# auggiemarignier/pxmcmc

Hardware: AMD Instinct MI355X
Metric: MYULA samples/sec at L=256 synthesis (higher is better)
Workload: dtype f64

## Files before the change

include/pxmcmc_amd.h:

```cpp
#ifndef PXMCMC_AMD_H
#define PXMCMC_AMD_H

#include <stddef.h>
#include <stdint.h>

#ifdef __cplusplus
extern "C" {
#endif

typedef struct pxm_sht_plan_s* pxm_sht_plan_t;
typedef struct pxm_wav_plan_s* pxm_wav_plan_t;
typedef struct pxm_dwav_plan_s* pxm_dwav_plan_t;
typedef struct pxm_hwav_plan_s* pxm_hwav_plan_t;
typedef struct pxm_dft_plan_s* pxm_dft_plan_t;
typedef struct pxm_gemm_plan_s* pxm_gemm_plan_t;
typedef void* pxm_stream_t;

int pxm_version(void);
#ifdef PXM_NOISE_F64
#error "the -DPXM_NOISE_F64 build switch was removed: pass the flag PXM_NOISE_F64 per call (one library serves both precisions)"
#endif
#define PXM_NOISE_F64 16
int pxm_noise_bits(void);
int64_t pxm_host_check_address_ranges(int L, double B, int J_min, int spin, int max_chains, int what);
int64_t pxm_host_gram_table_bytes(int L, double B, int J_min, int spin, int max_chains);
const char* pxm_last_error(void);
int pxm_device_count(void);

int pxm_capture_begin(void);
int pxm_capture_end(void);
int pxm_deferred_pending(void);
int pxm_tables_trim(void);

int pxm_j_max(int L, double B);
int pxm_wav_bandlimits(int L, double B, int J_min, int* bl_out, int cap);
int64_t pxm_wav_ncoefs(int L, double B, int J_min, int64_t* nscal_out);
int pxm_tiling_axisym(int L, double B, int J_min, double* kappa0, double* kappa);
int pxm_mw_ring_weights(int L, double* q);
int pxm_host_sht_tables(int L, int spin, int m, double* Binv, double* Afwd);
int pxm_host_rec_table(int L, int spin, int m, double* Brec);
int pxm_host_rec_geometry(int L, int spin, int C, int* out);
int pxm_host_pfa511_tables(uint16_t* idx, double* b2);
int pxm_host_dft_geometry(int L, int* out);

int pxm_sht_plan_create(int L, int spin, int max_chains, unsigned flags, pxm_sht_plan_t* plan);
int pxm_sht_plan_destroy(pxm_sht_plan_t plan);
int pxm_sht_uses_recursion(pxm_sht_plan_t plan);
int pxm_rec_reduce_selftest(double* out128);
int pxm_sht_inverse(pxm_sht_plan_t plan, const void* flm, void* f, int C, pxm_stream_t stream);
int pxm_sht_forward(pxm_sht_plan_t plan, const void* f, void* flm, int C, pxm_stream_t stream);
int pxm_sht_inverse_adjoint(pxm_sht_plan_t plan, const void* f, void* flm, int C, pxm_stream_t stream);
int pxm_sht_forward_adjoint(pxm_sht_plan_t plan, const void* flm, void* f, int C, pxm_stream_t stream);
int64_t pxm_sht_table_bytes(pxm_sht_plan_t plan, int op );

int pxm_dft_plan_create(int L, int max_chains, pxm_dft_plan_t* plan);
int pxm_dft_plan_destroy(pxm_dft_plan_t plan);
int pxm_dft_px2ring(pxm_dft_plan_t plan, const void* f, void* G, int C, pxm_stream_t stream);
int pxm_dft_ring2px(pxm_dft_plan_t plan, const void* G, void* f, int C, pxm_stream_t stream);
int pxm_dft_status(pxm_dft_plan_t plan, int clear, pxm_stream_t stream);

#define PXM_GEMM_SIDE_INTS 16
int pxm_gemm_plan_create(int spin, int max_chains, int pk, const int* sides, int n_sides, pxm_gemm_plan_t* plan);
int pxm_gemm_plan_destroy(pxm_gemm_plan_t plan);
int64_t pxm_gemm_plan_report(pxm_gemm_plan_t plan, int what, int side, int64_t* out, int64_t cap);
int64_t pxm_host_gemm_plan_report(int spin, int max_chains, int pk, const int* sides, int n_sides, int what, int side,
                                  int64_t* out, int64_t cap);
int pxm_gemm_plan_write(pxm_gemm_plan_t plan, int64_t offset, const double* src, int64_t n, pxm_stream_t stream);
int pxm_gemm_plan_read(pxm_gemm_plan_t plan, int64_t offset, double* dst, int64_t n, pxm_stream_t stream);
int pxm_gemm_plan_table_read(pxm_gemm_plan_t plan, int side, int which, double* dst, int64_t n, pxm_stream_t stream);
int pxm_gemm_plan_run(pxm_gemm_plan_t plan, int C, int affine, double ns, double wr, double wi, int bump, pxm_stream_t stream);

int pxm_wav_plan_create(int L, double B, int J_min, int max_chains, unsigned flags, pxm_wav_plan_t* plan);
int pxm_wav_plan_create_spin(int L, double B, int J_min, int spin, int max_chains, unsigned flags, pxm_wav_plan_t* plan);
int pxm_wav_plan_destroy(pxm_wav_plan_t plan);
int pxm_wav_synthesis(pxm_wav_plan_t plan, const void* X, void* f, int C, pxm_stream_t stream);
int pxm_wav_synthesis_adjoint(pxm_wav_plan_t plan, const void* f, void* X, int C, pxm_stream_t stream);
int pxm_wav_analysis(pxm_wav_plan_t plan, const void* f, void* X, int C, pxm_stream_t stream);
int pxm_wav_analysis_adjoint(pxm_wav_plan_t plan, const void* X, void* f, int C, pxm_stream_t stream);
int64_t pxm_wav_table_bytes(pxm_wav_plan_t plan, int op );

int pxm_dwav_plan_create(int L, double B, int J_min, int N, int max_chains, unsigned flags, pxm_dwav_plan_t* plan);
int pxm_dwav_plan_destroy(pxm_dwav_plan_t plan);
int pxm_dwav_synthesis(pxm_dwav_plan_t plan, const void* X, void* f, int C, pxm_stream_t stream);
int pxm_dwav_synthesis_adjoint(pxm_dwav_plan_t plan, const void* f, void* X, int C, pxm_stream_t stream);
int pxm_dwav_analysis(pxm_dwav_plan_t plan, const void* f, void* X, int C, pxm_stream_t stream);
int pxm_dwav_analysis_adjoint(pxm_dwav_plan_t plan, const void* X, void* f, int C, pxm_stream_t stream);
int64_t pxm_dwav_ncoefs(int L, double B, int J_min, int N, int64_t* nscal_out);
int64_t pxm_dwav_table_bytes(pxm_dwav_plan_t plan);
int pxm_dwav_status(pxm_dwav_plan_t plan, int clear, pxm_stream_t stream);
int pxm_dwav_plan_info(pxm_dwav_plan_t plan, int* nitems, int* split_blocks, int* gamma_blocks);

int pxm_hwav_plan_create(int L, double B, int J_min, int N, int spin, int max_chains, unsigned flags, pxm_hwav_plan_t* plan);
int pxm_hwav_plan_destroy(pxm_hwav_plan_t plan);
int pxm_hwav_synthesis(pxm_hwav_plan_t plan, const void* X, void* flm, int C, pxm_stream_t stream);
int pxm_hwav_synthesis_adjoint(pxm_hwav_plan_t plan, const void* flm, void* X, int C, pxm_stream_t stream);
int pxm_hwav_analysis(pxm_hwav_plan_t plan, const void* flm, void* X, int C, pxm_stream_t stream);
int pxm_hwav_analysis_adjoint(pxm_hwav_plan_t plan, const void* X, void* flm, int C, pxm_stream_t stream);
int64_t pxm_hwav_ncoefs(int L, double B, int J_min, int N, int64_t* nscal_out);
int pxm_hwav_status(pxm_hwav_plan_t plan, int clear, pxm_stream_t stream);
int pxm_hwav_myula_step(pxm_hwav_plan_t plan, const void* X, const void* data, const void* invcov, int invcov_complex,
                        const double* kernel, const double* T, double T_scalar, double delta, double lmda, int mode,
                        uint64_t seed, uint64_t chain0, uint64_t iter, const uint64_t* iter_dev, void* X_out,
                        void* preds_out, int C, pxm_stream_t stream);
int pxm_hwav_plan_info(pxm_hwav_plan_t plan, int* nitems, int* split_blocks, int* kact);

int pxm_wav_set_iter_counter(pxm_wav_plan_t plan, uint64_t* counter_dev);
int pxm_wav_release_iter_counter(pxm_wav_plan_t plan, const uint64_t* counter_dev);
int pxm_wav_iter_counter_add(pxm_wav_plan_t plan, uint64_t inc, pxm_stream_t stream);
#define PXM_STATUS_PAIR_SYNC 2
int pxm_wav_status(pxm_wav_plan_t plan, int clear, pxm_stream_t stream);
int pxm_sht_status(pxm_sht_plan_t plan, int clear, pxm_stream_t stream);
int pxm_wav_exact_dft_scales(pxm_wav_plan_t plan);

int pxm_wav_profile_enable(pxm_wav_plan_t plan, int max_launches);
int pxm_wav_profile_read(pxm_wav_plan_t plan, double* gemm_ms, int64_t* gemm_launches, double* gemm_alg_bytes,
                         double* gemm_flops);
int pxm_wav_profile_read_dft(pxm_wav_plan_t plan, double* dft_ms, int64_t* dft_launches, double* dft_alg_bytes);
int pxm_wav_profile_read_launches(pxm_wav_plan_t plan, double* launch_ms, double* launch_alg_bytes,
                                  int32_t* launch_workgroups, int64_t cap, int64_t* launches);
int64_t pxm_wav_workspace_nonfinite(pxm_wav_plan_t plan, pxm_stream_t stream);

#define PXM_MODE_REAL_NOISE 0
#define PXM_MODE_CPLX_NOISE 1
#define PXM_MODE_REAL_PAIRS 2
int pxm_wav_gradg_step(pxm_wav_plan_t plan, const void* X, const void* preds, const void* data,
                       const void* invcov, int invcov_complex, const double* T, double T_scalar,
                       double delta, double lmda, const void* noise, int mode,
                       uint64_t seed, uint64_t chain0, uint64_t iter, void* X_out, int C,
                       pxm_stream_t stream);

int pxm_wav_image_init(pxm_wav_plan_t plan, const void* preds, const void* data, const void* invcov,
                       int invcov_complex, int C, pxm_stream_t stream);
int pxm_wav_image_step(pxm_wav_plan_t plan, const void* X, const void* data, const void* invcov,
                       int invcov_complex, const double* T, double T_scalar, double delta, double lmda,
                       const void* noise, int mode, uint64_t seed, uint64_t chain0, uint64_t iter,
                       void* X_out, void* preds_out, int C, pxm_stream_t stream);

int pxm_wav_ring_set_data(pxm_wav_plan_t plan, const void* data, pxm_stream_t stream);
int pxm_wav_ring_init(pxm_wav_plan_t plan, const void* X, int C, pxm_stream_t stream);
int pxm_wav_ring_step(pxm_wav_plan_t plan, const void* X, double w_re, double w_im, const double* T,
                      double T_scalar, double delta, double lmda, const void* noise, int mode,
                      uint64_t seed, uint64_t chain0, uint64_t iter, void* X_out, int C, pxm_stream_t stream);
int pxm_wav_ring_preds(pxm_wav_plan_t plan, void* preds, int C, pxm_stream_t stream);

int pxm_wav_wl_attach(pxm_wav_plan_t plan, const int32_t* pix2data, const double* weight, int64_t ndata);
int pxm_wav_wl_uses_recursion(pxm_wav_plan_t plan);
int pxm_wav_wl_forward(pxm_wav_plan_t plan, const void* X, void* gamma, int C, pxm_stream_t stream);
int pxm_wav_wl_adjoint(pxm_wav_plan_t plan, const void* gamma, const void* data, const void* invcov,
                       int invcov_complex, void* X_out, int C, pxm_stream_t stream);

int pxm_soft(const void* X, const double* T, double T_scalar, void* out, int64_t n, int C, int dtype,
             pxm_stream_t stream);
int pxm_residual_grad(const void* preds, const void* data, const void* invcov, int invcov_complex,
                      void* out, int64_t n, int C, int dtype, pxm_stream_t stream);
int pxm_myula_step(const void* X, const void* gradg, const double* T, double T_scalar,
                   const double* delta_dev, double delta, double lmda, const void* noise,
                   int noise_complex, uint64_t seed, uint64_t chain0, uint64_t iter,
                   const uint64_t* iter_dev, void* X_out, int64_t n, int C, int dtype,
                   pxm_stream_t stream);
int pxm_chain_step(const void* X, const void* proxf, const void* gradg, const double* delta_dev,
                   double delta, double lmda, const void* noise, int noise_complex, uint64_t seed,
                   uint64_t chain0, uint64_t iter, const uint64_t* iter_dev, void* X_out, int64_t n,
                   int C, int dtype, pxm_stream_t stream);
int pxm_skrock_stage(const void* U, const void* proxf, const double* T, double T_scalar, const void* gradg,
                     const void* V, double a, double b, double c, double e, double r, const void* noise,
                     int noise_complex, uint64_t seed, uint64_t chain0, uint64_t iter, const uint64_t* iter_dev,
                     void* out, int64_t n, int C, int dtype, pxm_stream_t stream);
#define PXM_FISTA_SLICES_MAX 256
int pxm_fista_step(const void* Y, const void* gradg, const void* proxf, const double* T, double T_scalar,
                   const void* X_prev, double gamma, double lmda, const double* beta_table, int64_t n_beta,
                   uint64_t iter, const uint64_t* iter_dev, void* X_out, void* Y_out, double* sums, double* scratch,
                   int64_t n, int C, int dtype, pxm_stream_t stream);
int pxm_fista_step_restart(const void* Y, const void* gradg, const void* proxf, const double* T, double T_scalar,
                           const void* X_prev, double gamma, double lmda, const double* beta_table, int64_t n_beta,
                           uint64_t* momentum_index, uint64_t* restarts, int restart_on, void* X_out, void* Y_out,
                           double* sums, double* scratch, int64_t n, int C, int dtype, pxm_stream_t stream);
#define PXM_SAPG_SLICES_MAX 256
int pxm_sapg_step(const void* X, const void* gradg, const double* T, double T_scalar, double delta, double lmda,
                  const void* noise, int noise_complex, uint64_t seed, uint64_t chain0, uint64_t iter,
                  const uint64_t* iter_dev, double* theta, double* eta, double d, const double* rho_table, int64_t n_rho,
                  double eta_min, double eta_max, int pool, double* trace, int64_t n_trace, void* X_out, double* scratch,
                  int64_t n, int C, int dtype, pxm_stream_t stream);
#define PXM_SAPG_GROUPS_MAX 32
int pxm_sapg_step_groups(const void* X, const void* gradg, const double* T, double T_scalar, double delta, double lmda,
                         const void* noise, int noise_complex, uint64_t seed, uint64_t chain0, uint64_t iter,
                         const uint64_t* iter_dev, double* theta, double* eta, const int64_t* bounds, int K, const double* d,
                         const double* rho_table, int64_t n_rho, double eta_min, double eta_max, int pool, double* trace,
                         int64_t n_trace, void* X_out, double* scratch, int64_t n, int C, int dtype, pxm_stream_t stream);
#define PXM_LCI_POINTS 32
#define PXM_LCI_ROUNDS_MAX 64
#define PXM_LCI_EMPTY 1
#define PXM_LCI_UNCONSTRAINED 2
#define PXM_LCI_NONFINITE 4
int64_t pxm_lci_scratch_doubles(int64_t n, int C);
int pxm_lci_data_terms(const void* preds_a, const void* preds_b, const void* data, const double* w, double* quad,
                       double* scratch, int64_t ndata, int C, int dtype, pxm_stream_t stream);
int pxm_lci_eval(const void* a, const void* b, const double* T, double T_scalar, const double* xi, double* P,
                 double* scratch, int64_t n, int C, int dtype, pxm_stream_t stream);
int pxm_lci_search(const void* a, const void* b, const double* T, double T_scalar, const double* quad, double lmda,
                   const double* gamma, int rounds, double* out, int* status, double* scratch, int64_t n, int C, int dtype,
                   pxm_stream_t stream);
int pxm_randn(void* out, int64_t n, int C, int dtype, uint64_t seed, uint64_t chain0, uint64_t iter,
              pxm_stream_t stream);
int pxm_box_muller(const double* u1, const double* u2, double* z0, double* z1, int64_t n, int f64, pxm_stream_t stream);
int64_t pxm_reduce_scratch_doubles(int C);
int pxm_reduce_l1(const void* X, const double* w, double* out, double* scratch, int64_t n, int C, int dtype,
                  pxm_stream_t stream);
int pxm_reduce_l2(const void* preds, const void* data, const void* invcov, int invcov_complex,
                  double* out, double* scratch, int64_t n, int C, int dtype, pxm_stream_t stream);
int pxm_reduce_vdot(const void* a, const void* b, double* out, double* scratch, int64_t n, int C, int dtype,
                    pxm_stream_t stream);
int pxm_quantile_range(const double* chain, int64_t nsamples, int64_t nparams, int64_t ld, double alpha, double* out,
                       pxm_stream_t stream);
int pxm_logtransition(const void* X1, const void* X2, const void* proxf, const void* gradg,
                      const double* delta_dev, double delta, double lmda, double* out, double* scratch,
                      int64_t n, int C, int dtype, pxm_stream_t stream);
int pxm_pxmala_propose(const void* X, const void* proxf, const void* gradg, const double* T, double T_scalar,
                       const double* prior_weights, const double* delta_dev, double lmda, const void* noise,
                       int noise_complex, uint64_t seed, uint64_t chain0, uint64_t iter, const uint64_t* iter_dev,
                       void* X_prop, void* proxf_prop, double* logtrans_out, double* prior_out, double* scratch,
                       int64_t n, int C, int dtype, pxm_stream_t stream);
int pxm_pxmala_accept(const double* logtrans_pc, const double* logtrans_cp, const double* prior_p, const double* L2_p,
                      double mu, double* logpi_c, double* L2_c, double* prior_c, const double* u, uint64_t seed,
                      uint64_t chain0, uint64_t iter, const uint64_t* iter_dev, int32_t* accept_out, double* delta_dev,
                      int tune, double lmda, int32_t* acc_trace, double* delta_trace, int chunk, int C,
                      pxm_stream_t stream);
int pxm_pxmala_finish(const void* X_prop, const void* X_curr, const void* proxf_prop, const double* T, double T_scalar,
                      const void* gradg_prop, int64_t n, int dtype, const void* preds_prop, const void* data, const void* invcov, int invcov_complex,
                      int64_t n_data, int data_dtype, const double* propose_scratch, double mu, double lmda, double* logpi_c,
                      double* L2_c, double* prior_c, const double* u, uint64_t seed, uint64_t chain0, uint64_t iter,
                      const uint64_t* iter_dev, int32_t* accept_out, double* delta_dev, int tune, int32_t* acc_trace,
                      double* delta_trace, int chunk, double* logtrans_pc_out, double* logtrans_cp_out, double* prior_p_out,
                      double* L2_p_out, double* scratch, uint64_t* bump_counter, int C, pxm_stream_t stream);
int pxm_select_copy_many(const int32_t* flag, int narrays, const void* const* src, void* const* dst, const int64_t* n,
                         const int* esize, int C, pxm_stream_t stream);
int pxm_counter_add(uint64_t* counter_dev, uint64_t inc, pxm_stream_t stream);

int pxm_moments_update(const double* x, int x_stride, int64_t* count, double* mean, double* m2, const int* mask,
                       const double* logpi, int logpi_stride, double* best_logpi, double* best_x, int64_t m, int C,
                       pxm_stream_t stream);
int64_t pxm_moments_scratch_doubles(int64_t m);
int pxm_moments_finalize(const int64_t* count, const double* mean, const double* m2, int64_t m, int C, double* pooled_mean,
                         double* pooled_var, double* rhat, double* stats, double* scratch, pxm_stream_t stream);

int64_t pxm_tails_buffer_doubles(int64_t m, int C, int64_t k);
int64_t pxm_tails_stage_doubles(int64_t m, int C);
int pxm_tails_update(const double* x, int x_stride, const int64_t* count, double* lo, double* hi, double* thr_lo, double* thr_hi,
                     double* stage, const int* mask, int64_t m, int C, int64_t k, int64_t nsamples, pxm_stream_t stream);
int pxm_tails_quantiles(const int64_t* count, const double* lo, const double* hi, const double* stage, int64_t m, int C, int64_t k,
                        int64_t nsamples, double alpha, double* q_lo, double* q_hi, pxm_stream_t stream);

int pxm_acov_stage_depth(void);
int64_t pxm_acov_state_doubles(int64_t m, int C, int K);
int64_t pxm_acov_ring_doubles(int64_t m, int C, int K);
int64_t pxm_acov_scratch_doubles(int64_t m);
int pxm_acov_update(const double* x, int x_stride, const int64_t* count, double* acc, double* tot, double* head, double* ring,
                    const int* mask, int64_t m, int C, int K, pxm_stream_t stream);
int pxm_acov_ess(const int64_t* count, const double* acc, const double* tot, const double* head, const double* ring, int64_t m, int C,
                 int K, double* ess, int* ess_lag, double* ess_pooled, double* mcse, double* stats, double* scratch,
                 pxm_stream_t stream);

int pxm_wl_harmonic_mapping(const void* flm, const double* kernel, void* out, int64_t n, int C,
                            pxm_stream_t stream);
int pxm_wl_mask_gather(const void* f, const int64_t* idx, const double* w, void* out, int64_t npix,
                       int64_t ndata, int C, pxm_stream_t stream);
// ... 12 lines not shown
```

pxmcmc_amd/_lib.py:

```python
import ctypes as C
import os

import torch

_HERE = os.path.dirname(os.path.abspath(__file__))
LIB_PATH = os.environ.get("PXM_LIB_PATH") or os.path.join(_HERE, "lib", "libpxmcmc_amd.so")

c_i64, c_u64, c_int, c_dbl, c_vp = C.c_int64, C.c_uint64, C.c_int, C.c_double, C.c_void_p

SIGNATURES = {
    "pxm_version": (c_int, []),
    "pxm_noise_bits": (c_int, []),
    "pxm_host_check_address_ranges": (c_i64, [c_int, c_dbl, c_int, c_int, c_int, c_int]),
    "pxm_host_gram_table_bytes": (c_i64, [c_int, c_dbl, c_int, c_int, c_int]),
    "pxm_last_error": (C.c_char_p, []),
    "pxm_device_count": (c_int, []),
    "pxm_capture_begin": (c_int, []),
    "pxm_capture_end": (c_int, []),
    "pxm_deferred_pending": (c_int, []),
    "pxm_tables_trim": (c_int, []),
    "pxm_wav_set_iter_counter": (c_int, [c_vp, c_vp]),
    "pxm_wav_release_iter_counter": (c_int, [c_vp, c_vp]),
    "pxm_wav_iter_counter_add": (c_int, [c_vp, c_u64, c_vp]),
    "pxm_wav_exact_dft_scales": (c_int, [c_vp]),
    "pxm_wav_status": (c_int, [c_vp, c_int, c_vp]),
    "pxm_sht_status": (c_int, [c_vp, c_int, c_vp]),
    "pxm_wav_profile_enable": (c_int, [c_vp, c_int]),
    "pxm_wav_profile_read": (c_int, [c_vp, c_vp, c_vp, c_vp, c_vp]),
    "pxm_wav_profile_read_launches": (c_int, [c_vp, c_vp, c_vp, c_vp, c_i64, c_vp]),
    "pxm_wav_profile_read_dft": (c_int, [c_vp, c_vp, c_vp, c_vp]),
    "pxm_wav_workspace_nonfinite": (c_i64, [c_vp, c_vp]),
    "pxm_reduce_scratch_doubles": (c_i64, [c_int]),
    "pxm_j_max": (c_int, [c_int, c_dbl]),
    "pxm_wav_bandlimits": (c_int, [c_int, c_dbl, c_int, c_vp, c_int]),
    "pxm_wav_ncoefs": (c_i64, [c_int, c_dbl, c_int, c_vp]),
    "pxm_tiling_axisym": (c_int, [c_int, c_dbl, c_int, c_vp, c_vp]),
    "pxm_mw_ring_weights": (c_int, [c_int, c_vp]),
    "pxm_host_sht_tables": (c_int, [c_int, c_int, c_int, c_vp, c_vp]),
    "pxm_host_rec_table": (c_int, [c_int, c_int, c_int, c_vp]),
    "pxm_host_rec_geometry": (c_int, [c_int, c_int, c_int, c_vp]),
    "pxm_host_pfa511_tables": (c_int, [c_vp, c_vp]),
    "pxm_host_dft_geometry": (c_int, [c_int, c_vp]),
    "pxm_quantile_range": (c_int, [c_vp, c_i64, c_i64, c_i64, c_dbl, c_vp, c_vp]),
    "pxm_moments_update": (c_int, [c_vp, c_int, c_vp, c_vp, c_vp, c_vp, c_vp, c_int, c_vp, c_vp, c_i64, c_int, c_vp]),
    "pxm_moments_scratch_doubles": (c_i64, [c_i64]),
    "pxm_moments_finalize": (c_int, [c_vp, c_vp, c_vp, c_i64, c_int, c_vp, c_vp, c_vp, c_vp, c_vp, c_vp]),
    "pxm_tails_buffer_doubles": (c_i64, [c_i64, c_int, c_i64]),
    "pxm_tails_stage_doubles": (c_i64, [c_i64, c_int]),
    "pxm_tails_update": (c_int, [c_vp, c_int, c_vp, c_vp, c_vp, c_vp, c_vp, c_vp, c_vp, c_i64, c_int, c_i64, c_i64, c_vp]),
    "pxm_tails_quantiles": (c_int, [c_vp, c_vp, c_vp, c_vp, c_i64, c_int, c_i64, c_i64, c_dbl, c_vp, c_vp, c_vp]),
    "pxm_acov_stage_depth": (c_int, []),
    "pxm_acov_state_doubles": (c_i64, [c_i64, c_int, c_int]),
    "pxm_acov_ring_doubles": (c_i64, [c_i64, c_int, c_int]),
    "pxm_acov_scratch_doubles": (c_i64, [c_i64]),
    "pxm_acov_update": (c_int, [c_vp, c_int, c_vp, c_vp, c_vp, c_vp, c_vp, c_vp, c_i64, c_int, c_int, c_vp]),
    "pxm_acov_ess": (c_int, [c_vp, c_vp, c_vp, c_vp, c_vp, c_i64, c_int, c_int, c_vp, c_vp, c_vp, c_vp, c_vp, c_vp, c_vp]),
    "pxm_sht_uses_recursion": (c_int, [c_vp]),
    "pxm_rec_reduce_selftest": (c_int, [c_vp]),
    "pxm_sht_plan_create": (c_int, [c_int, c_int, c_int, C.c_uint, C.POINTER(c_vp)]),
    "pxm_sht_plan_destroy": (c_int, [c_vp]),
    "pxm_sht_inverse": (c_int, [c_vp, c_vp, c_vp, c_int, c_vp]),
    "pxm_sht_forward": (c_int, [c_vp, c_vp, c_vp, c_int, c_vp]),
    "pxm_sht_inverse_adjoint": (c_int, [c_vp, c_vp, c_vp, c_int, c_vp]),
    "pxm_sht_forward_adjoint": (c_int, [c_vp, c_vp, c_vp, c_int, c_vp]),
    "pxm_sht_table_bytes": (c_i64, [c_vp, c_int]),
    "pxm_dft_plan_create": (c_int, [c_int, c_int, C.POINTER(c_vp)]),
    "pxm_dft_plan_destroy": (c_int, [c_vp]),
    "pxm_dft_px2ring": (c_int, [c_vp, c_vp, c_vp, c_int, c_vp]),
    "pxm_dft_ring2px": (c_int, [c_vp, c_vp, c_vp, c_int, c_vp]),
    "pxm_dft_status": (c_int, [c_vp, c_int, c_vp]),
    "pxm_gemm_plan_create": (c_int, [c_int, c_int, c_int, c_vp, c_int, C.POINTER(c_vp)]),
    "pxm_gemm_plan_destroy": (c_int, [c_vp]),
    "pxm_gemm_plan_report": (c_i64, [c_vp, c_int, c_int, c_vp, c_i64]),
    "pxm_host_gemm_plan_report": (c_i64, [c_int, c_int, c_int, c_vp, c_int, c_int, c_int, c_vp, c_i64]),
    "pxm_gemm_plan_write": (c_int, [c_vp, c_i64, c_vp, c_i64, c_vp]),
    "pxm_gemm_plan_read": (c_int, [c_vp, c_i64, c_vp, c_i64, c_vp]),
    "pxm_gemm_plan_table_read": (c_int, [c_vp, c_int, c_int, c_vp, c_i64, c_vp]),
    "pxm_gemm_plan_run": (c_int, [c_vp, c_int, c_int, c_dbl, c_dbl, c_dbl, c_int, c_vp]),
    "pxm_dwav_plan_create": (c_int, [c_int, c_dbl, c_int, c_int, c_int, C.c_uint, C.POINTER(c_vp)]),
    "pxm_dwav_plan_destroy": (c_int, [c_vp]),
    "pxm_dwav_synthesis": (c_int, [c_vp, c_vp, c_vp, c_int, c_vp]),
    "pxm_dwav_synthesis_adjoint": (c_int, [c_vp, c_vp, c_vp, c_int, c_vp]),
    "pxm_dwav_analysis": (c_int, [c_vp, c_vp, c_vp, c_int, c_vp]),
    "pxm_dwav_analysis_adjoint": (c_int, [c_vp, c_vp, c_vp, c_int, c_vp]),
    "pxm_dwav_ncoefs": (c_i64, [c_int, c_dbl, c_int, c_int, c_vp]),
    "pxm_dwav_table_bytes": (c_i64, [c_vp]),
    "pxm_dwav_status": (c_int, [c_vp, c_int, c_vp]),
    "pxm_dwav_plan_info": (c_int, [c_vp, c_vp, c_vp, c_vp]),
    "pxm_hwav_plan_create": (c_int, [c_int, c_dbl, c_int, c_int, c_int, c_int, C.c_uint, C.POINTER(c_vp)]),
    "pxm_hwav_plan_destroy": (c_int, [c_vp]),
    "pxm_hwav_synthesis": (c_int, [c_vp, c_vp, c_vp, c_int, c_vp]),
    "pxm_hwav_synthesis_adjoint": (c_int, [c_vp, c_vp, c_vp, c_int, c_vp]),
    "pxm_hwav_analysis": (c_int, [c_vp, c_vp, c_vp, c_int, c_vp]),
    "pxm_hwav_analysis_adjoint": (c_int, [c_vp, c_vp, c_vp, c_int, c_vp]),
    "pxm_hwav_ncoefs": (c_i64, [c_int, c_dbl, c_int, c_int, c_vp]),
    "pxm_hwav_status": (c_int, [c_vp, c_int, c_vp]),
    "pxm_hwav_plan_info": (c_int, [c_vp, c_vp, c_vp, c_vp]),
    "pxm_hwav_myula_step": (
        c_int,
        [c_vp, c_vp, c_vp, c_vp, c_int, c_vp, c_vp, c_dbl, c_dbl, c_dbl, c_int, c_u64, c_u64, c_u64, c_vp, c_vp, c_vp, c_int, c_vp],
    ),
    "pxm_wav_plan_create": (c_int, [c_int, c_dbl, c_int, c_int, C.c_uint, C.POINTER(c_vp)]),
    "pxm_wav_plan_create_spin": (c_int, [c_int, c_dbl, c_int, c_int, c_int, C.c_uint, C.POINTER(c_vp)]),
    "pxm_wav_plan_destroy": (c_int, [c_vp]),
    "pxm_wav_synthesis": (c_int, [c_vp, c_vp, c_vp, c_int, c_vp]),
    "pxm_wav_synthesis_adjoint": (c_int, [c_vp, c_vp, c_vp, c_int, c_vp]),
    "pxm_wav_analysis": (c_int, [c_vp, c_vp, c_vp, c_int, c_vp]),
    "pxm_wav_analysis_adjoint": (c_int, [c_vp, c_vp, c_vp, c_int, c_vp]),
    "pxm_wav_table_bytes": (c_i64, [c_vp, c_int]),
    "pxm_wav_gradg_step": (
        c_int,
        [c_vp, c_vp, c_vp, c_vp, c_vp, c_int, c_vp, c_dbl, c_dbl, c_dbl, c_vp, c_int, c_u64, c_u64, c_u64, c_vp, c_int, c_vp],
    ),
    "pxm_wav_image_init": (c_int, [c_vp, c_vp, c_vp, c_vp, c_int, c_int, c_vp]),
    "pxm_wav_image_step": (
        c_int,
        [c_vp, c_vp, c_vp, c_vp, c_int, c_vp, c_dbl, c_dbl, c_dbl, c_vp, c_int, c_u64, c_u64, c_u64, c_vp, c_vp, c_int, c_vp],
    ),
    "pxm_wav_ring_set_data": (c_int, [c_vp, c_vp, c_vp]),
    "pxm_wav_ring_init": (c_int, [c_vp, c_vp, c_int, c_vp]),
    "pxm_wav_ring_step": (
        c_int,
        [c_vp, c_vp, c_dbl, c_dbl, c_vp, c_dbl, c_dbl, c_dbl, c_vp, c_int, c_u64, c_u64, c_u64, c_vp, c_int, c_vp],
    ),
    "pxm_wav_ring_preds": (c_int, [c_vp, c_vp, c_int, c_vp]),
    "pxm_wav_wl_attach": (c_int, [c_vp, c_vp, c_vp, c_i64]),
    "pxm_wav_wl_uses_recursion": (c_int, [c_vp]),
    "pxm_wav_wl_forward": (c_int, [c_vp, c_vp, c_vp, c_int, c_vp]),
    "pxm_wav_wl_adjoint": (c_int, [c_vp, c_vp, c_vp, c_vp, c_int, c_vp, c_int, c_vp]),
    "pxm_soft": (c_int, [c_vp, c_vp, c_dbl, c_vp, c_i64, c_int, c_int, c_vp]),
    "pxm_residual_grad": (c_int, [c_vp, c_vp, c_vp, c_int, c_vp, c_i64, c_int, c_int, c_vp]),
    "pxm_myula_step": (
        c_int,
        [c_vp, c_vp, c_vp, c_dbl, c_vp, c_dbl, c_dbl, c_vp, c_int, c_u64, c_u64, c_u64, c_vp, c_vp, c_i64, c_int, c_int, c_vp],
    ),
    "pxm_chain_step": (
        c_int,
        [c_vp, c_vp, c_vp, c_vp, c_dbl, c_dbl, c_vp, c_int, c_u64, c_u64, c_u64, c_vp, c_vp, c_i64, c_int, c_int, c_vp],
    ),
    "pxm_skrock_stage": (
        c_int,
        [c_vp, c_vp, c_vp, c_dbl, c_vp, c_vp, c_dbl, c_dbl, c_dbl, c_dbl, c_dbl, c_vp, c_int, c_u64, c_u64, c_u64, c_vp, c_vp,
         c_i64, c_int, c_int, c_vp],
    ),
    "pxm_fista_step": (
        c_int,
        [c_vp, c_vp, c_vp, c_vp, c_dbl, c_vp, c_dbl, c_dbl, c_vp, c_i64, c_u64, c_vp, c_vp, c_vp, c_vp, c_vp, c_i64, c_int, c_int,
         c_vp],
    ),
    "pxm_fista_step_restart": (
        c_int,
        [c_vp, c_vp, c_vp, c_vp, c_dbl, c_vp, c_dbl, c_dbl, c_vp, c_i64, c_vp, c_vp, c_int, c_vp, c_vp, c_vp, c_vp, c_i64, c_int,
         c_int, c_vp],
    ),
    "pxm_lci_scratch_doubles": (c_i64, [c_i64, c_int]),
    "pxm_lci_data_terms": (c_int, [c_vp, c_vp, c_vp, c_vp, c_vp, c_vp, c_i64, c_int, c_int, c_vp]),
    "pxm_lci_eval": (c_int, [c_vp, c_vp, c_vp, c_dbl, c_vp, c_vp, c_vp, c_i64, c_int, c_int, c_vp]),
    "pxm_lci_search": (c_int, [c_vp, c_vp, c_vp, c_dbl, c_vp, c_dbl, c_vp, c_int, c_vp, c_vp, c_vp, c_i64, c_int, c_int, c_vp]),
    "pxm_sapg_step": (
        c_int,
        [c_vp, c_vp, c_vp, c_dbl, c_dbl, c_dbl, c_vp, c_int, c_u64, c_u64, c_u64, c_vp, c_vp, c_vp, c_dbl, c_vp, c_i64, c_dbl, c_dbl,
         c_int, c_vp, c_i64, c_vp, c_vp, c_i64, c_int, c_int, c_vp],
    ),
    "pxm_sapg_step_groups": (
        c_int,
        [c_vp, c_vp, c_vp, c_dbl, c_dbl, c_dbl, c_vp, c_int, c_u64, c_u64, c_u64, c_vp, c_vp, c_vp, c_vp, c_int, c_vp, c_vp, c_i64,
         c_dbl, c_dbl, c_int, c_vp, c_i64, c_vp, c_vp, c_i64, c_int, c_int, c_vp],
    ),
    "pxm_randn": (c_int, [c_vp, c_i64, c_int, c_int, c_u64, c_u64, c_u64, c_vp]),
    "pxm_box_muller": (c_int, [c_vp, c_vp, c_vp, c_vp, c_i64, c_int, c_vp]),
    "pxm_reduce_l1": (c_int, [c_vp, c_vp, c_vp, c_vp, c_i64, c_int, c_int, c_vp]),
    "pxm_reduce_l2": (c_int, [c_vp, c_vp, c_vp, c_int, c_vp, c_vp, c_i64, c_int, c_int, c_vp]),
    "pxm_reduce_vdot": (c_int, [c_vp, c_vp, c_vp, c_vp, c_i64, c_int, c_int, c_vp]),
    "pxm_logtransition": (c_int, [c_vp, c_vp, c_vp, c_vp, c_vp, c_dbl, c_dbl, c_vp, c_vp, c_i64, c_int, c_int, c_vp]),
    "pxm_pxmala_propose": (
        c_int,
        [c_vp, c_vp, c_vp, c_vp, c_dbl, c_vp, c_vp, c_dbl, c_vp, c_int, c_u64, c_u64, c_u64, c_vp, c_vp, c_vp, c_vp, c_vp, c_vp,
         c_i64, c_int, c_int, c_vp],
    ),
    "pxm_pxmala_accept": (
        c_int,
        [c_vp, c_vp, c_vp, c_vp, c_dbl, c_vp, c_vp, c_vp, c_vp, c_u64, c_u64, c_u64, c_vp, c_vp, c_vp, c_int, c_dbl, c_vp, c_vp,
         c_int, c_int, c_vp],
    ),
    "pxm_pxmala_finish": (
        c_int,
        [c_vp, c_vp, c_vp, c_vp, c_dbl, c_vp, c_i64, c_int, c_vp, c_vp, c_vp, c_int, c_i64, c_int, c_vp, c_dbl, c_dbl, c_vp, c_vp,
         c_vp, c_vp, c_u64, c_u64, c_u64, c_vp, c_vp, c_vp, c_int, c_vp, c_vp, c_int, c_vp, c_vp, c_vp, c_vp, c_vp, c_vp, c_int,
         c_vp],
    ),
    "pxm_select_copy_many": (c_int, [c_vp, c_int, c_vp, c_vp, c_vp, c_vp, c_int, c_vp]),
    "pxm_counter_add": (c_int, [c_vp, c_u64, c_vp]),
    "pxm_wl_harmonic_mapping": (c_int, [c_vp, c_vp, c_vp, c_i64, c_int, c_vp]),
    "pxm_wl_mask_gather": (c_int, [c_vp, c_vp, c_vp, c_vp, c_i64, c_i64, c_int, c_vp]),
    "pxm_wl_mask_scatter": (c_int, [c_vp, c_vp, c_vp, c_vp, c_i64, c_i64, c_int, c_vp]),
# ... 55 lines not shown
```

pxmcmc_amd/csrc/dft.hip:

```cpp
#include "dft_unit.h"
#include "elem.h"
#include "update.h"

#include <cstdlib>

namespace pxm {

struct DftArgs {
  int L, n, M, logM, Rp, R;
  const double2* chirp;
  const double2* bhat;
  const double2* tw;
};

__device__ inline void bluestein_core(double2* buf, const double2* tw, const DftArgs& a) {
  const int M = a.M, half = M >> 1, R = a.R;
  const int total = R * half;
  for (int s = half, st = 1; s >= 1; s >>= 1, st <<= 1) {
    __syncthreads();
    for (int idx = threadIdx.x; idx < total; idx += blockDim.x) {
      const int r = idx / half, b = idx - r * half;
      const int g = b / s, p = b - g * s;
      double2* x = buf + r * M + g * 2 * s + p;
      const double2 u = x[0], v = x[s];
      x[0] = cadd(u, v);
      x[s] = cmul(csub(u, v), tw[p * st]);
    }
  }
  __syncthreads();
  for (int idx = threadIdx.x; idx < R * M; idx += blockDim.x) {
    const int j = idx & (M - 1);
    buf[idx] = cmul(buf[idx], a.bhat[j]);
  }
  for (int s = 1, st = half; s <= half; s <<= 1, st >>= 1) {
    __syncthreads();
    for (int idx = threadIdx.x; idx < total; idx += blockDim.x) {
      const int r = idx / half, b = idx - r * half;
      const int g = b / s, p = b - g * s;
      double2* x = buf + r * M + g * 2 * s + p;
      const double2 u = x[0], v = cmulc(x[s], tw[p * st]);
      x[0] = cadd(u, v);
      x[s] = csub(u, v);
    }
  }
  __syncthreads();
}

__global__ void k_px2ring(DftArgs a, PxIn in, double* __restrict__ G, int ncol, int C) {
  extern __shared__ double2 lds[];
  double2* tw = lds;
  double2* buf = lds + (a.M >> 1);
  const int t = blockIdx.x, c0 = blockIdx.y * a.R;
  const int n = a.n, M = a.M, R = a.R;
  if (in.bump && blockIdx.x == 0 && blockIdx.y == 0 && threadIdx.x == 0) *in.bump += 1;
  for (int k = threadIdx.x; k < (M >> 1); k += blockDim.x) tw[k] = a.tw[k];
  for (int idx = threadIdx.x; idx < R * M; idx += blockDim.x) {
    const int r = idx / M, j = idx - r * M;
    const int c = c0 + r;
    double2 v{0.0, 0.0};
    if (j < n && c < C) {
      const int64_t e = in.ring0 + (int64_t)t * n + j;
      v = px_in_load(in, c, e);
      v = cmul(v, a.chirp[j]);
    }
    buf[idx] = v;
  }
  bluestein_core(buf, tw, a);
  const int Cp = ncol >> 1;
  for (int idx = threadIdx.x; idx < n * R; idx += blockDim.x) {
    const int k = idx / R, r = idx - k * R;
    const int c = c0 + r;
    if (c >= Cp) continue;
    const double2 y = cmul(buf[r * M + k], a.chirp[k]);
    const int m = (k < a.L) ? k : k - n;
    reinterpret_cast<double2*>(G)[((int64_t)(m + a.L - 1) * a.Rp + t) * Cp + c] = y;
  }
}

__global__ void k_ring2px(DftArgs a, const double* __restrict__ G, int ncol, PxOut out, int C) {
  extern __shared__ double2 lds[];
  double2* tw = lds;
  double2* buf = lds + (a.M >> 1);
  const int t = blockIdx.x, c0 = blockIdx.y * a.R;
  const int n = a.n, M = a.M, R = a.R;
  const int Cp = ncol >> 1;
  for (int k = threadIdx.x; k < (M >> 1); k += blockDim.x) tw[k] = a.tw[k];
  for (int idx = threadIdx.x; idx < (M - n) * R; idx += blockDim.x) {
    const int r = idx / (M - n), j = n + idx - r * (M - n);
    buf[r * M + j] = double2{0.0, 0.0};
  }
  for (int idx = threadIdx.x; idx < n * R; idx += blockDim.x) {
    const int k = idx / R, r = idx - k * R;
    const int c = c0 + r;
    double2 v{0.0, 0.0};
    if (c < Cp) {
      const int m = (k < a.L) ? k : k - n;
      v = reinterpret_cast<const double2*>(G)[((int64_t)(m + a.L - 1) * a.Rp + t) * Cp + c];
      v.y = -v.y;
      v = cmul(v, a.chirp[k]);
    }
    buf[r * M + k] = v;
  }
  bluestein_core(buf, tw, a);
  for (int idx = threadIdx.x; idx < R * n; idx += blockDim.x) {
    const int r = idx / n, p = idx - r * n;
    const int c = c0 + r;
    if (c >= C) continue;
    double2 y = cmul(buf[r * M + p], a.chirp[p]);
    y.y = -y.y;
    const int64_t e = out.ring0 + (int64_t)t * n + p;
    const int64_t ce = (int64_t)c * out.chain_stride + e;
    if (out.X) {
      const uint64_t it_eff = out.iter + (out.iter_dev ? *out.iter_dev : 0);
      const double2 x = reinterpret_cast<const double2*>(out.X)[ce];
      const double T = out.T ? out.T[e] : out.T_scalar;
      const double2 w = out.noise ? px_noise_load(out, c, e) : px_noise_philox(out, c, e, it_eff);
      reinterpret_cast<double2*>(out.f)[ce] = px_update(out, x, T, y, w);
    } else {
      px_out_store(out, c, e, y);
    }
  }
}

int dft_geometry(int L, DftGeometry* g) {
  PXM_REQUIRE(L >= 1 && L <= (1 << 28), "dft_geometry: need 1 <= L <= 2^28");
  const int n = 2 * L - 1;
  const bool radix2_only = getenv("PXM_DFT_NO_W") != nullptr;
  const char* pfa_env = getenv("PXM_DFT_PFA");
  *g = DftGeometry();
  g->pfa = !(pfa_env && atoi(pfa_env) == 0);
  if (!radix2_only && pair_r0(n)) {
    g->unit = DFT_PAIR;
    g->M = 128 * pair_r0(n);
    pair_workgroup(n, g->pfa, &g->per_wg, &g->threads, &g->lds, &g->exact);
  } else if (!radix2_only && n <= 1023) {
    g->unit = DFT_QUAD;
    g->M = 2048;
    quad_workgroup(&g->per_wg, &g->threads, &g->lds);
  } else {
    g->unit = DFT_RADIX2;
    g->M = bluestein_size(n);
    int R = 8;
    while (R > 1 && (size_t)R * g->M * 16 > 128 * 1024) R >>= 1;
    g->per_wg = R;
    g->lds = ((size_t)R * g->M + g->M / 2) * 16;
    const int64_t th = (int64_t)R * g->M / 2;
    g->threads = th < 64 ? 64 : (th > 1024 ? 1024 : (int)th);
  }
  PXM_REQUIRE(g->lds <= DFT_LDS_MAX, "phi-DFT stage: no unit for bandlimit L = " + std::to_string(L) + ": the radix-2 unit at M = " +
                                         std::to_string(g->M) + " needs " + std::to_string(g->lds) + " B of LDS per workgroup, a CU has " +
                                         std::to_string(DFT_LDS_MAX) + " (the largest bandlimit is L = 1024)");
  return 0;
}

int make_dft_plan(int L, DftPlan* p) {
  DftGeometry g;
  if (int rc = dft_geometry(L, &g)) return rc;
  p->L = L;
  p->n = 2 * L - 1;
  p->Rp = round_up(L, 16);
  p->unit = g.unit;
  if (g.unit == DFT_PAIR) {
    if (const char* e = getenv("PXM_DEBUG_PAIR_SYNC_LIMIT")) p->spin_limit = (unsigned)std::max(0, atoi(e));
    return pair_make_tables(p->n, g.pfa, &p->pair);
  }
  if (g.unit == DFT_QUAD) return quad_make_tables(p->n, &p->quad);
  BluesteinTables b = make_bluestein(p->n, g.M);
  PXM_REQUIRE(b.M == g.M, "make_dft_plan: the Bluestein tables disagree with dft_geometry");
  p->M = b.M;
  p->logM = b.logM;
  p->R = g.per_wg;
  p->lds = g.lds;
  p->threads = g.threads;
  int rc;
  if ((rc = dev_table(&p->d_chirp, b.chirp, "Bluestein chirp"))) return rc;
  if ((rc = dev_table(&p->d_bhat, b.bhat, "Bluestein filter spectrum"))) return rc;
  if ((rc = dev_table(&p->d_tw, b.tw, "radix-2 twiddles"))) return rc;
  static std::atomic<uint64_t> lds_done{0};
  return allow_dynamic_lds(lds_done, {reinterpret_cast<const void*>(k_px2ring), reinterpret_cast<const void*>(k_ring2px)});
}

void free_dft_plan(DftPlan* p) {
  for (double** d : {&p->d_chirp, &p->d_bhat, &p->d_tw, &p->pair.d_all, &p->quad.d_all}) {
    if (*d) deferred_free(*d);
    *d = nullptr;
  }
}

static DftArgs make_args(const DftPlan& p) {
  DftArgs a;
  a.L = p.L;
  a.n = p.n;
  a.M = p.M;
  a.logM = p.logM;
  a.Rp = p.Rp;
  a.R = p.R;
  a.chirp = reinterpret_cast<const double2*>(p.d_chirp);
  a.bhat = reinterpret_cast<const double2*>(p.d_bhat);
  a.tw = reinterpret_cast<const double2*>(p.d_tw);
  return a;
}

int launch_px2ring(const DftPlan& p, const PxIn& in, double* G, int ncol, int C, hipStream_t stream) {
  switch (p.unit) {
    case DFT_PAIR: return pair_px2ring(p, in, G, ncol, C, stream);
    case DFT_QUAD: return quad_px2ring(p, in, G, ncol, C, stream);
    case DFT_RADIX2: break;
  }
  const int Cp = ncol / 2;
  dim3 grid(p.L, (Cp + p.R - 1) / p.R), block(p.threads);
  hipLaunchKernelGGL(k_px2ring, grid, block, p.lds, stream, make_args(p), in, G, ncol, C);
  PXM_HIP(hipGetLastError());
  return 0;
}

int launch_ring2px2ring(const DftPlan& p, double* G, int ncol, const PxOut& out, int C, hipStream_t stream) {
  PXM_REQUIRE(dft_can_fuse(p), "launch_ring2px2ring: the plan's DFT unit has no fused rings -> pixels -> rings kernel");
  return pair_ring2px(p, G, ncol, out, C, stream, true);
}

int launch_ring2px(const DftPlan& p, const double* G, int ncol, const PxOut& out, int C, hipStream_t stream) {
  switch (p.unit) {
    case DFT_PAIR: return pair_ring2px(p, G, ncol, out, C, stream, false);
    case DFT_QUAD: return quad_ring2px(p, G, ncol, out, C, stream);
    case DFT_RADIX2: break;
  }
  dim3 grid(p.L, (C + p.R - 1) / p.R), block(p.threads);
  hipLaunchKernelGGL(k_ring2px, grid, block, p.lds, stream, make_args(p), G, ncol, out, C);
  PXM_HIP(hipGetLastError());
  return 0;
}

__global__ void k_lm_to_mel(const double2* __restrict__ flm, double2* __restrict__ H, int L, int Rp, int Cp, int C,
                            int spin) {
  const int64_t total = (int64_t)(2 * L - 1) * Rp * Cp;
  for (int64_t i = blockIdx.x * (int64_t)blockDim.x + threadIdx.x; i < total; i += (int64_t)gridDim.x * blockDim.x) {
    const int c = (int)(i % Cp);
    const int el = (int)((i / Cp) % Rp);
    const int m = (int)(i / ((int64_t)Cp * Rp)) - (L - 1);
    double2 v{0.0, 0.0};
    const int am = m < 0 ? -m : m, as = spin < 0 ? -spin : spin;
    if (c < C && el < L && el >= am && el >= as) v = flm[(int64_t)c * L * L + (int64_t)el * el + el + m];
    H[i] = v;
  }
}

__global__ void k_mel_to_lm(const double2* __restrict__ H, double2* __restrict__ flm, int L, int Rp, int Cp, int C,
                            int spin) {
  const int64_t total = (int64_t)C * L * L;
  for (int64_t i = blockIdx.x * (int64_t)blockDim.x + threadIdx.x; i < total; i += (int64_t)gridDim.x * blockDim.x) {
    const int c = (int)(i / ((int64_t)L * L));
    const int lm = (int)(i - (int64_t)c * L * L);
    int el = (int)sqrt((double)lm);
    while ((el + 1) * (el + 1) <= lm) ++el;
    while (el * el > lm) --el;
    const int m = lm - el * el - el;
    const int as = spin < 0 ? -spin : spin;
    double2 v{0.0, 0.0};
    if (el >= as) v = H[((int64_t)(m + L - 1) * Rp + el) * Cp + c];
    flm[i] = v;
  }
}

int launch_lm_to_mel(const double* flm, double* H, int L, int Rp, int ncol, int C, int spin, hipStream_t stream) {
  const int Cp = ncol / 2;
  const int64_t total = (int64_t)(2 * L - 1) * Rp * Cp;
  int blocks = (int)std::min<int64_t>((total + 255) / 256, 4096);
  hipLaunchKernelGGL(k_lm_to_mel, dim3(blocks), dim3(256), 0, stream, reinterpret_cast<const double2*>(flm),
                     reinterpret_cast<double2*>(H), L, Rp, Cp, C, spin);
  PXM_HIP(hipGetLastError());
  return 0;
}

int launch_mel_to_lm(const double* H, double* flm, int L, int Rp, int ncol, int C, int spin, hipStream_t stream) {
  const int Cp = ncol / 2;
  const int64_t total = (int64_t)C * L * L;
  int blocks = (int)std::min<int64_t>((total + 255) / 256, 4096);
  hipLaunchKernelGGL(k_mel_to_lm, dim3(blocks), dim3(256), 0, stream, reinterpret_cast<const double2*>(H),
                     reinterpret_cast<double2*>(flm), L, Rp, Cp, C, spin);
  PXM_HIP(hipGetLastError());
  return 0;
}

}
```

pxmcmc_amd/csrc/dft_pfa.h:

```cpp
#pragma once
#include "dft_wave.h"

namespace pxm {

constexpr int PFA_N = 511;
constexpr int PFA_PLANE = 576;
constexpr int PFA_Y0 = 504;
constexpr int PFA_TAB_GAT = 0;
constexpr int PFA_TAB_KIDX = 128;
constexpr int PFA_TAB_B2 = 288;
constexpr int PFA_TAB_DOUBLES = 288 + 144;

template <int SGN>
__device__ __forceinline__ void pfa_dft3(double2& a, double2& b, double2& c) {
  constexpr double C3 = 0.86602540378443864676 * (SGN > 0 ? 1.0 : -1.0);
  const double2 s = cadd(b, c), d = csub(b, c);
  const double2 m{fma(s.x, -0.5, a.x), fma(s.y, -0.5, a.y)};
  a = cadd(a, s);
  b = double2{fma(-C3, d.y, m.x), fma(C3, d.x, m.y)};
  c = double2{fma(C3, d.y, m.x), fma(-C3, d.x, m.y)};
}

template <int SGN>
__device__ __forceinline__ void pfa_dft9(double2 (&x)[9]) {
  constexpr double S = SGN > 0 ? 1.0 : -1.0;
  constexpr double2 W1{0.76604444311897803520, S * 0.64278760968653932632};
  constexpr double2 W2{0.17364817766693034885, S * 0.98480775301220805937};
  constexpr double2 W4{-0.93969262078590838405, S * 0.34202014332566873304};
  pfa_dft3<SGN>(x[0], x[3], x[6]);
  pfa_dft3<SGN>(x[1], x[4], x[7]);
  pfa_dft3<SGN>(x[2], x[5], x[8]);
  x[4] = cmul(x[4], W1);
  x[5] = cmul(x[5], W2);
  x[7] = cmul(x[7], W2);
  x[8] = cmul(x[8], W4);
  pfa_dft3<SGN>(x[0], x[1], x[2]);
  pfa_dft3<SGN>(x[3], x[4], x[5]);
  pfa_dft3<SGN>(x[6], x[7], x[8]);
  d5_swap(x[1], x[3]);
  d5_swap(x[2], x[6]);
  d5_swap(x[5], x[7]);
}

template <int SGN>
__device__ __forceinline__ void pfa_dft7(double2 (&x)[7]) {
  constexpr double c1 = 0.62348980185873353053, c2 = -0.22252093395631440429, c3 = -0.90096886790241912624;
  constexpr double s1 = 0.78183148246802980871, s2 = 0.97492791218182360702, s3 = 0.43388373911755812048;
  const double2 p1 = cadd(x[1], x[6]), p2 = cadd(x[2], x[5]), p3 = cadd(x[3], x[4]);
  const double2 m1 = csub(x[1], x[6]), m2 = csub(x[2], x[5]), m3 = csub(x[3], x[4]);
  const double2 x0 = x[0];
  x[0] = cadd(cadd(x0, p1), cadd(p2, p3));
  auto comb = [&](double ca, double cb, double cc, double sa, double sb, double sc, double2& lo, double2& hi) {
    const double2 a{fma(p3.x, cc, fma(p2.x, cb, fma(p1.x, ca, x0.x))), fma(p3.y, cc, fma(p2.y, cb, fma(p1.y, ca, x0.y)))};
    double2 b{fma(m3.x, sc, fma(m2.x, sb, m1.x * sa)), fma(m3.y, sc, fma(m2.y, sb, m1.y * sa))};
    if (SGN < 0) b = double2{-b.x, -b.y};
    lo = double2{a.x - b.y, a.y + b.x};
    hi = double2{a.x + b.y, a.y - b.x};
  };
  comb(c1, c2, c3, s1, s2, s3, x[1], x[6]);
  comb(c2, c3, c1, s2, -s3, -s1, x[2], x[5]);
  comb(c3, c1, c2, s3, -s1, s2, x[3], x[4]);
}

__device__ __forceinline__ unsigned pfa_u16(const uint4& v, int k) {
  const unsigned w = k < 2 ? v.x : (k < 4 ? v.y : (k < 6 ? v.z : v.w));
  return (k & 1) ? (w >> 16) : (w & 0xffffu);
}

__device__ __forceinline__ void pfa511_core(double2 (&z)[8], const double2 x0, double2 (&o1)[7], double2 (&o2)[7], double2* plane,
                                            const double2* B2l, int lane) {
  const int j1l = lane / 9, q9l = lane - 9 * j1l;
  const int j1m = lane >> 3, k8m = lane & 7;
  dft8r<-1, 0>(z);
  if (lane < 63) {
    double2* w = plane + j1l * 72 + q9l;
#pragma unroll
    for (int k = 0; k < 8; ++k) w[9 * k] = z[k];
  }
  d5_wave_sync();
  double2 y[9];
  double2* const a2 = plane + (j1m < 7 ? j1m : 6) * 72 + k8m * 9;
#pragma unroll
  for (int k = 0; k < 9; ++k) y[k] = a2[k];
  d5_wave_sync();
  pfa_dft9<-1>(y);
  const double2 Y0 = cadd(x0, y[0]);
  const double2* bw = B2l + k8m * 9;
#pragma unroll
  for (int k = 0; k < 9; ++k) y[k] = cmul(y[k], bw[k]);
  if (k8m == 0) y[0] = cadd(y[0], x0);
  pfa_dft9<+1>(y);
  if (lane < 56) {
#pragma unroll
    for (int k = 0; k < 9; ++k) a2[k] = y[k];
    if (k8m == 0) plane[PFA_Y0 + j1m] = Y0;
  }
  d5_wave_sync();
  {
    const double2* r3 = plane + (j1l < 7 ? j1l : 6) * 72 + q9l;
#pragma unroll
    for (int k = 0; k < 8; ++k) z[k] = r3[9 * k];
  }
  d5_wave_sync();
  dft8r<+1, 0>(z);
  if (lane < 63) {
    double2* w = plane + q9l * 7 + j1l;
#pragma unroll
    for (int k = 0; k < 8; ++k) w[63 * k] = z[k];
  }
  d5_wave_sync();
  {
    const double2* r4 = plane + lane * 7;
    const double2* r5 = plane + (64 + (lane < 9 ? lane : 8)) * 7;
#pragma unroll
    for (int k = 0; k < 7; ++k) o1[k] = r4[k];
#pragma unroll
    for (int k = 0; k < 7; ++k) o2[k] = r5[k];
  }
  d5_wave_sync();
  pfa_dft7<-1>(o1);
  pfa_dft7<-1>(o2);
}


struct PfaTabs {
  const uint16_t* gat;
  const uint16_t* kidx;
  const double2* B2;
};

constexpr int PFA_STAGE_S = 514;
static_assert(4 * PFA_STAGE_S <= 4 * PFA_PLANE, "a ring group's stage fits in its four planes");

template <bool RING_OUT, bool N64>
__device__ __forceinline__ void ring2px_body_pfa(const Dft5Args& a, const PfaTabs& pt, double* __restrict__ G, int ncol,
                                                 const PxOut& out, int C, int bxw, int by, int passes, double2* lds5) {
  if ((by << 2) >= C) return;
#ifdef PXM_D5_TRACE
  unsigned long long d5_stamp[7] = {0, 0, 0, 0, 0, 0, 0};
  unsigned long long d5_t0 = wall_clock64();
#endif
  constexpr int n = PFA_N, R = 4, S = PFA_STAGE_S;
#define PXM_PFA_THREAD_SETUP                                                                                              \
  int tid = threadIdx.x;                                                                                                  \
  asm volatile("" : "+v"(tid));                                                                                           \
  const int wave = __builtin_amdgcn_readfirstlane(tid >> 6), lane = tid & 63;                                             \
  const int r = wave & 3, grp = wave >> 2;  \
  const int c0 = by * R, ch = c0 + r;                                                                                     \
  const int Cp = ncol >> 1;                                                                                               \
  double2* stage = lds5 + grp * (4 * PFA_PLANE);               \
  double2* plane = lds5 + wave * PFA_PLANE;                                                                               \
  double2* B2l = lds5 + 8 * PFA_PLANE;                                                                                    \
  const double2* const logt = B2l + 72;                                                                                   \
  const double2* const sct = B2l + 72 + NOISE_LOG_N;                                                                      \
  unsigned* const gcnt = reinterpret_cast<unsigned*>(B2l + 72 + NOISE_LOG_N + 256) + grp;                                 \
  const int j1m = lane >> 3;                                                                                              \
  const int x0k = (73 * (j1m < 7 ? j1m : 6)) % n;                          \
  const int mstride = a.Rp * Cp;                                              \
                   \
  const int rr = tid & (R - 1), kq = (tid & 255) >> 2;                                                                    \
  const bool cv = c0 + rr < Cp;                                                                                           \
  double2* const Gc = reinterpret_cast<double2*>(G) + c0 + rr;
#define PXM_PFA_RING_LOAD(TT)                                                                                             \
  {                                                                 \
    const int tt_ = (TT);                                                                                                 \
    const bool rv_ = cv && tt_ < a.L;                                                                                     \
    _Pragma("unroll") for (int i = 0; i < 8; ++i) {                                                                       \
      const int k = kq + 64 * i;                                                                                          \
      v[i] = double2{0.0, 0.0};                                                                                           \
      if (rv_ && k < n) v[i] = Gc[((k < a.L) ? k + a.L - 1 : k - a.L) * mstride + tt_ * Cp];                              \
    }                                                                                                                     \
  }
  double2 v[8];
  unsigned epoch = 0;
  const D5Sync sy{a.err, a.spin_limit};
  {
    PXM_PFA_THREAD_SETUP
    (void)ch; (void)stage; (void)plane; (void)logt; (void)sct; (void)gcnt; (void)x0k; (void)lane;
    if (tid < 72) B2l[tid] = pt.B2[tid];
#if !defined(PXM_NOISE_F64_POLY)
    if (N64 && out.X && !out.noise && tid < NOISE_LOG_N + 256)
      B2l[72 + tid] = tid < NOISE_LOG_N ? reinterpret_cast<const double2*>(&NOISE_LOG_TAB[0][0])[tid]
                                        : reinterpret_cast<const double2*>(&NOISE_SINCOS_TAB[0][0])[tid - NOISE_LOG_N];
#endif
    if (tid < 2) reinterpret_cast<unsigned*>(B2l + 72 + NOISE_LOG_N + 256)[tid] = 0;
    PXM_PFA_RING_LOAD((bxw * passes) * 2 + grp)
  }
  d5_barrier();
#pragma nounroll
  for (int ps = 0; ps < passes; ++ps) {
  PXM_PFA_THREAD_SETUP
  const int t = (bxw * passes + ps) * 2 + grp;
  const bool tv = t < a.L;
#pragma unroll
  for (int i = 0; i < 8; ++i) {
    const int k = kq + 64 * i;
    if (k < n) stage[rr * S + k] = double2{v[i].x, -v[i].y};
  }
  d5_pair_sync(gcnt, epoch += 4, lane, sy);
  PXM_D5_STAMP(0)
  double2 z[8], o1[7], o2[7];
  double2 x0;
  {
    const char* sb = reinterpret_cast<const char*>(stage + r * S);
    const uint4 gv = reinterpret_cast<const uint4*>(pt.gat)[lane];
#pragma unroll
    for (int q = 0; q < 8; ++q) z[q] = *reinterpret_cast<const double2*>(sb + pfa_u16(gv, q));
    x0 = *reinterpret_cast<const double2*>(sb + 16 * x0k);
  }
  d5_pair_sync(gcnt, epoch += 4, lane, sy);
  PXM_D5_STAMP(1)
  pfa511_core(z, x0, o1, o2, plane, B2l, lane);
  PXM_D5_STAMP(2)
  {
    char* pb_ = reinterpret_cast<char*>(plane);
    const uint4 kv1 = reinterpret_cast<const uint4*>(pt.kidx)[lane];
    const uint4 kv2 = reinterpret_cast<const uint4*>(pt.kidx)[64 + (lane < 9 ? lane : 8)];
#pragma unroll
    for (int k = 0; k < 7; ++k) *reinterpret_cast<double2*>(pb_ + pfa_u16(kv1, k)) = o1[k];
    if (lane < 9) {
#pragma unroll
      for (int k = 0; k < 7; ++k) *reinterpret_cast<double2*>(pb_ + pfa_u16(kv2, k)) = o2[k];
    }
    d5_wave_sync();
  }
  const bool act = ch < C && tv;
  const int64_t e0 = out.ring0 + (int64_t)t * n + lane;
  const int64_t ce0 = (int64_t)ch * out.chain_stride + e0;
  const bool last_ok = lane < 63;
  const uint64_t it_eff = out.iter + (out.iter_dev ? *out.iter_dev : 0);
  const int ch_s = __builtin_amdgcn_readfirstlane(ch);
#pragma unroll
  for (int g0 = 0; g0 < 8; g0 += 4) {
    double2 x[4];
    if (!N64 || !(act && out.X)) {
#pragma unroll
      for (int u = 0; u < 4; ++u) x[u] = plane[lane + 64 * (g0 + u)];
    }
    if (act && out.X) {
      double2 xs[4], wn[4], wph[4];
      double Ts[4];
      int eo[4];
#pragma unroll
      for (int u = 0; u < 4; ++u) eo[u] = (g0 + u < 7 || last_ok) ? 64 * (g0 + u) : -lane;
#pragma unroll
      for (int u = 0; u < 4; ++u) xs[u] = reinterpret_cast<const double2*>(out.X)[ce0 + eo[u]];
      if (out.T) {
#pragma unroll
        for (int u = 0; u < 4; ++u) Ts[u] = out.T[e0 + eo[u]];
      } else {
#pragma unroll
        for (int u = 0; u < 4; ++u) Ts[u] = out.T_scalar;
      }
      if (out.noise) {
#pragma unroll
        for (int u = 0; u < 4; ++u) wn[u] = px_noise_load(out, ch, e0 + eo[u]);
      } else {
#pragma unroll
        for (int u = 0; u < 4; ++u) wn[u] = double2{0.0, 0.0};
      }
      __builtin_amdgcn_sched_barrier(0);
#if !defined(PXM_NOISE_F64_POLY)
      if (N64 && !out.noise && out.mode == PXM_MODE_REAL_PAIRS && !(out.chain0 & 1)) {
        uint4 pbits[4];
#pragma unroll
        for (int u = 0; u < 4; ++u)
          pbits[u] = philox_bits(out.seed + PXM_PAIR_TWEAK, (out.chain0 >> 1) + ch_s, (uint64_t)(e0 + 64 * (g0 + u)), it_eff);
        __builtin_amdgcn_sched_barrier(0);
#pragma unroll
        for (int u = 0; u < 4; ++u) {
          const NormalPair q_ = normal_pair_from_bits_tabs(pbits[u], logt, sct);
          wph[u] = double2{q_.z0, q_.z1};
          __builtin_amdgcn_sched_barrier(0);
        }
      } else
#endif
      {
#pragma unroll
      for (int u = 0; u < 4; ++u) {
        wph[u] = double2{0.0, 0.0};
#if defined(PXM_NOISE_F64_POLY)
        if (!out.noise) wph[u] = px_noise_philox_t<N64>(out, ch_s, e0 + 64 * (g0 + u), it_eff);
#else
        if (!out.noise) wph[u] = N64 ? px_noise_philox_tabs(out, ch_s, e0 + 64 * (g0 + u), it_eff, logt, sct)
                                     : px_noise_philox_t<false>(out, ch_s, e0 + 64 * (g0 + u), it_eff);
#endif
        __builtin_amdgcn_sched_barrier(0);
      }
      }
      if (N64) {
#pragma unroll
        for (int u = 0; u < 4; ++u) x[u] = plane[lane + 64 * (g0 + u)];
      }
#pragma unroll
      for (int u = 0; u < 4; ++u) {
        const int p = g0 + u;
        if (p == 7 && !last_ok) {
          x[u] = double2{0.0, 0.0};
          continue;
        }
        const double2 y{x[u].x, -x[u].y};
        const double2 w = out.noise ? wn[u] : wph[u];
        x[u] = px_update(out, xs[u], Ts[u], y, w);
        reinterpret_cast<double2*>(out.f)[ce0 + 64 * p] = x[u];
      }
    } else if (act) {
      bool ok[4];
      int64_t ev[4];
      double2 yv[4];
#pragma unroll
      for (int u = 0; u < 4; ++u) {
        ok[u] = g0 + u < 7 || last_ok;
        ev[u] = ok[u] ? e0 + 64 * (g0 + u) : out.ring0 + (int64_t)t * n;
        yv[u] = double2{x[u].x, -x[u].y};
      }
      px_out_store_n<4>(out, ch, ev, yv, ok);
      if (out.rdata) {
        double2 rd[4], rc[4];
#pragma unroll
        for (int u = 0; u < 4; ++u) rd[u] = reinterpret_cast<const double2*>(out.rdata)[ev[u]];
        if (out.rinvcov_complex) {
#pragma unroll
          for (int u = 0; u < 4; ++u) rc[u] = reinterpret_cast<const double2*>(out.rinvcov)[ev[u]];
        } else {
#pragma unroll
          for (int u = 0; u < 4; ++u) rc[u] = double2{out.rinvcov[ev[u]], 0.0};
        }
#pragma unroll
        for (int u = 0; u < 4; ++u) {
          const double2 d = csub(yv[u], rd[u]);
          yv[u] = out.rinvcov_complex ? cmul(rc[u], d) : double2{rc[u].x * d.x, rc[u].x * d.y};
        }
      }
#pragma unroll
      for (int u = 0; u < 4; ++u) x[u] = ok[u] ? yv[u] : double2{0.0, 0.0};
    } else {
#pragma unroll
      for (int u = 0; u < 4; ++u) x[u] = double2{0.0, 0.0};
    }
    if (RING_OUT) {
#pragma unroll
      for (int u = 0; u < 4; ++u) plane[lane + 64 * (g0 + u)] = x[u];
    }
#ifdef PXM_D5_TRACE
    if (g0 == 0) PXM_D5_STAMP(3) else PXM_D5_STAMP(4)
#endif
  }
  if (!RING_OUT) {
    PXM_PFA_RING_LOAD(ps + 1 < passes ? (bxw * passes + ps + 1) * 2 + grp : a.L)
    if (ps + 1 < passes) d5_pair_sync(gcnt, epoch += 4, lane, sy);
    continue;
  }
  d5_wave_sync();
  {
    const char* pb_ = reinterpret_cast<const char*>(plane);
    const uint4 gv = reinterpret_cast<const uint4*>(pt.gat)[lane];
#pragma unroll
    for (int q = 0; q < 8; ++q) z[q] = *reinterpret_cast<const double2*>(pb_ + pfa_u16(gv, q));
    x0 = plane[x0k];
  }
  d5_wave_sync();
  pfa511_core(z, x0, o1, o2, plane, B2l, lane);
  PXM_D5_STAMP(5)
  d5_pair_sync(gcnt, epoch += 4, lane, sy);
  {
    char* sb = reinterpret_cast<char*>(stage + r * S);
    const uint4 kv1 = reinterpret_cast<const uint4*>(pt.kidx)[lane];
    const uint4 kv2 = reinterpret_cast<const uint4*>(pt.kidx)[64 + (lane < 9 ? lane : 8)];
#pragma unroll
    for (int k = 0; k < 7; ++k) *reinterpret_cast<double2*>(sb + pfa_u16(kv1, k)) = o1[k];
    if (lane < 9) {
#pragma unroll
      for (int k = 0; k < 7; ++k) *reinterpret_cast<double2*>(sb + pfa_u16(kv2, k)) = o2[k];
    }
  }
  PXM_PFA_RING_LOAD(ps + 1 < passes ? (bxw * passes + ps + 1) * 2 + grp : a.L)
  d5_pair_sync(gcnt, epoch += 4, lane, sy);
  PXM_D5_STAMP(6)
  if (cv && tv) {
#pragma unroll
    for (int i = 0; i < 8; ++i) {
      const int k = kq + 64 * i;
      if (k < n) Gc[((k < a.L) ? k + a.L - 1 : k - a.L) * mstride + t * Cp] = stage[rr * S + k];
    }
  }
  if (ps + 1 < passes) d5_pair_sync(gcnt, epoch += 4, lane, sy);
// ... 114 lines not shown
```

pxmcmc_amd/csrc/dft_plan.hip:

```cpp
#include "plan_common.h"

#include <memory>

using namespace pxm;

struct pxm_dft_plan_s {
  int L = 0, Cmax = 0, Cp = 0, ncol = 0, Rp = 0;
  DftPlan dft;
  unsigned* d_status = nullptr;
};

extern "C" {

int pxm_host_dft_geometry(int L, int* out) {
  PXM_REQUIRE(out, "pxm_host_dft_geometry: null output");
  PXM_REQUIRE(L >= 1, "pxm_host_dft_geometry: need L >= 1");
  DftGeometry g;
  if (int rc = dft_geometry(L, &g)) return rc;
  out[0] = g.unit == DFT_RADIX2 ? 0 : (g.unit == DFT_PAIR ? 1 : 2);
  out[1] = g.M;
  out[2] = g.per_wg;
  out[3] = g.threads;
  out[4] = (int)g.lds;
  out[5] = g.exact ? 1 : 0;
  return 0;
}

int pxm_dft_plan_create(int L, int max_chains, pxm_dft_plan_t* plan) {
  PXM_REQUIRE(plan, "pxm_dft_plan_create: null plan pointer");
  PXM_REQUIRE(L >= 1, "pxm_dft_plan_create: Bandlimit must be greater than 0");
  PXM_REQUIRE(max_chains >= 1, "pxm_dft_plan_create: max_chains must be >= 1");
  PXM_REQUIRE(dry_run() || pxm_device_count() > 0, "pxm_dft_plan_create: no HIP device visible (the HIP path is the only path)");
  drain_deferred();
  std::unique_ptr<pxm_dft_plan_s, int (*)(pxm_dft_plan_t)> guard(new pxm_dft_plan_s(), pxm_dft_plan_destroy);
  pxm_dft_plan_s* p = guard.get();
  p->L = L;
  p->Cmax = max_chains;
  p->Cp = round_up(max_chains, 8);
  p->ncol = 2 * p->Cp;
  p->Rp = round_up(L, 16);
  int rc;
  if ((rc = make_dft_plan(L, &p->dft))) return rc;
  if ((rc = status_alloc(&p->d_status))) return rc;
  p->dft.d_status = p->d_status;
  *plan = guard.release();
  return 0;
}

int pxm_dft_plan_destroy(pxm_dft_plan_t p) {
  if (!p) return 0;
  free_dft_plan(&p->dft);
  deferred_free(p->d_status);
  delete p;
  drain_deferred();
  return 0;
}

int pxm_dft_px2ring(pxm_dft_plan_t p, const void* f, void* G, int C, pxm_stream_t s) {
  if (int rc = plan_check(p, f, G, C, "pxm_dft_px2ring")) return rc;
  PXM_REQUIRE(((uintptr_t)G & 15) == 0, "pxm_dft_px2ring: the ring array must be 16-byte aligned");
  note_stream((hipStream_t)s);
  return launch_px2ring(p->dft, image_in(p->L, f), (double*)G, p->ncol, C, (hipStream_t)s);
}

int pxm_dft_ring2px(pxm_dft_plan_t p, const void* G, void* f, int C, pxm_stream_t s) {
  if (int rc = plan_check(p, G, f, C, "pxm_dft_ring2px")) return rc;
  PXM_REQUIRE(((uintptr_t)G & 15) == 0, "pxm_dft_ring2px: the ring array must be 16-byte aligned");
  note_stream((hipStream_t)s);
  return launch_ring2px(p->dft, (const double*)G, p->ncol, image_out(p->L, f), C, (hipStream_t)s);
}

int pxm_dft_status(pxm_dft_plan_t p, int clear, pxm_stream_t stream) {
  PXM_REQUIRE(p, "pxm_dft_status: null plan");
  return status_read(p->d_status, (hipStream_t)stream, clear);
}

}
```

pxmcmc_amd/csrc/dft_wave.hip:

```cpp
#include "dft_unit.h"
#include "dft_wave.h"
#include "update.h"

#include <hip/hip_ext.h>

#include <algorithm>
#include <cmath>
#include <complex>
#include <cstdlib>
#include <cstring>
#include <vector>

namespace pxm {

constexpr int D5_RMAX = 4;

struct Dft5Args {
  int L, n, Rp;
  int lgR;
  const double2* cE;
  const double2* cO;
  const double2* dO;
  const double2* tw1;
  const double2* wt;
  const double2* bE;
  const double2* bO;
  unsigned* err;
  unsigned spin_limit;
  const double* pfa;
};

struct Dft5Group {
  Dft5Args a;
  int64_t g_off;
  int64_t ring0;
  int r0;
  int b0, nbx, nby;
  int xs;
  int64_t tbase;
  int toff[7];
  int pfa_off;
  int pfa_passes;
};

template <int R0>
__device__ __forceinline__ void d5_dft_half(double2 (&x)[8], double2* plane, int lane, const D5Lane& q, int jb, int half,
                                            const Dft5Args& a, const double2* tw) {
  const double2* __restrict__ cin = (half ? a.cO : a.cE) + jb;
  const double2* __restrict__ cout = (half ? a.dO : a.cE) + jb;
#pragma unroll
  for (int p = 0; p < 8; ++p) x[p] = cmul(x[p], cin[8 * R0 * p]);
  d5_conv<R0>(x, plane, lane, q, tw, half ? a.bO : a.bE);
#pragma unroll
  for (int p = 0; p < 8; ++p) x[p] = cmul(x[p], cout[8 * R0 * p]);
}
template <int SLOT>
__device__ __forceinline__ void d5_exchange_sum(double2 (&x)[8], double2* plane, double2* pplane, int lane, int half,
                                                unsigned* pcnt, unsigned& epoch, const D5Sync& sy) {
#pragma unroll
  for (int u = 0; u < 4; ++u) plane[256 * SLOT + 64 * u + lane] = d5_sel(half, x[u], x[4 + u]);
  d5_pair_sync(pcnt, epoch += 2, lane, sy);
#pragma unroll
  for (int u = 0; u < 4; ++u) x[u] = cadd(d5_sel(half, x[4 + u], x[u]), pplane[256 * SLOT + 64 * u + lane]);
}
template <int SLOT>
__device__ __forceinline__ void d5_exchange_fill(double2 (&x)[8], double2* plane, double2* pplane, int lane, int half,
                                                 unsigned* pcnt, unsigned& epoch, const D5Sync& sy) {
#pragma unroll
  for (int u = 0; u < 4; ++u) plane[256 * SLOT + 64 * u + lane] = x[u];
  d5_pair_sync(pcnt, epoch += 2, lane, sy);
#pragma unroll
  for (int u = 0; u < 4; ++u) {
    const double2 o = pplane[256 * SLOT + 64 * u + lane], own = x[u];
    x[u] = d5_sel(half, o, own);
    x[4 + u] = d5_sel(half, own, o);
  }
}

#define PXM_D5_GEOMETRY                                                                     \
  constexpr int RPW = 8 / R0;                                                               \
  constexpr int lgR = 2, R = 4;                        \
  const int n = a.n;                                                                        \
   \
  if (R0 > 1) __builtin_assume(n > 32 * R0 && n <= 64 * R0);                                \
  const int wave = __builtin_amdgcn_readfirstlane((int)(threadIdx.x >> 6)), lane = threadIdx.x & 63;  \
  const int half = wave & 1, unit = wave >> 1;                  \
  const D5Lane q{lane & 7, lane >> 3};                                                      \
  const int r = unit;                                           \
  const int rho = q.lo / R0;                           \
  const int jb = (q.lo & (R0 - 1)) + R0 * q.hi;        \
  constexpr int TRS = RPW;                                         \
  const int trs = rho;                                   \
  const int t = bx * TRS + trs;                                               \
  const int c0 = by * R, ch = c0 + r;                                                       \
  const bool tv = t < a.L;                                                                  \
  const int Cp = ncol >> 1;                                                                 \
  const int rsh = 4 - lgR;                             \
  constexpr int P1 = 4;                                \
  const int pb = 4 * half;                                      \
  double2* stage = lds5;                                                                    \
  double2* plane = lds5 + wave * D5_PLANE;                                                  \
  double2* pplane = lds5 + (wave ^ 1) * D5_PLANE;                                           \
  const double2* tw = lds5 + 2 * R * D5_PLANE;         \
   \
  unsigned* pcnt = reinterpret_cast<unsigned*>(lds5 + 2 * R * D5_PLANE + 448) + unit;       \
  unsigned epoch = 0;                                                                       \
  const D5Sync sy{a.err, a.spin_limit};                                                     \
  for (int i = threadIdx.x; i < D5_TW; i += 512)                                     \
    lds5[2 * R * D5_PLANE + i] = i < 448 ? a.tw1[64 + i] : (i < 456 ? double2{0.0, 0.0} : a.wt[i - 448]);
#define PXM_D5_SLOT(RING, K, CH) ((((RING)*n + (K)) << lgR) + (((CH) + ((K) >> rsh)) & (R - 1)))

#define PXM_D5_STORE_RINGS(ZFILL)                                                                              \
  {                                                                                                            \
    const int rr = threadIdx.x & (R - 1), kq = threadIdx.x >> lgR, kstep = (512 >> lgR) ;                 \
    const int mstride = a.Rp * Cp;                                 \
    double2* Gc = reinterpret_cast<double2*>(G) + c0 + rr;                                                     \
    const bool zf = (ZFILL) && c0 + R >= C;                                                                    \
    if (c0 + rr < Cp) {                                                                                        \
      _Pragma("nounroll") for (int trr = 0; trr < TRS; ++trr) {                                                \
        const int tt = bx * TRS + trr;                                                                         \
        if (tt >= a.L) break;                                                                                  \
        for (int k = kq; k < n; k += kstep) {                                                                  \
          const int mi = (k < a.L) ? k + a.L - 1 : k - a.L;                                     \
          double2* line = Gc + mi * mstride + tt * Cp;                                                         \
          *line = stage[PXM_D5_SLOT(trr, k, rr)];                                                              \
          if (zf) for (int z = R; c0 + rr + z < Cp; z += R) line[z] = double2{0.0, 0.0};                       \
        }                                                                                                      \
      }                                                                                                        \
    }                                                                                                          \
  }

#define PXM_D5_TRANSFORM(SLOT)                                            \
  d5_dft_half<R0>(x, plane, lane, q, jb, half, a, tw);                    \
  d5_exchange_sum<SLOT>(x, plane, pplane, lane, half, pcnt, epoch, sy);
#define PXM_D5_TO_STAGE                                                   \
  d5_barrier();                                                        \
  _Pragma("unroll") for (int u = 0; u < P1; ++u) {                        \
    const int j = jb + 8 * R0 * (pb + u);                                 \
    if (j < n) stage[PXM_D5_SLOT(trs, j, r)] = x[u];                      \
  }                                                                       \
  d5_barrier();

template <int R0>
__device__ __forceinline__ void px2ring_body5(const Dft5Args& a, const PxIn& in, double* __restrict__ G, int ncol, int C,
                                              int bx, int by, double2* lds5) {
  if ((by << 2) >= C) return;
  PXM_D5_GEOMETRY
  {
    int64_t ev[4];
    bool ok[4];
    double2 v[4];
    const bool act = ch < C && tv;
    const int64_t e_ring = in.ring0 + (int64_t)(tv ? t : 0) * n;
#pragma unroll
    for (int u = 0; u < 4; ++u) {
      const int j = jb + 8 * R0 * (pb + u);
      ok[u] = act && j < n;
      ev[u] = e_ring + (j < n ? j : 0);
    }
    if (ch < C) px_in_load_n<4>(in, ch, ev, ok, v);
    else {
#pragma unroll
      for (int u = 0; u < 4; ++u) v[u] = double2{0.0, 0.0};
    }
#pragma unroll
    for (int u = 0; u < 4; ++u) {
      const int j = jb + 8 * R0 * (pb + u);
      if (j < n) stage[PXM_D5_SLOT(trs, j, r)] = v[u];
    }
  }
  d5_barrier();
  double2 x[8];
#pragma unroll
  for (int p = 0; p < 8; ++p) {
    const int j = jb + 8 * R0 * p;
    x[p] = j < n ? stage[PXM_D5_SLOT(trs, j, r)] : double2{0.0, 0.0};
  }
  d5_barrier();
  PXM_D5_TRANSFORM(0)
  PXM_D5_TO_STAGE
  PXM_D5_STORE_RINGS(true)
}

#ifdef PXM_D5_TRACE
__device__ unsigned long long* g_dft_trace = nullptr;
#define PXM_D5_STAMP(K) { __builtin_amdgcn_sched_barrier(0); asm volatile("s_waitcnt vmcnt(0) lgkmcnt(0)" ::: "memory"); d5_stamp[K] = wall_clock64(); __builtin_amdgcn_sched_barrier(0); }
#else
#define PXM_D5_STAMP(K)
#endif
template <int R0, bool RING_OUT, bool N64>
__device__ __forceinline__ void ring2px_body5(const Dft5Args& a, double* __restrict__ G, int ncol, const PxOut& out, int C,
                                              int bx, int by, double2* lds5) {
  if ((by << 2) >= C) return;
#ifdef PXM_D5_TRACE
  unsigned long long d5_stamp[4] = {0, 0, 0, 0};
  const unsigned long long d5_t0 = wall_clock64();
#endif
  PXM_D5_GEOMETRY
  {
    const int rr = threadIdx.x & (R - 1), kq = threadIdx.x >> lgR, kstep = (512 >> lgR) ;
    const int mstride = a.Rp * Cp;
    const double2* Gc = reinterpret_cast<const double2*>(G) + c0 + rr;
    const bool cv = c0 + rr < Cp;
    constexpr int RU = TRS >= 4 ? 4 : (TRS >= 2 ? 2 : 1);
    constexpr int NB = TRS >= 4 ? 1 : (TRS >= 2 ? 2 : 4);
#pragma nounroll
    for (int tr0 = 0; tr0 < TRS; tr0 += RU) {
      for (int kb = kq; kb < n; kb += NB * kstep) {
        double2 v[RU][NB];
#pragma unroll
        for (int ru = 0; ru < RU; ++ru) {
          const int tt = bx * TRS + tr0 + ru;
          const bool rv = cv && tt < a.L;
#pragma unroll
          for (int u = 0; u < NB; ++u) {
            const int k = kb + u * kstep;
            v[ru][u] = double2{0.0, 0.0};
            if (rv && k < n) v[ru][u] = Gc[((k < a.L) ? k + a.L - 1 : k - a.L) * mstride + tt * Cp];
          }
        }
#pragma unroll
        for (int ru = 0; ru < RU; ++ru)
#pragma unroll
          for (int u = 0; u < NB; ++u) {
            const int k = kb + u * kstep;
            if (k < n) stage[PXM_D5_SLOT(tr0 + ru, k, rr)] = double2{v[ru][u].x, -v[ru][u].y};
          }
      }
    }
  }
  d5_barrier();
  PXM_D5_STAMP(0)
  double2 x[8];
#pragma unroll
  for (int p = 0; p < 8; ++p) {
    const int j = jb + 8 * R0 * p;
    x[p] = j < n ? stage[PXM_D5_SLOT(trs, j, r)] : double2{0.0, 0.0};
  }
  d5_barrier();
  PXM_D5_TRANSFORM(0)
  PXM_D5_STAMP(1)
  const bool act = ch < C && tv;
  const int64_t e0 = out.ring0 + (int64_t)t * n + jb + (int64_t)(8 * R0) * pb;
  const int64_t ce0 = (int64_t)ch * out.chain_stride + e0;
  if (act && out.X) {
    const uint64_t it_eff = out.iter + (out.iter_dev ? *out.iter_dev : 0);
    const int ch_s = __builtin_amdgcn_readfirstlane(ch);
#pragma unroll
    for (int g0 = 0; g0 < P1; g0 += 4) {
      double2 xs[4], wn[4];
      double Ts[4];
      int64_t eo[4];
      double2 wph[4];
#pragma unroll
      for (int u = 0; u < 4; ++u) {
        wph[u] = double2{0.0, 0.0};
        if (!out.noise) wph[u] = px_noise_philox_t<N64>(out, ch_s, e0 + (int64_t)(8 * R0) * (g0 + u), it_eff);
        __builtin_amdgcn_sched_barrier(0);
      }
#pragma unroll
      for (int u = 0; u < 4; ++u) {
        const int p = g0 + u;
        const bool ok = jb + 8 * R0 * (pb + p) < n;
        eo[u] = ok ? (int64_t)(8 * R0) * p : -(int64_t)(jb + 8 * R0 * pb);
      }
#pragma unroll
      for (int u = 0; u < 4; ++u) xs[u] = reinterpret_cast<const double2*>(out.X)[ce0 + eo[u]];
      if (out.T) {
#pragma unroll
        for (int u = 0; u < 4; ++u) Ts[u] = out.T[e0 + eo[u]];
      } else {
#pragma unroll
        for (int u = 0; u < 4; ++u) Ts[u] = out.T_scalar;
      }
      if (out.noise) {
#pragma unroll
        for (int u = 0; u < 4; ++u) wn[u] = px_noise_load(out, ch, e0 + eo[u]);
      } else {
#pragma unroll
        for (int u = 0; u < 4; ++u) wn[u] = double2{0.0, 0.0};
      }
#pragma unroll
      for (int u = 0; u < 4; ++u) {
        const int p = g0 + u;
        if (jb + 8 * R0 * (pb + p) >= n) {
          x[p] = double2{0.0, 0.0};
          continue;
        }
        const int64_t off = (int64_t)(8 * R0) * p;
        const double2 y{x[p].x, -x[p].y};
        double2 w = wn[u];
        if (!out.noise) w = wph[u];
        x[p] = px_update(out, xs[u], Ts[u], y, w);
        reinterpret_cast<double2*>(out.f)[ce0 + off] = x[p];
      }
    }
  } else if (act) {
    bool ok[P1];
    int64_t ev[P1];
    double2 yv[P1];
#pragma unroll
    for (int p = 0; p < P1; ++p) {
      ok[p] = jb + 8 * R0 * (pb + p) < n;
      ev[p] = ok[p] ? e0 + (int64_t)(8 * R0) * p : out.ring0 + (int64_t)t * n;
      yv[p] = double2{x[p].x, -x[p].y};
    }
    px_out_store_n<P1>(out, ch, ev, yv, ok);
    if (RING_OUT && out.rdata) {
      double2 rd[P1], rc[P1];
#pragma unroll
      for (int p = 0; p < P1; ++p) rd[p] = reinterpret_cast<const double2*>(out.rdata)[ev[p]];
      if (out.rinvcov_complex) {
#pragma unroll
        for (int p = 0; p < P1; ++p) rc[p] = reinterpret_cast<const double2*>(out.rinvcov)[ev[p]];
      } else {
#pragma unroll
        for (int p = 0; p < P1; ++p) rc[p] = double2{out.rinvcov[ev[p]], 0.0};
      }
#pragma unroll
      for (int p = 0; p < P1; ++p) {
        const double2 d = csub(yv[p], rd[p]);
        yv[p] = out.rinvcov_complex ? cmul(rc[p], d) : double2{rc[p].x * d.x, rc[p].x * d.y};
      }
    }
#pragma unroll
    for (int p = 0; p < P1; ++p) x[p] = ok[p] ? yv[p] : double2{0.0, 0.0};
  } else {
#pragma unroll
    for (int p = 0; p < P1; ++p) x[p] = double2{0.0, 0.0};
  }
  if (!RING_OUT) return;
  PXM_D5_STAMP(2)
  d5_exchange_fill<1>(x, plane, pplane, lane, half, pcnt, epoch, sy);
  d5_pair_sync(pcnt, epoch += 2, lane, sy);
  PXM_D5_TRANSFORM(0)
  PXM_D5_STAMP(3)
  PXM_D5_TO_STAGE
  PXM_D5_STORE_RINGS(false)
#ifdef PXM_D5_TRACE
  d5_barrier();
  if (threadIdx.x == 0 && g_dft_trace) {
    const unsigned long long slot = atomicAdd(g_dft_trace + 1, 1ull);
    unsigned long long* rr_ = g_dft_trace + 8 + 8 * 4096 + 8 * slot;
    rr_[0] = R0; rr_[1] = d5_stamp[0] - d5_t0; rr_[2] = d5_stamp[1] - d5_t0; rr_[3] = d5_stamp[2] - d5_t0;
    rr_[4] = d5_stamp[3] - d5_t0; rr_[5] = wall_clock64() - d5_t0; rr_[6] = bx; rr_[7] = by;
  }
#endif
}

}
#include "dft_pfa.h"
namespace pxm {

template <int R0>
__global__ __launch_bounds__(128 * D5_RMAX, 4) void k_px2ring5(Dft5Args a, PxIn in, double* __restrict__ G,
                                                                                 int ncol, int C) {
  extern __shared__ double2 lds5[];
  if (in.bump && blockIdx.x == 0 && blockIdx.y == 0 && threadIdx.x == 0) *in.bump += 1;
  if constexpr (R0 == 8) {
    if (a.pfa && ncol >= 8) {
      const PfaTabs pt{reinterpret_cast<const uint16_t*>(a.pfa + PFA_TAB_GAT), reinterpret_cast<const uint16_t*>(a.pfa + PFA_TAB_KIDX),
                       reinterpret_cast<const double2*>(a.pfa + PFA_TAB_B2)};
      px2ring_body_pfa(a, pt, in, G, ncol, C, blockIdx.x, blockIdx.y, 1, lds5);
      return;
    }
  }
  px2ring_body5<R0>(a, in, G, ncol, C, blockIdx.x, blockIdx.y, lds5);
}

template <int R0, bool RING_OUT, bool N64>
__global__ __launch_bounds__(128 * D5_RMAX, 4) void k_ring2px5(Dft5Args a, double* __restrict__ G, int ncol,
                                                                                 PxOut out, int C) {
  extern __shared__ double2 lds5[];
  if constexpr (R0 == 8) {
    if (a.pfa && ncol >= 8) {
      const PfaTabs pt{reinterpret_cast<const uint16_t*>(a.pfa + PFA_TAB_GAT), reinterpret_cast<const uint16_t*>(a.pfa + PFA_TAB_KIDX),
                       reinterpret_cast<const double2*>(a.pfa + PFA_TAB_B2)};
      ring2px_body_pfa<RING_OUT, N64>(a, pt, G, ncol, out, C, blockIdx.x, blockIdx.y, 1, lds5);
      return;
    }
  }
  ring2px_body5<R0, RING_OUT, N64>(a, G, ncol, out, C, blockIdx.x, blockIdx.y, lds5);
}

#define PXM_D5_GROUP_DECODE                                              \
  int e = 0;                                                             \
  while (e + 1 < nent && (int)blockIdx.x >= ents[e + 1].b0) ++e;         \
  const Dft5Group g = ents[e];                                           \
  const int local = blockIdx.x - g.b0;                                   \
  const int rest = local >> 3;                                           \
  const int by = rest % g.nby;                                           \
  int bx = (rest / g.nby) * 8 + (local & 7);                             \
   \
  if (g.xs > 1 && bx < (g.nbx & ~(8 * g.xs - 1))) {                      \
    const int q = rest / g.nby;                                          \
    bx = g.xs * (8 * (q / g.xs) + (local & 7)) + q % g.xs;               \
  }                                                                      \
  if (bx >= g.nbx) return;                                               \
  double* G = ws + g.g_off;                                              \
  Dft5Args a = g.a;                                                      \
  {                                                                      \
    const double* tb = ws + g.tbase;                                     \
    a.cE = reinterpret_cast<const double2*>(tb + g.toff[0]);             \
    a.cO = reinterpret_cast<const double2*>(tb + g.toff[1]);             \
    a.dO = reinterpret_cast<const double2*>(tb + g.toff[2]);             \
    a.tw1 = reinterpret_cast<const double2*>(tb + g.toff[3]);            \
    a.wt = reinterpret_cast<const double2*>(tb + g.toff[4]);             \
    a.bE = reinterpret_cast<const double2*>(tb + g.toff[5]);             \
    a.bO = reinterpret_cast<const double2*>(tb + g.toff[6]);             \
  }

#ifdef PXM_D5_TRACE
extern "C" int pxm_debug_set_dft_trace(unsigned long long* buf) {
  return hipMemcpyToSymbol(HIP_SYMBOL(g_dft_trace), &buf, sizeof(buf)) == hipSuccess ? 0 : -1;
}
#endif
template <bool RING_OUT, bool N64>
__global__ __launch_bounds__(128 * D5_RMAX, 4) void k_ring2px_group5(const Dft5Group* __restrict__ ents, int nent,
                                                                                       double* __restrict__ ws, int ncol, PxOut out,
                                                                                       int C) {
  extern __shared__ double2 lds5[];
#ifdef PXM_D5_TRACE
  const unsigned long long trace_t0 = wall_clock64();
#endif
  PXM_D5_GROUP_DECODE
  out.ring0 = g.ring0;
  if (g.r0 == 9) {
    const double* pb = ws + g.tbase + g.pfa_off;
    const PfaTabs pt{reinterpret_cast<const uint16_t*>(pb + PFA_TAB_GAT), reinterpret_cast<const uint16_t*>(pb + PFA_TAB_KIDX),
                     reinterpret_cast<const double2*>(pb + PFA_TAB_B2)};
    ring2px_body_pfa<RING_OUT, N64>(a, pt, G, ncol, out, C, bx, by, g.pfa_passes, lds5);
  }
  switch (g.r0) {
    case 9: break;
    case 8: ring2px_body5<8, RING_OUT, N64>(a, G, ncol, out, C, bx, by, lds5); break;
    case 4: ring2px_body5<4, RING_OUT, N64>(a, G, ncol, out, C, bx, by, lds5); break;
    case 2: ring2px_body5<2, RING_OUT, N64>(a, G, ncol, out, C, bx, by, lds5); break;
    default: ring2px_body5<1, RING_OUT, N64>(a, G, ncol, out, C, bx, by, lds5); break;
  }
#ifdef PXM_D5_TRACE
  if (threadIdx.x == 0 && g_dft_trace) {
    unsigned hw, xcc;
    asm volatile("s_getreg_b32 %0, hwreg(HW_REG_HW_ID)" : "=s"(hw));
    asm volatile("s_getreg_b32 %0, hwreg(HW_REG_XCC_ID)" : "=s"(xcc));
    const unsigned long long slot = atomicAdd(g_dft_trace, 1ull);
    unsigned long long* r = g_dft_trace + 8 + 8 * slot;
    r[0] = blockIdx.x; r[1] = gridDim.x; r[2] = trace_t0; r[3] = wall_clock64();
    r[4] = ((unsigned long long)(xcc & 0xf) << 32) | hw; r[5] = g.r0; r[6] = e; r[7] = by;
  }
#endif
}

__global__ __launch_bounds__(128 * D5_RMAX, 4) void k_px2ring_group5(const Dft5Group* __restrict__ ents, int nent,
                                                                                       double* __restrict__ ws, int ncol, PxIn in,
                                                                                       int C) {
  extern __shared__ double2 lds5[];
  if (in.bump && blockIdx.x == 0 && threadIdx.x == 0) *in.bump += 1;
  PXM_D5_GROUP_DECODE
  in.ring0 = g.ring0;
  if (g.r0 == 9) {
    const double* pb = ws + g.tbase + g.pfa_off;
    const PfaTabs pt{reinterpret_cast<const uint16_t*>(pb + PFA_TAB_GAT), reinterpret_cast<const uint16_t*>(pb + PFA_TAB_KIDX),
                     reinterpret_cast<const double2*>(pb + PFA_TAB_B2)};
    px2ring_body_pfa(a, pt, in, G, ncol, C, bx, by, g.pfa_passes, lds5);
    return;
  }
  switch (g.r0) {
    case 8: px2ring_body5<8>(a, in, G, ncol, C, bx, by, lds5); break;
    case 4: px2ring_body5<4>(a, in, G, ncol, C, bx, by, lds5); break;
    case 2: px2ring_body5<2>(a, in, G, ncol, C, bx, by, lds5); break;
    default: px2ring_body5<1>(a, in, G, ncol, C, bx, by, lds5); break;
  }
}


struct Dft6Args {
  int L, n, Rp;
  int lgR;
  const double2 *cA, *cB, *dA, *dB;
  const double2 *tw1, *wt;
  const double2* bQ;
};

#define PXM_D6_GEOMETRY                                                                      \
  constexpr int lgR = LGR, R = 1 << LGR;             \
  const int n = a.n;                                                                         \
  const int wave = threadIdx.x >> 6, lane = threadIdx.x & 63;                                \
  const int w = wave & 3, r = wave >> 2;             \
  const D5Lane q{lane & 7, lane >> 3};                                                       \
  const int t = bx, c0 = by * R, ch = c0 + r;                                                \
  const int Cp = ncol >> 1;                                                                  \
  const int rsh = 4 - lgR;                                                                   \
  const int wa = w & 1, wb = w >> 1;                                                         \
  const int pb = 4 * wa + 2 * wb;                    \
  double2* stage = lds5;                                                                     \
  double2* plane = lds5 + wave * D5_PLANE;                                                   \
  const double2* pp1 = lds5 + (wave ^ 1) * D5_PLANE;                                         \
  const double2* pp2 = lds5 + (wave ^ 2) * D5_PLANE;                                         \
  const double2* tw = lds5 + 4 * R * D5_PLANE;                                               \
  for (int i = threadIdx.x; i < D5_TW; i += 256 * R) lds5[4 * R * D5_PLANE + i] = i < 448 ? a.tw1[64 + i] : a.wt[i - 448];
#define PXM_D6_SLOT(K, CH) (((K) << lgR) + (((CH) + ((K) >> rsh)) & (R - 1)))

__device__ __forceinline__ void d6_transform(double2 (&xl)[8], const double2 (&xh)[8], double2 (&fo)[2][2], double2* plane,
                                             const double2* pp1, const double2* pp2, const double2* tw, int lane,
                                             const D5Lane& q, int w, const Dft6Args& a) {
  const int wa = w & 1, wb = w >> 1;
  const double2* __restrict__ cA = a.cA + w * 512 + lane;
  const double2* __restrict__ cB = a.cB + w * 512 + lane;
  const double2* __restrict__ dA = a.dA + w * 512 + lane;
  const double2* __restrict__ dB = a.dB + w * 512 + lane;
#pragma unroll
  for (int p = 0; p < 8; ++p) xl[p] = cadd(cmul(xl[p], cA[64 * p]), cmul(xh[p], cB[64 * p]));
  d5_conv<8>(xl, plane, lane, q, tw, a.bQ + w * 512);
  double2 su[4], sv[4];
#pragma unroll
  for (int i = 0; i < 4; ++i) {
    const double2 yk = d5_sel(wa, xl[4 + i], xl[i]), ys = d5_sel(wa, xl[i], xl[4 + i]);
    const int pk = 64 * (4 * wa + i), ps = 64 * (4 * (1 - wa) + i);
    su[i] = cmul(yk, dA[pk]);
    sv[i] = cmul(yk, dB[pk]);
    plane[64 * i + lane] = cmul(ys, dA[ps]);
    plane[256 + 64 * i + lane] = cmul(ys, dB[ps]);
  }
  d5_barrier();
#pragma unroll
  for (int i = 0; i < 4; ++i) {
    su[i] = cadd(su[i], pp1[64 * i + lane]);
    sv[i] = cadd(sv[i], pp1[256 + 64 * i + lane]);
  }
  d5_barrier();
#pragma unroll
  for (int ii = 0; ii < 2; ++ii) {
    plane[64 * ii + lane] = d5_sel(wb, su[ii], su[2 + ii]);
    plane[128 + 64 * ii + lane] = d5_sel(wb, sv[ii], sv[2 + ii]);
  }
  d5_barrier();
#pragma unroll
  for (int ii = 0; ii < 2; ++ii) {
    fo[ii][0] = cadd(d5_sel(wb, su[2 + ii], su[ii]), pp2[64 * ii + lane]);
    fo[ii][1] = cadd(d5_sel(wb, sv[2 + ii], sv[ii]), pp2[128 + 64 * ii + lane]);
  }
}

__device__ __forceinline__ int d6_ring_of_block(int b, int nb) {
  if (b >= (nb & ~63)) return b;
  const int x = b & 7, q = b >> 3;
  return ((((q >> 3) << 3) + x) << 3) + (q & 7);
}

template <int LGR>
__global__ __launch_bounds__(256 << LGR, 4) void k_px2ring6(Dft6Args a, PxIn in, double* __restrict__ G, int ncol, int C) {
  extern __shared__ double2 lds5[];
  if (in.bump && blockIdx.x == 0 && blockIdx.y == 0 && threadIdx.x == 0) *in.bump += 1;
  const int bx = d6_ring_of_block(blockIdx.x, gridDim.x), by = blockIdx.y;
  if ((by << LGR) >= C) return;
  PXM_D6_GEOMETRY
  {
    int64_t ev[4];
    bool ok[4];
    double2 v[4];
#pragma unroll
    for (int u = 0; u < 4; ++u) {
      const int j = lane + 64 * (2 * w + (u >> 1)) + 512 * (u & 1);
      ok[u] = ch < C && j < n;
      ev[u] = in.ring0 + (int64_t)t * n + (j < n ? j : 0);
    }
    if (ch < C) px_in_load_n<4>(in, ch, ev, ok, v);
    else {
#pragma unroll
      for (int u = 0; u < 4; ++u) v[u] = double2{0.0, 0.0};
    }
#pragma unroll
    for (int u = 0; u < 4; ++u) {
      const int j = lane + 64 * (2 * w + (u >> 1)) + 512 * (u & 1);
      if (j < n) stage[PXM_D6_SLOT(j, r)] = v[u];
    }
  }
  d5_barrier();
  double2 xl[8], xh[8];
#pragma unroll
  for (int p = 0; p < 8; ++p) {
    const int j = lane + 64 * p;
    xl[p] = stage[PXM_D6_SLOT(j, r)];
    xh[p] = (j + 512 < n) ? stage[PXM_D6_SLOT(j + 512, r)] : double2{0.0, 0.0};
  }
  d5_barrier();
  double2 fo[2][2];
  d6_transform(xl, xh, fo, plane, pp1, pp2, tw, lane, q, w, a);
  d5_barrier();
#pragma unroll
  for (int ii = 0; ii < 2; ++ii)
// ... 59 lines not shown
  const uint64_t it_eff = out.iter + (out.iter_dev ? *out.iter_dev : 0);
  const int64_t e0 = out.ring0 + (int64_t)t * n + lane + 64 * pb;
  const int64_t ce0 = (int64_t)ch * out.chain_stride + e0;
  bool ok[4];
  int64_t eo[4];
  double2 yv[4];
#pragma unroll
  for (int u = 0; u < 4; ++u) {
    const int ii = u >> 1, hq = u & 1;
    ok[u] = lane + 64 * (pb + ii) + 512 * hq < n;
    eo[u] = ok[u] ? 64 * ii + 512 * hq : 0;
    yv[u] = double2{fo[ii][hq].x, -fo[ii][hq].y};
  }
  if (out.X) {
    double2 xs[4], wn[4];
    double Ts[4];
#pragma unroll
    for (int u = 0; u < 4; ++u) xs[u] = reinterpret_cast<const double2*>(out.X)[ce0 + eo[u]];
    if (out.T) {
#pragma unroll
      for (int u = 0; u < 4; ++u) Ts[u] = out.T[e0 + eo[u]];
    } else {
#pragma unroll
      for (int u = 0; u < 4; ++u) Ts[u] = out.T_scalar;
    }
    if (out.noise) {
#pragma unroll
      for (int u = 0; u < 4; ++u) wn[u] = px_noise_load(out, ch, e0 + eo[u]);
    }
#pragma unroll
    for (int u = 0; u < 4; ++u) {
      if (!ok[u]) continue;
      const double2 wv = out.noise ? wn[u] : px_noise_philox_t<N64>(out, ch, e0 + eo[u], it_eff);
      reinterpret_cast<double2*>(out.f)[ce0 + eo[u]] = px_update(out, xs[u], Ts[u], yv[u], wv);
    }
  } else {
    int64_t ev[4];
#pragma unroll
    for (int u = 0; u < 4; ++u) ev[u] = e0 + eo[u];
    px_out_store_n<4>(out, ch, ev, yv, ok);
  }
}

int pair_r0(int n) {
  if (n > 512) return 0;
  int Mh = 64;
  while (Mh < n) Mh <<= 1;
  return Mh / 64;
}

void pfa511_host_tables(uint16_t* idx, double* b2) {
  typedef std::complex<long double> cld;
  const long double PI_L = 3.141592653589793238462643383279502884L;
  const int n = PFA_N, N2 = 73, g = 5;
  auto ang = [&](long double num, long double den) { return cld(cosl(-PI_L * num / den), sinl(-PI_L * num / den)); };
  auto powm = [&](long long b, int e) { long long r_ = 1; for (int i = 0; i < e; ++i) r_ = r_ * b % N2; return (int)r_; };
  const int ginv = powm(g, 71);
  auto crt72 = [](int q8, int q9) { return (9 * q8 + 64 * q9) % 72; };
  std::fill(idx, idx + (size_t)(64 + 80) * 8, (uint16_t)0);
  for (int l = 0; l < 63; ++l)
    for (int q8 = 0; q8 < 8; ++q8) idx[(size_t)l * 8 + q8] = (uint16_t)(16 * ((73 * (l / 9) + 7 * powm(ginv, crt72(q8, l % 9))) % n));
  for (int inst = 0; inst < 73; ++inst) {
    const int k2 = inst < 72 ? powm(g, crt72(inst / 9, inst % 9)) : 0;
    for (int k1 = 0; k1 < 7; ++k1) idx[(size_t)(64 + inst) * 8 + k1] = (uint16_t)(16 * ((365 * k1 + 147 * k2) % n));
  }
  for (int k8 = 0; k8 < 8; ++k8)
    for (int k9 = 0; k9 < 9; ++k9) {
      cld acc(0, 0);
      for (int q8 = 0; q8 < 8; ++q8)
        for (int q9 = 0; q9 < 9; ++q9)
          acc += ang(2.0L * powm(g, crt72(q8, q9)), N2) * ang(2.0L * ((q8 * k8) % 8), 8) * ang(2.0L * ((q9 * k9) % 9), 9);
      acc /= 72.0L;
      b2[2 * (k8 * 9 + k9)] = (double)acc.real();
      b2[2 * (k8 * 9 + k9) + 1] = (double)acc.imag();
    }
}

int pair_make_tables(int n, bool pfa, PairTables* t) {
  typedef std::complex<long double> cld;
  const long double PI_L = 3.141592653589793238462643383279502884L;
  const int r0 = pair_r0(n), Mh = 64 * r0, M = 2 * Mh;
  auto ang = [&](long double num, long double den) { return cld(cosl(-PI_L * num / den), sinl(-PI_L * num / den)); };
  std::vector<cld> chirp, bhat;
  bluestein_chirp_spectrum(n, M, true, chirp, bhat);
  std::vector<double> h;
  auto put = [&](const cld& v) {
    h.push_back((double)v.real());
    h.push_back((double)v.imag());
  };
  const cld zero(0, 0);
  const size_t o_cE = 0;
  for (int j = 0; j < Mh; ++j) put(j < n ? chirp[j] : zero);
  const size_t o_cO = h.size();
  for (int j = 0; j < Mh; ++j) put(j < n ? chirp[j] * ang(2.0L * j, M) : zero);
  const size_t o_dO = h.size();
  for (int j = 0; j < Mh; ++j) put(j < n ? chirp[j] * std::conj(ang(2.0L * j, M)) : zero);
  const size_t o_tw1 = h.size();
  for (int k = 0; k < 8; ++k)
    for (int lane = 0; lane < 64; ++lane) {
      const int lam = ((lane & 7) % r0) + r0 * (lane >> 3);
      put(ang(2.0L * ((lam * k) % Mh), Mh));
    }
  const size_t o_wt = h.size();
  for (int a = 0; a < 8; ++a)
    for (int b = 0; b < 8; ++b) put(ang(2.0L * ((a * b) % (8 * r0)), 8 * r0));
  size_t o_b[2];
  for (int w = 0; w < 2; ++w) {
    o_b[w] = h.size();
    for (int k0 = 0; k0 < r0; ++k0)
      for (int lane = 0; lane < 64; ++lane) put(bhat[2 * ((lane >> 3) + 8 * (lane & 7) + 64 * k0) + w]);
  }
  size_t o_pfa = 0;
  if (n == PFA_N && pfa) {
    o_pfa = h.size();
    h.resize(h.size() + PFA_TAB_DOUBLES);
    pfa511_host_tables(reinterpret_cast<uint16_t*>(h.data() + o_pfa + PFA_TAB_GAT), h.data() + o_pfa + PFA_TAB_B2);
  }
  t->pfa_off = (int)o_pfa;
  if (int rc = dev_table(&t->d_all, h, "phi-DFT tables (8 points per lane)")) return rc;
  t->r0 = r0;
  t->cE = t->d_all + o_cE;
  t->cO = t->d_all + o_cO;
  t->dO = t->d_all + o_dO;
  t->tw1 = t->d_all + o_tw1;
  t->wt = t->d_all + o_wt;
  t->bE = t->d_all + o_b[0];
  t->bO = t->d_all + o_b[1];
  return 0;
}

constexpr size_t D5_LDS = (size_t)2 * D5_RMAX * D5_PLANE * 16 + (size_t)D5_TW * 16;
static_assert((size_t)512 * D5_RMAX * 16 <= (size_t)2 * D5_RMAX * D5_PLANE * 16, "the stage of a ring set fits in the planes");
static_assert(((size_t)8 * PFA_PLANE + 72 + NOISE_LOG_N + 256 + 1) * 16 <= D5_LDS, "PFA workgroup LDS");

void pair_workgroup(int n, bool pfa, int* rings, int* threads, size_t* lds, bool* exact) {
  *exact = n == PFA_N && pfa;
  *rings = *exact ? 2 : 8 / pair_r0(n);
  *threads = 128 * D5_RMAX;
  *lds = D5_LDS;
}

static Dft5Args pair_args(const DftPlan& p) {
  const PairTables& t = p.pair;
  auto c = [](const double* x) { return reinterpret_cast<const double2*>(x); };
  return Dft5Args{p.L, p.n, p.Rp, 2 , c(t.cE), c(t.cO), c(t.dO), c(t.tw1), c(t.wt), c(t.bE), c(t.bO),
                  p.d_status, p.spin_limit, t.pfa_off ? t.d_all + t.pfa_off : nullptr};
}

template <int R0>
static int pair_attr() {
  static std::atomic<uint64_t> done{0};
  return allow_dynamic_lds(done, {reinterpret_cast<const void*>(k_px2ring5<R0>), reinterpret_cast<const void*>(k_ring2px5<R0, false, false>),
                                  reinterpret_cast<const void*>(k_ring2px5<R0, true, false>), reinterpret_cast<const void*>(k_ring2px5<R0, false, true>),
                                  reinterpret_cast<const void*>(k_ring2px5<R0, true, true>)});
}

template <int R0>
static int pair_ring_blocks(const Dft5Args& a, int ncol) {
  const int rings = (R0 == 8 && a.pfa && ncol >= 8) ? 2 : 8 / R0;
  return (a.L + rings - 1) / rings;
}

template <int R0>
static int pair_px2ring_r(const DftPlan& p, const PxIn& in, double* G, int ncol, int C, hipStream_t st) {
  if (int rc = pair_attr<R0>()) return rc;
  const Dft5Args da = pair_args(p);
  dim3 grid(pair_ring_blocks<R0>(da, ncol), (ncol / 2 + D5_RMAX - 1) / D5_RMAX), block(128 * D5_RMAX);
  hipLaunchKernelGGL((k_px2ring5<R0>), grid, block, D5_LDS, st, da, in, G, ncol, C);
  PXM_HIP(hipGetLastError());
  return 0;
}

template <int R0>
static int pair_ring2px_r(const DftPlan& p, const double* G, int ncol, const PxOut& out, int C, hipStream_t st, bool ring_out) {
  if (int rc = pair_attr<R0>()) return rc;
  const Dft5Args da = pair_args(p);
  dim3 grid(pair_ring_blocks<R0>(da, ncol), (C + D5_RMAX - 1) / D5_RMAX), block(128 * D5_RMAX);
  double* Gw = const_cast<double*>(G);
  const bool n64 = out.X && !out.noise && out.noise64;
  if (ring_out) {
    if (n64) hipLaunchKernelGGL((k_ring2px5<R0, true, true>), grid, block, D5_LDS, st, da, Gw, ncol, out, C);
    else hipLaunchKernelGGL((k_ring2px5<R0, true, false>), grid, block, D5_LDS, st, da, Gw, ncol, out, C);
  } else {
    if (n64) hipLaunchKernelGGL((k_ring2px5<R0, false, true>), grid, block, D5_LDS, st, da, Gw, ncol, out, C);
    else hipLaunchKernelGGL((k_ring2px5<R0, false, false>), grid, block, D5_LDS, st, da, Gw, ncol, out, C);
  }
  PXM_HIP(hipGetLastError());
  return 0;
}

#define PXM_D5_DISPATCH(FN, ...)         \
  switch (p.pair.r0) {                   \
    case 8: return FN<8>(__VA_ARGS__);   \
    case 4: return FN<4>(__VA_ARGS__);   \
    case 2: return FN<2>(__VA_ARGS__);   \
    default: return FN<1>(__VA_ARGS__);  \
  }

int pair_px2ring(const DftPlan& p, const PxIn& in, double* G, int ncol, int C, hipStream_t st) {
  PXM_D5_DISPATCH(pair_px2ring_r, p, in, G, ncol, C, st)
}
int pair_ring2px(const DftPlan& p, const double* G, int ncol, const PxOut& out, int C, hipStream_t st, bool ring_out) {
  PXM_D5_DISPATCH(pair_ring2px_r, p, G, ncol, out, C, st, ring_out)
}

int dft_group_create(const std::vector<const DftPlan*>& plans, const std::vector<int64_t>& g_off,
                     const std::vector<int64_t>& ring0, int ncol, const double* ws_base, DftGroupList* out) {
  std::vector<int> order;
  for (size_t i = 0; i < plans.size(); ++i)
    if (plans[i]->unit == DFT_PAIR) order.push_back((int)i);
  std::stable_sort(order.begin(), order.end(), [&](int x, int y) { return plans[x]->L > plans[y]->L; });
  if (order.size() < 2) return 1;
  std::vector<Dft5Group> v;
  out->member.assign(plans.size(), 0);
  int b0 = 0;
  std::string why;
  int64_t nchk = 0;
  for (int s : order) {
    const DftPlan& p = *plans[s];
    const PairTables& t = p.pair;
    const std::string entry = "DFT group entry " + std::to_string(v.size());
    Dft5Group g;
    g.a = pair_args(p);
    g.g_off = g_off[s];
    g.ring0 = ring0[s];
    g.r0 = t.r0;
    g.tbase = t.d_all - ws_base;
    const double* tp[7] = {t.cE, t.cO, t.dO, t.tw1, t.wt, t.bE, t.bO};
    for (int k = 0; k < 7; ++k) g.toff[k] = (int)(tp[k] - t.d_all);
    const int rings = 8 / t.r0;
    g.nbx = (p.L + rings - 1) / rings;
    g.nby = (ncol / 2 + D5_RMAX - 1) / D5_RMAX;
    {
      const int per_line = 16 / ncol;
      g.xs = (g.nby == 1 && per_line > rings && per_line % rings == 0) ? per_line / rings : 1;
    }
    g.pfa_off = 0;
    g.pfa_passes = 1;
    if (t.pfa_off && ncol >= 8) {
      ++out->n_pfa;
      g.r0 = 9;
      g.pfa_off = t.pfa_off;
      g.pfa_passes = (getenv("PXM_PFA_PASSES") && atoi(getenv("PXM_PFA_PASSES")) == 1) ? 1 : 2;
      g.nbx = ((p.L + 1) / 2 + g.pfa_passes - 1) / g.pfa_passes;
      g.xs = 1;
    }
    g.b0 = b0;
    b0 += round_up(g.nbx, 8) * g.nby;
    out->px_elems += (double)p.L * p.n;
    out->member[s] = 1;
    v.push_back(g);

    const int64_t ring_doubles = (int64_t)(2 * p.L - 1) * p.Rp * ncol;
    ++nchk;
    if (!dev_range_ok(ws_base + g.g_off, ws_base + g.g_off + ring_doubles, &why)) {
      set_error(entry + ": ring array outside its buffer: " + why);
      return -1;
    }
    const int Mh = 64 * t.r0;
    const int64_t tsize[7] = {2 * Mh, 2 * Mh, 2 * Mh, 2 * 8 * 64, 2 * 64, 2 * t.r0 * 64, 2 * t.r0 * 64};
    for (int k = 0; k < 7; ++k) {
      ++nchk;
      const double* tb = ws_base + g.tbase + g.toff[k];
      if (!dev_range_ok(tb, tb + tsize[k], &why)) {
        set_error(entry + ": table view " + std::to_string(k) + " outside its buffer: " + why);
        return -1;
      }
    }
    out->ring_end = std::max(out->ring_end, g.ring0 + (int64_t)p.L * p.n);
    if (g.r0 == 9) {
      ++nchk;
      const double* tb = ws_base + g.tbase + g.pfa_off;
      if (!dev_range_ok(tb, tb + PFA_TAB_DOUBLES, &why)) {
        set_error(entry + ": PFA table block outside its buffer: " + why);
        return -1;
      }
    }
  }
  ranges_checked_add(nchk);
  out->n = (int)v.size();
  out->all = v.size() == plans.size();
  out->blocks = b0;
  if (int rc = dev_table(&out->d, v, "DFT group entries")) return rc;
  static std::atomic<uint64_t> lds_done{0};
  return allow_dynamic_lds(lds_done, {reinterpret_cast<const void*>(k_ring2px_group5<true, false>), reinterpret_cast<const void*>(k_ring2px_group5<true, true>),
                                      reinterpret_cast<const void*>(k_ring2px_group5<false, false>), reinterpret_cast<const void*>(k_ring2px_group5<false, true>),
                                      reinterpret_cast<const void*>(k_px2ring_group5)});
}

void dft_group_destroy(DftGroupList* g) {
  if (g->d) deferred_free(g->d);
  g->d = nullptr;
  g->n_pfa = 0;
  g->n = 0;
}

int dft_group_launch(const DftGroupList& g, double* ws, int ncol, const PxOut& out, int C, hipStream_t st, Profiler* prof) {
  PXM_REQUIRE(g.ring_end <= out.chain_stride, "dft_group_launch: a scale's coefficient block ends past chain_stride");
  const double bytes = g.px_elems * (2.0 * 16 * (ncol / 2) + 2.0 * 16 * C + (out.T ? 8.0 : 0.0));
  hipEvent_t ev0 = nullptr, ev1 = nullptr;
  if (prof) prof->next(prof->dft, &ev0, &ev1, bytes, 0.0);
  const Dft5Group* ents = reinterpret_cast<const Dft5Group*>(g.d);
  if (out.X && !out.noise && out.noise64)
    hipExtLaunchKernelGGL((k_ring2px_group5<true, true>), dim3(g.blocks), dim3(128 * D5_RMAX), D5_LDS, st, ev0, ev1, 0,
                          ents, g.n, ws, ncol, out, C);
  else
    hipExtLaunchKernelGGL((k_ring2px_group5<true, false>), dim3(g.blocks), dim3(128 * D5_RMAX), D5_LDS, st, ev0, ev1, 0,
                          ents, g.n, ws, ncol, out, C);
  PXM_HIP(hipGetLastError());
  return 0;
}

int dft_group_px2ring(const DftGroupList& g, double* ws, int ncol, const PxIn& in, int C, hipStream_t st) {
  PXM_REQUIRE(in.gidx || g.ring_end <= in.chain_stride, "dft_group_px2ring: a scale's coefficient block ends past chain_stride");
  hipLaunchKernelGGL(k_px2ring_group5, dim3(g.blocks), dim3(128 * D5_RMAX), D5_LDS, st, reinterpret_cast<const Dft5Group*>(g.d),
                     g.n, ws, ncol, in, C);
  PXM_HIP(hipGetLastError());
  return 0;
}

int dft_group_ring2px(const DftGroupList& g, double* ws, int ncol, const PxOut& out, int C, hipStream_t st) {
  PXM_REQUIRE(out.gidx || g.ring_end <= out.chain_stride, "dft_group_ring2px: a scale's coefficient block ends past chain_stride");
  const Dft5Group* ents = reinterpret_cast<const Dft5Group*>(g.d);
  if (out.X && !out.noise && out.noise64)
    hipLaunchKernelGGL((k_ring2px_group5<false, true>), dim3(g.blocks), dim3(128 * D5_RMAX), D5_LDS, st, ents, g.n, ws, ncol, out, C);
  else
    hipLaunchKernelGGL((k_ring2px_group5<false, false>), dim3(g.blocks), dim3(128 * D5_RMAX), D5_LDS, st, ents, g.n, ws, ncol, out, C);
  PXM_HIP(hipGetLastError());
  return 0;
}

int quad_make_tables(int n, QuadTables* t) {
  typedef std::complex<long double> cld;
  const long double PI_L = 3.141592653589793238462643383279502884L;
  const int M = 2048;
  auto ang = [&](long double num, long double den) { return cld(cosl(-PI_L * num / den), sinl(-PI_L * num / den)); };
  std::vector<cld> chirp, bhat;
  bluestein_chirp_spectrum(n, M, true, chirp, bhat);
  chirp.resize(1024, cld(0, 0));
  std::vector<double> h;
  auto put = [&](const cld& v) {
    h.push_back((double)v.real());
    h.push_back((double)v.imag());
  };
  const cld mi(0, -1), pi(0, 1);
  auto ipow = [](cld b, int e) { cld r(1, 0); for (int i = 0; i < e; ++i) r *= b; return r; };
  size_t o[4];
  for (int tab = 0; tab < 4; ++tab) {
    o[tab] = h.size();
    for (int w = 0; w < 4; ++w)
      for (int j = 0; j < 512; ++j) {
        const cld W = ang(2.0L * ((j * w) % M), M);
        if (tab == 0) put(chirp[j] * W);
        else if (tab == 1) put(ipow(mi, w) * chirp[j + 512] * W);
        else if (tab == 2) put(chirp[j] * std::conj(W));
        else put(ipow(pi, w) * chirp[j + 512] * std::conj(W));
      }
  }
  const size_t o_tw1 = h.size();
  for (int k = 0; k < 8; ++k)
    for (int lane = 0; lane < 64; ++lane) put(ang(2.0L * ((lane * k) % 512), 512));
  const size_t o_wt = h.size();
  for (int x = 0; x < 8; ++x)
    for (int y = 0; y < 8; ++y) put(ang(2.0L * ((x * y) % 64), 64));
  const size_t o_bq = h.size();
  for (int w = 0; w < 4; ++w)
    for (int k0 = 0; k0 < 8; ++k0)
      for (int lane = 0; lane < 64; ++lane) put(bhat[4 * ((lane >> 3) + 8 * (lane & 7) + 64 * k0) + w]);
  if (int rc = dev_table(&t->d_all, h, "phi-DFT tables (four waves per ring)")) return rc;
  t->cA = t->d_all + o[0];
  t->cB = t->d_all + o[1];
  t->dA = t->d_all + o[2];
  t->dB = t->d_all + o[3];
  t->tw1 = t->d_all + o_tw1;
  t->wt = t->d_all + o_wt;
  t->bQ = t->d_all + o_bq;
  return 0;
}

static Dft6Args quad_args(const DftPlan& p) {
  const QuadTables& t = p.quad;
  auto c = [](const double* x) { return reinterpret_cast<const double2*>(x); };
  return Dft6Args{p.L, p.n, p.Rp, 1, c(t.cA), c(t.cB), c(t.dA), c(t.dB), c(t.tw1), c(t.wt), c(t.bQ)};
}
static size_t quad_lds(int R) { return (size_t)4 * R * D5_PLANE * 16 + (size_t)D5_TW * 16; }
static int quad_attr() {
  static std::atomic<uint64_t> done{0};
  return allow_dynamic_lds(done, {reinterpret_cast<const void*>(k_px2ring6<0>), reinterpret_cast<const void*>(k_px2ring6<1>),
                                  reinterpret_cast<const void*>(k_ring2px6<false, 0>), reinterpret_cast<const void*>(k_ring2px6<true, 0>),
                                  reinterpret_cast<const void*>(k_ring2px6<false, 1>), reinterpret_cast<const void*>(k_ring2px6<true, 1>)});
}
static int quad_chains_per_wg(int C) { return C == 1 ? 1 : 2; }
void quad_workgroup(int* chains, int* threads, size_t* lds) {
  *chains = quad_chains_per_wg(2);
  *threads = 256 * *chains;
  *lds = quad_lds(*chains);
}
int quad_px2ring(const DftPlan& p, const PxIn& in, double* G, int ncol, int C, hipStream_t st) {
  if (int rc = quad_attr()) return rc;
  const int R = quad_chains_per_wg(C);
  dim3 grid(p.L, (ncol / 2 + R - 1) / R), block(256 * R);
  if (R == 1) hipLaunchKernelGGL(k_px2ring6<0>, grid, block, quad_lds(R), st, quad_args(p), in, G, ncol, C);
  else hipLaunchKernelGGL(k_px2ring6<1>, grid, block, quad_lds(R), st, quad_args(p), in, G, ncol, C);
  PXM_HIP(hipGetLastError());
  return 0;
}
int quad_ring2px(const DftPlan& p, const double* G, int ncol, const PxOut& out, int C, hipStream_t st) {
  if (int rc = quad_attr()) return rc;
  const int R = quad_chains_per_wg(C);
  dim3 grid(p.L, (C + R - 1) / R), block(256 * R);
  const bool n64 = out.X && !out.noise && out.noise64;
  const Dft6Args a = quad_args(p);
  if (R == 1) {
    if (n64) hipLaunchKernelGGL((k_ring2px6<true, 0>), grid, block, quad_lds(R), st, a, G, ncol, out, C);
    else hipLaunchKernelGGL((k_ring2px6<false, 0>), grid, block, quad_lds(R), st, a, G, ncol, out, C);
  } else {
    if (n64) hipLaunchKernelGGL((k_ring2px6<true, 1>), grid, block, quad_lds(R), st, a, G, ncol, out, C);
    else hipLaunchKernelGGL((k_ring2px6<false, 1>), grid, block, quad_lds(R), st, a, G, ncol, out, C);
  }
  PXM_HIP(hipGetLastError());
  return 0;
}

}
```

pxmcmc_amd/csrc/elem.h:

```cpp
#pragma once
#include <hip/hip_runtime.h>

#include "philox.h"

namespace pxm {

__device__ inline double2 cmul(double2 a, double2 b) { return double2{a.x * b.x - a.y * b.y, a.x * b.y + a.y * b.x}; }
__device__ inline double2 cmulc(double2 a, double2 b) {
  return double2{a.x * b.x + a.y * b.y, a.y * b.x - a.x * b.y};
}
__device__ inline double2 cadd(double2 a, double2 b) { return double2{a.x + b.x, a.y + b.y}; }
__device__ inline double2 csub(double2 a, double2 b) { return double2{a.x - b.x, a.y - b.y}; }

__device__ inline double soft_real(double x, double T) {
  const double a = fabs(x);
  if (a <= T) return 0.0;
  return copysign(a - T, x);
}
__device__ inline double2 soft_cplx(double2 z, double T) {
  const double a = sqrt(fma(z.x, z.x, z.y * z.y));
  if (a <= T) return double2{0.0, 0.0};
  const double s = (a - T) / a;
  return double2{z.x * s, z.y * s};
}

__device__ inline double chain_step_real(double X, double px, double g, double w, double delta, double lmda) {
  const double r = delta / lmda;
  return (1 - r) * X + r * px - delta * g + sqrt(2 * delta) * w;
}
__device__ inline double2 chain_step_cplx(double2 X, double2 px, double2 g, double2 w, double delta, double lmda) {
  return double2{chain_step_real(X.x, px.x, g.x, w.x, delta, lmda), chain_step_real(X.y, px.y, g.y, w.y, delta, lmda)};
}

__device__ __forceinline__ double abs2_plain(double x, double y) {
#pragma clang fp contract(off)
  return x * x + y * y;
}

struct NoiseSrc {
  const double* noise;
  int noise_complex;
  uint64_t seed, chain0, iter;
  const uint64_t* iter_dev = nullptr;
  int f64 = 0;
};
constexpr int NOISE_F64_FLAG = 16;
static inline NoiseSrc make_noise_src(const void* noise, int noise_arg, uint64_t seed, uint64_t chain0, uint64_t iter,
                                      const uint64_t* iter_dev = nullptr) {
  return NoiseSrc{(const double*)noise, noise_arg & 1, seed, chain0, iter, iter_dev, (noise_arg & NOISE_F64_FLAG) ? 1 : 0};
}

template <bool CPLX>
__device__ inline double2 draw_noise(const NoiseSrc& ns, int c, int64_t n, int64_t i) {
  if (ns.noise) {
    if (CPLX && ns.noise_complex) return reinterpret_cast<const double2*>(ns.noise)[(int64_t)c * n + i];
    return double2{ns.noise[(int64_t)c * n + i], 0.0};
  }
  const uint64_t it = ns.iter + (ns.iter_dev ? *ns.iter_dev : 0);
  if (CPLX && ns.noise_complex) {
    NormalPair q = philox_normal_pair(ns.seed, ns.chain0 + c, (uint64_t)i, it, ns.f64);
    return double2{q.z0, q.z1};
  }
  return double2{philox_normal_real(ns.seed, ns.chain0 + c, (uint64_t)i, it, ns.f64), 0.0};
}

}
```

pxmcmc_amd/csrc/philox.h:

```cpp
#pragma once
#include <hip/hip_runtime.h>

#include <cstdint>

#include "noise_tables.h"

namespace pxm {

struct NormalPair {
  double z0, z1;
};

__host__ __device__ inline void philox4x32_10(uint32_t c[4], uint32_t k0, uint32_t k1) {
#pragma unroll
  for (int r = 0; r < 10; ++r) {
    const uint64_t p0 = (uint64_t)0xD2511F53u * c[0];
    const uint64_t p1 = (uint64_t)0xCD9E8D57u * c[2];
#if defined(__HIP_DEVICE_COMPILE__) && defined(__gfx950__) && __has_builtin(__builtin_amdgcn_bitop3_b32)
    const uint32_t n0 = __builtin_amdgcn_bitop3_b32((uint32_t)(p1 >> 32), c[1], k0, 0x96);
    const uint32_t n2 = __builtin_amdgcn_bitop3_b32((uint32_t)(p0 >> 32), c[3], k1, 0x96);
#else
    const uint32_t n0 = (uint32_t)(p1 >> 32) ^ c[1] ^ k0;
    const uint32_t n2 = (uint32_t)(p0 >> 32) ^ c[3] ^ k1;
#endif
    const uint32_t n1 = (uint32_t)p1;
    const uint32_t n3 = (uint32_t)p0;
    c[0] = n0;
    c[1] = n1;
    c[2] = n2;
    c[3] = n3;
    k0 += 0x9E3779B9u;
    k1 += 0xBB67AE85u;
  }
}

__device__ inline NormalPair box_muller_fast(double u1, double u2) {
  const int ex = __builtin_amdgcn_frexp_exp(u1);
  const float mant = (float)__builtin_amdgcn_frexp_mant(u1);
  const float log2u = (float)ex + __builtin_amdgcn_logf(mant);
  const float r = __builtin_amdgcn_sqrtf(-1.3862943611198906f * log2u);
  const float turns = (float)u2;
  return NormalPair{(double)(r * __builtin_amdgcn_cosf(turns)), (double)(r * __builtin_amdgcn_sinf(turns))};
}

__device__ inline NormalPair box_muller_f64_poly(double u1, double u2) {
  int ex = __builtin_amdgcn_frexp_exp(u1);
  double m = __builtin_amdgcn_frexp_mant(u1);
  const bool lo = m < 0.70710678118654752440;
  m = lo ? 2.0 * m : m;
  ex = lo ? ex - 1 : ex;
  const double num = m - 1.0, den = m + 1.0;
  double rc = __builtin_amdgcn_rcp(den);
  rc = fma(fma(-den, rc, 1.0), rc, rc);
  double s = num * rc;
  s = fma(fma(-den, s, num), rc, s);
  const double z = s * s;
  double p = 1.0 / 19.0;
  p = fma(p, z, 1.0 / 17.0);
  p = fma(p, z, 1.0 / 15.0);
  p = fma(p, z, 1.0 / 13.0);
  p = fma(p, z, 1.0 / 11.0);
  p = fma(p, z, 1.0 / 9.0);
  p = fma(p, z, 1.0 / 7.0);
  p = fma(p, z, 1.0 / 5.0);
  p = fma(p, z, 1.0 / 3.0);
  p = fma(p, z, 1.0);
  const double e = (double)ex;
  double x = fma(e, -2.0 * 0.693147180369123816490, fma(-4.0 * s, p, e * (-2.0 * 1.90821492927058770002e-10)));
  x = fmax(x, 1e-300);
  double h = __builtin_amdgcn_rsq(x);
  double g = x * h;
  h *= 0.5;
  const double r = fma(-h, g, 0.5);
  g = fma(g, r, g);
  g = fma(fma(-g, g, x), h, g);
  const double t = 4.0 * u2;
  const double k = __builtin_rint(t);
  const double a = (t - k) * 1.57079632679489661923;
  const double a2 = a * a;
  double ps = 1.0 / 355687428096000.0, pc = 1.0 / 20922789888000.0;
  ps = fma(ps, a2, -1.0 / 1307674368000.0);  pc = fma(pc, a2, -1.0 / 87178291200.0);
  ps = fma(ps, a2, 1.0 / 6227020800.0);      pc = fma(pc, a2, 1.0 / 479001600.0);
  ps = fma(ps, a2, -1.0 / 39916800.0);       pc = fma(pc, a2, -1.0 / 3628800.0);
  ps = fma(ps, a2, 1.0 / 362880.0);          pc = fma(pc, a2, 1.0 / 40320.0);
  ps = fma(ps, a2, -1.0 / 5040.0);           pc = fma(pc, a2, -1.0 / 720.0);
  ps = fma(ps, a2, 1.0 / 120.0);             pc = fma(pc, a2, 1.0 / 24.0);
  ps = fma(ps, a2, -1.0 / 6.0);              pc = fma(pc, a2, -0.5);
  const double sn = fma(ps * a2, a, a), cs = fma(pc, a2, 1.0);
  const int q = (int)k;
  const bool odd = q & 1;
  const double ss = odd ? cs : sn, cc = odd ? sn : cs;
  const double S = (q & 2) ? -ss : ss, C = ((q + 1) & 2) ? -cc : cc;
  return NormalPair{g * C, g * S};
}

__device__ inline NormalPair box_muller_f64_tab(double u1, double u2, const double2* logt, const double2* sct) {
  const int ex = __builtin_amdgcn_frexp_exp(u1);
  const double m = __builtin_amdgcn_frexp_mant(u1);
  const int j = min(max((int)__builtin_rint(m * 256.0), NOISE_LOG_J0), 256);
  const double2 lt = logt[j - NOISE_LOG_J0];
  const double r = fma(m, lt.x, -1.0);
  double p = 1.0 / 7.0;
  p = fma(p, r, -1.0 / 6.0);
  p = fma(p, r, 1.0 / 5.0);
  p = fma(p, r, -0.25);
  p = fma(p, r, 1.0 / 3.0);
  p = fma(p, r, -0.5);
  p = fma(p, r, 1.0);
  p *= r;
  const double e = (double)ex;
  double x = fma(-2.0, p, fma(e, -2.0 * 0.693147180369123816490, fma(e, -2.0 * 1.90821492927058770002e-10, lt.y)));
  x = fmax(x, 1e-300);
  double h = __builtin_amdgcn_rsq(x);
  double g = x * h;
  h *= 0.5;
  const double rr = fma(-h, g, 0.5);
  g = fma(g, rr, g);
  g = fma(fma(-g, g, x), h, g);
  const double t = 256.0 * u2;
  const double k = __builtin_rint(t);
  const double a = (t - k) * 0.024543692606170259675;
  const double2 cs = sct[(int)k & 255];
  const double a2 = a * a;
  const double q = fma(fma(a2, -1.0 / 5040.0, 1.0 / 120.0), a2, -1.0 / 6.0);
  const double sa = fma(a * a2, q, a);
  const double cm1 = fma(fma(a2, -1.0 / 720.0, 1.0 / 24.0), a2, -0.5) * a2;
  const double C = cs.x + fma(-cs.y, sa, cs.x * cm1);
  const double S = cs.y + fma(cs.x, sa, cs.y * cm1);
  return NormalPair{g * C, g * S};
}
__device__ inline NormalPair box_muller_f64_tab(double u1, double u2) {
  return box_muller_f64_tab(u1, u2, reinterpret_cast<const double2*>(&NOISE_LOG_TAB[0][0]), reinterpret_cast<const double2*>(&NOISE_SINCOS_TAB[0][0]));
}
__device__ inline NormalPair box_muller_f64(double u1, double u2) {
#ifdef PXM_NOISE_F64_POLY
  return box_muller_f64_poly(u1, u2);
#else
  return box_muller_f64_tab(u1, u2);
#endif
}

template <bool F64>
__device__ inline NormalPair philox_normal_pair_t(uint64_t seed, uint64_t chain, uint64_t index, uint64_t iter) {
  const uint64_t key = seed + chain * 0x9E3779B97F4A7C15ull;
  uint32_t c[4] = {(uint32_t)index, (uint32_t)(index >> 32), (uint32_t)iter, (uint32_t)(iter >> 32)};
  philox4x32_10(c, (uint32_t)key, (uint32_t)(key >> 32));
  const uint64_t a = (((uint64_t)c[1] << 32) | c[0]) >> 11;
  const uint64_t b = (((uint64_t)c[3] << 32) | c[2]) >> 11;
  const double u1 = ((double)a + 0.5) * 0x1.0p-53;
  const double u2 = ((double)b + 0.5) * 0x1.0p-53;
  if (F64) return box_muller_f64(u1, u2);
  return box_muller_fast(u1, u2);
}
__device__ inline uint4 philox_bits(uint64_t seed, uint64_t chain, uint64_t index, uint64_t iter) {
  const uint64_t key = seed + chain * 0x9E3779B97F4A7C15ull;
  uint32_t c[4] = {(uint32_t)index, (uint32_t)(index >> 32), (uint32_t)iter, (uint32_t)(iter >> 32)};
  philox4x32_10(c, (uint32_t)key, (uint32_t)(key >> 32));
  return uint4{c[0], c[1], c[2], c[3]};
}
__device__ inline NormalPair normal_pair_from_bits_tabs(const uint4 c, const double2* logt, const double2* sct) {
  const uint64_t a = (((uint64_t)c.y << 32) | c.x) >> 11;
  const uint64_t b = (((uint64_t)c.w << 32) | c.z) >> 11;
  return box_muller_f64_tab(((double)a + 0.5) * 0x1.0p-53, ((double)b + 0.5) * 0x1.0p-53, logt, sct);
}
__device__ inline NormalPair philox_normal_pair_tabs(uint64_t seed, uint64_t chain, uint64_t index, uint64_t iter, const double2* logt,
                                                     const double2* sct) {
  const uint64_t key = seed + chain * 0x9E3779B97F4A7C15ull;
  uint32_t c[4] = {(uint32_t)index, (uint32_t)(index >> 32), (uint32_t)iter, (uint32_t)(iter >> 32)};
  philox4x32_10(c, (uint32_t)key, (uint32_t)(key >> 32));
  const uint64_t a = (((uint64_t)c[1] << 32) | c[0]) >> 11;
  const uint64_t b = (((uint64_t)c[3] << 32) | c[2]) >> 11;
  return box_muller_f64_tab(((double)a + 0.5) * 0x1.0p-53, ((double)b + 0.5) * 0x1.0p-53, logt, sct);
}
__device__ inline NormalPair philox_normal_pair(uint64_t seed, uint64_t chain, uint64_t index, uint64_t iter, bool f64 = false) {
  return f64 ? philox_normal_pair_t<true>(seed, chain, index, iter) : philox_normal_pair_t<false>(seed, chain, index, iter);
}

constexpr uint64_t PXM_PAIR_TWEAK = 0xD1B54A32D192ED03ull;
template <bool F64>
__device__ inline NormalPair philox_normal_chainpair_t(uint64_t seed, uint64_t pair, uint64_t e, uint64_t iter) {
  return philox_normal_pair_t<F64>(seed + PXM_PAIR_TWEAK, pair, e, iter);
}
__device__ inline NormalPair philox_normal_chainpair(uint64_t seed, uint64_t pair, uint64_t e, uint64_t iter, bool f64 = false) {
  return philox_normal_pair(seed + PXM_PAIR_TWEAK, pair, e, iter, f64);
}
__device__ inline double philox_normal_real(uint64_t seed, uint64_t chain, uint64_t e, uint64_t iter, bool f64 = false) {
  const NormalPair p = philox_normal_chainpair(seed, chain >> 1, e, iter, f64);
  return (chain & 1) ? p.z1 : p.z0;
}

__device__ inline double philox_uniform(uint64_t seed, uint64_t chain, uint64_t iter) {
  const uint64_t key = seed + chain * 0x9E3779B97F4A7C15ull;
  const uint64_t index = 0x8000000000000000ull;
  uint32_t c[4] = {(uint32_t)index, (uint32_t)(index >> 32), (uint32_t)iter, (uint32_t)(iter >> 32)};
  philox4x32_10(c, (uint32_t)key, (uint32_t)(key >> 32));
  const uint64_t a = (((uint64_t)c[1] << 32) | c[0]) >> 11;
  return ((double)a + 0.5) * 0x1.0p-53;
}

}
```

pxmcmc_amd/csrc/sht_core.h:

```cpp
#pragma once
#include "common.h"
#include "profiler.h"

namespace pxm {

constexpr int GEMM_TASK_ROW_TILES = 8;

struct GemmTask {
  int64_t tab_off;
  int64_t rt_stride;
  int64_t x_off[4];
  int64_t y_off[4];
  int64_t x2_off[4];
  int64_t hd_off[4];
  int64_t ks_off[2];
  int64_t rs_off[2];
  int row_lo[2], row_hi[2];
  int k_beg, k_end;
  int row0;
  int n_rt;
  int nslab;
  double sign1;
  int m_unit;
  int hd_stride;
  int x_ncol, y_ncol;
  int pole_n;
  int pole_dx;
  int64_t pole_b_off;
  int64_t pole_bo_off;
};

struct GemmAffine {
  double ns = 0, wr = 0, wi = 0;
  int on = 0;
  int ncol_live = 1 << 30;
  uint64_t* bump = nullptr;
};

constexpr int GEMM_TASK_FIXED_STEPS = 32;

enum GemmListFlag {
  GEMM_LIST_TWO = 1,
  GEMM_LIST_SCALE = 2,
  GEMM_LIST_POLE = 4,
};

constexpr int GEMM_GROUP_COLS = 32;
inline int gemm_group_tiles(int ncol, int col0) { return (ncol - col0 >= GEMM_GROUP_COLS) ? 2 : 1; }

int launch_gemm_packed(const GemmTask* d_tasks, int n_tasks, int pk, int flags, const double* X, double* Y, int ncol, int col0,
                       double alg_bytes, double flops, hipStream_t stream, Profiler* prof = nullptr);

int launch_gemm(const GemmTask* d_tasks, int n_tasks, int nslab, int flags, const double* X, double* Y, int ncol,
                int col0, int ct, double alg_bytes, double flops, hipStream_t stream,
                const GemmAffine& aff = GemmAffine(), Profiler* prof = nullptr);

inline double gemm_table_bytes(int L, bool paired, int el_lo = 0) {
  double tab_entries = 0;
  for (int m = paired ? 0 : -(L - 1); m < L; ++m) {
    const int am = m < 0 ? -m : m;
    const int n = L - (am > el_lo ? am : el_lo);
    if (n > 0) tab_entries += n;
  }
  return 8.0 * L * tab_entries;
}
inline double gemm_alg_bytes(int L, bool paired, int C, int el_lo = 0) {
  double tab_entries = 0, lm_entries = 0;
  for (int m = paired ? 0 : -(L - 1); m < L; ++m) {
    const int am = m < 0 ? -m : m;
    const int n = L - (am > el_lo ? am : el_lo);
    if (n > 0) tab_entries += n;
  }
  for (int m = -(L - 1); m < L; ++m) {
    const int am = m < 0 ? -m : m;
    const int n = L - (am > el_lo ? am : el_lo);
    if (n > 0) lm_entries += n;
  }
  return 8.0 * L * tab_entries + 16.0 * C * (lm_entries + (double)L * (2 * L - 1));
}

int check_gemm_task_ranges(const std::vector<GemmTask>& v, int nslab, int pk, int flags, int ncol, const double* ws_base,
                           const char* list_name);

enum DftUnit { DFT_RADIX2, DFT_PAIR, DFT_QUAD };

struct PairTables {
  double* d_all = nullptr;
  int r0 = 0;
  int pfa_off = 0;
  const double *cE = nullptr, *cO = nullptr, *dO = nullptr, *tw1 = nullptr, *wt = nullptr, *bE = nullptr, *bO = nullptr;
};

struct QuadTables {
  double* d_all = nullptr;
  const double *cA = nullptr, *cB = nullptr, *dA = nullptr, *dB = nullptr, *tw1 = nullptr, *wt = nullptr, *bQ = nullptr;
};

struct DftPlan {
  int L = 0, n = 0, Rp = 0;
  DftUnit unit = DFT_RADIX2;
  int M = 0, logM = 0, R = 0, threads = 0;
  size_t lds = 0;
  double *d_chirp = nullptr, *d_bhat = nullptr, *d_tw = nullptr;
  PairTables pair;
  QuadTables quad;
  unsigned* d_status = nullptr;
  unsigned spin_limit = 1u << 18;
};
enum { PXM_STATUS_PAIR_SYNC_BIT = 2 };

struct DftGeometry {
  DftUnit unit = DFT_RADIX2;
  int M = 0;
  int per_wg = 0;
  int threads = 0;
  size_t lds = 0;
  bool exact = false;
  bool pfa = true;
};
constexpr size_t DFT_LDS_MAX = 160 * 1024;
int dft_geometry(int L, DftGeometry* g);

int make_dft_plan(int L, DftPlan* p);
void free_dft_plan(DftPlan* p);

struct PxIn {
  const double* f = nullptr;
  int64_t chain_stride = 0;
  int64_t ring0 = 0;
  const double* data = nullptr;
  const double* invcov = nullptr;
  int invcov_complex = 0;
  uint64_t* bump = nullptr;
  const int32_t* gidx = nullptr;
  const double* gw = nullptr;
};
struct PxOut {
  double* f = nullptr;
  int64_t chain_stride = 0;
  int64_t ring0 = 0;
  const double* X = nullptr;
  const double* T = nullptr;
  double T_scalar = 0, delta = 0, lmda = 0;
  const double* noise = nullptr;
  int mode = 0;
  int noise64 = 0;
  uint64_t seed = 0, chain0 = 0, iter = 0;
  const uint64_t* iter_dev = nullptr;
  const double* rdata = nullptr;
  const double* rinvcov = nullptr;
  int rinvcov_complex = 0;
  const int32_t* gidx = nullptr;
  const double* gw = nullptr;
};

struct DftGroupList {
  void* d = nullptr;
  int n = 0, blocks = 0;
  int n_pfa = 0;
  double px_elems = 0;
  int64_t ring_end = 0;
  std::vector<char> member;
  bool all = false;
};
int dft_group_create(const std::vector<const DftPlan*>& plans, const std::vector<int64_t>& g_off,
                     const std::vector<int64_t>& ring0, int ncol, const double* ws_base,
                     DftGroupList* out);
void dft_group_destroy(DftGroupList* g);
int dft_group_launch(const DftGroupList& g, double* ws, int ncol, const PxOut& out, int C, hipStream_t st,
                     Profiler* prof = nullptr);
int dft_group_px2ring(const DftGroupList& g, double* ws, int ncol, const PxIn& in, int C, hipStream_t st);
int dft_group_ring2px(const DftGroupList& g, double* ws, int ncol, const PxOut& out, int C, hipStream_t st);

int launch_px2ring(const DftPlan& p, const PxIn& in, double* G, int ncol, int C, hipStream_t stream);
int launch_ring2px(const DftPlan& p, const double* G, int ncol, const PxOut& out, int C, hipStream_t stream);
int launch_ring2px2ring(const DftPlan& p, double* G, int ncol, const PxOut& out, int C, hipStream_t stream);
inline bool dft_can_fuse(const DftPlan& p) { return p.unit == DFT_PAIR; }

int launch_lm_to_mel(const double* flm, double* H, int L, int Rp, int ncol, int C, int spin, hipStream_t stream);
int launch_mel_to_lm(const double* H, double* flm, int L, int Rp, int ncol, int C, int spin, hipStream_t stream);

}
```

pxmcmc_amd/csrc/update.h:

```cpp
#pragma once
#include "elem.h"
#include "sht_core.h"

namespace pxm {

enum { PXM_MODE_REAL_NOISE = 0, PXM_MODE_CPLX_NOISE = 1, PXM_MODE_REAL_PAIRS = 2 };

__device__ __forceinline__ double2 px_in_load(const PxIn& in, int ch, int64_t e) {
  int64_t src = e;
  if (in.gidx) {
    const int idx = in.gidx[e];
    if (idx < 0) return double2{0.0, 0.0};
    src = idx;
  }
  double2 v = reinterpret_cast<const double2*>(in.f)[(int64_t)ch * in.chain_stride + src];
  if (in.data) {
    v = csub(v, reinterpret_cast<const double2*>(in.data)[src]);
    if (in.invcov_complex) v = cmul(reinterpret_cast<const double2*>(in.invcov)[src], v);
    else {
      const double w = in.invcov[src];
      v = double2{w * v.x, w * v.y};
    }
  }
  if (in.gw) {
// ... 11 lines not shown
    int idx[N];
#pragma unroll
    for (int u = 0; u < N; ++u) idx[u] = in.gidx[e[u]];
#pragma unroll
    for (int u = 0; u < N; ++u) {
      live[u] = ok[u] && idx[u] >= 0;
      src[u] = idx[u] < 0 ? 0 : idx[u];
    }
  } else {
#pragma unroll
    for (int u = 0; u < N; ++u) {
      live[u] = ok[u];
      src[u] = e[u];
    }
  }
  const double2* f = reinterpret_cast<const double2*>(in.f) + (int64_t)ch * in.chain_stride;
#pragma unroll
  for (int u = 0; u < N; ++u) v[u] = f[src[u]];
  if (in.data) {
    double2 d[N], c[N];
#pragma unroll
    for (int u = 0; u < N; ++u) d[u] = reinterpret_cast<const double2*>(in.data)[src[u]];
    if (in.invcov_complex) {
#pragma unroll
      for (int u = 0; u < N; ++u) c[u] = reinterpret_cast<const double2*>(in.invcov)[src[u]];
#pragma unroll
      for (int u = 0; u < N; ++u) v[u] = cmul(c[u], csub(v[u], d[u]));
    } else {
#pragma unroll
      for (int u = 0; u < N; ++u) c[u].x = in.invcov[src[u]];
#pragma unroll
      for (int u = 0; u < N; ++u) {
        const double2 r = csub(v[u], d[u]);
        v[u] = double2{c[u].x * r.x, c[u].x * r.y};
      }
    }
  }
  if (in.gw) {
    double w[N];
#pragma unroll
    for (int u = 0; u < N; ++u) w[u] = in.gw[src[u]];
#pragma unroll
    for (int u = 0; u < N; ++u) v[u] = double2{w[u] * v[u].x, w[u] * v[u].y};
  }
#pragma unroll
  for (int u = 0; u < N; ++u)
    if (!live[u]) v[u] = double2{0.0, 0.0};
}

__device__ __forceinline__ void px_out_store(const PxOut& out, int ch, int64_t e, double2 y) {
  if (out.gidx) {
    const int idx = out.gidx[e];
    if (idx < 0) return;
    if (out.gw) {
      const double w = out.gw[idx];
      y = double2{w * y.x, w * y.y};
    }
    reinterpret_cast<double2*>(out.f)[(int64_t)ch * out.chain_stride + idx] = y;
    return;
  }
  reinterpret_cast<double2*>(out.f)[(int64_t)ch * out.chain_stride + e] = y;
}

template <int N>
__device__ __forceinline__ void px_out_store_n(const PxOut& out, int ch, const int64_t (&e)[N], const double2 (&y)[N], const bool (&ok)[N]) {
  double2* f = reinterpret_cast<double2*>(out.f) + (int64_t)ch * out.chain_stride;
  if (out.gidx) {
    int idx[N];
    double w[N];
#pragma unroll
    for (int u = 0; u < N; ++u) idx[u] = out.gidx[e[u]];
    if (out.gw) {
#pragma unroll
      for (int u = 0; u < N; ++u) w[u] = out.gw[idx[u] < 0 ? 0 : idx[u]];
    } else {
#pragma unroll
      for (int u = 0; u < N; ++u) w[u] = 1.0;
    }
#pragma unroll
    for (int u = 0; u < N; ++u)
      if (ok[u] && idx[u] >= 0) f[idx[u]] = double2{w[u] * y[u].x, w[u] * y[u].y};
    return;
  }
#pragma unroll
  for (int u = 0; u < N; ++u)
    if (ok[u]) f[e[u]] = y[u];
}

__device__ __forceinline__ double2 px_noise_load(const PxOut& o, int c, int64_t e) {
  if (o.mode == PXM_MODE_CPLX_NOISE) return reinterpret_cast<const double2*>(o.noise)[(int64_t)c * o.chain_stride + e];
  if (o.mode == PXM_MODE_REAL_PAIRS)
    return double2{o.noise[(int64_t)(2 * c) * o.chain_stride + e], o.noise[(int64_t)(2 * c + 1) * o.chain_stride + e]};
  return double2{o.noise[(int64_t)c * o.chain_stride + e], 0.0};
}

template <bool F64>
__device__ __forceinline__ double2 px_noise_philox_t(const PxOut& o, int c, int64_t e, uint64_t it) {
  const bool pairs = o.mode == PXM_MODE_REAL_PAIRS, cplx = o.mode == PXM_MODE_CPLX_NOISE;
  if (pairs && !(o.chain0 & 1)) {
    const NormalPair q = philox_normal_chainpair_t<F64>(o.seed, (o.chain0 >> 1) + c, (uint64_t)e, it);
    return double2{q.z0, q.z1};
  }
  const int nk = pairs ? 2 : 1;
  double2 w{0.0, 0.0};
#pragma nounroll
  for (int k = 0; k < nk; ++k) {
    const uint64_t chain = o.chain0 + (pairs ? 2 * c + k : c);
    const NormalPair q = cplx ? philox_normal_pair_t<F64>(o.seed, chain, (uint64_t)e, it)
                              : philox_normal_chainpair_t<F64>(o.seed, chain >> 1, (uint64_t)e, it);
    const double v = (cplx || !(chain & 1)) ? q.z0 : q.z1;
    if (k == 0) {
      w.x = v;
      w.y = cplx ? q.z1 : 0.0;
    } else {
      w.y = v;
    }
  }
  return w;
}
__device__ __forceinline__ double2 px_noise_philox_tabs(const PxOut& o, int c, int64_t e, uint64_t it, const double2* logt, const double2* sct) {
  const bool pairs = o.mode == PXM_MODE_REAL_PAIRS, cplx = o.mode == PXM_MODE_CPLX_NOISE;
  if (pairs && !(o.chain0 & 1)) {
    const NormalPair q = philox_normal_pair_tabs(o.seed + PXM_PAIR_TWEAK, (o.chain0 >> 1) + c, (uint64_t)e, it, logt, sct);
    return double2{q.z0, q.z1};
  }
  const int nk = pairs ? 2 : 1;
  double2 w{0.0, 0.0};
#pragma nounroll
  for (int k = 0; k < nk; ++k) {
    const uint64_t chain = o.chain0 + (pairs ? 2 * c + k : c);
    const NormalPair q = cplx ? philox_normal_pair_tabs(o.seed, chain, (uint64_t)e, it, logt, sct)
                              : philox_normal_pair_tabs(o.seed + PXM_PAIR_TWEAK, chain >> 1, (uint64_t)e, it, logt, sct);
    const double v = (cplx || !(chain & 1)) ? q.z0 : q.z1;
    if (k == 0) {
      w.x = v;
      w.y = cplx ? q.z1 : 0.0;
    } else {
      w.y = v;
    }
  }
  return w;
}
__device__ __forceinline__ double2 px_noise_philox(const PxOut& o, int c, int64_t e, uint64_t it) {
  return o.noise64 ? px_noise_philox_t<true>(o, c, e, it) : px_noise_philox_t<false>(o, c, e, it);
}

__device__ __forceinline__ double2 px_update(const PxOut& o, double2 x, double T, double2 g, double2 w) {
  double2 px;
  if (o.mode == PXM_MODE_REAL_PAIRS) px = double2{soft_real(x.x, T), soft_real(x.y, T)};
  else px = soft_cplx(x, T);
  return chain_step_cplx(x, px, g, w, o.delta, o.lmda);
}

}
```

pxmcmc_amd/csrc/wav_plan.hip:

```cpp
#include "wav_plan.h"

#include <cmath>
#include <memory>
#include <mutex>

using namespace pxm;

struct SideOverride {
  const int64_t* g = nullptr;
  int g_ncol = 0;
  const WlAttach* h = nullptr;
};
static GemmSide wav_side(const pxm_wav_plan_s* p, int s, int which, const SideOverride& ov = SideOverride()) {
  const int L = p->L, b = p->bl[s], Rb = round_up(b, 16);
  const int64_t G = ov.g ? *ov.g : p->offG[s];
  GemmSide g;
  const bool ring_is_x = which == 0 || which == 3;
  if (ov.g && ov.g_ncol) (ring_is_x ? g.x_ncol : g.y_ncol) = ov.g_ncol;
  if (ov.h) (ring_is_x ? g.y_ncol : g.x_ncol) = ov.h->ncol_h;
  g.el_lo = p->el_lo_s[s];
  g.fuse = GemmFuse();
  g.kscale = nullptr;
  const int cls = (s == 0) ? 1 : ((s - 1) & 1);
  const int64_t hcls = ov.h ? (cls ? ov.h->offHBn : ov.h->offHAn) : (cls ? p->offHB : p->offHA);
// ... 162 lines not shown
  if ((rc = upload_tasks(v_adj_fwdadj, true, &p->adj_fwdadj, p->bl, p->ncol, p->ws, "synthesis-adjoint forward-adjoint (all scales)", el_lo, pk, shared))) return rc;
  if ((rc = upload_tasks(v_ana_inv, true, &p->ana_inv, p->bl, p->ncol, p->ws, "analysis inverse (all scales)", el_lo))) return rc;
  if ((rc = upload_tasks(v_anadj_invadj, true, &p->anadj_invadj, p->bl, p->ncol, p->ws, "analysis-adjoint inverse-adjoint (all scales)", el_lo))) return rc;
  GemmFuse sum2;
  sum2.x2_base = p->offHB;
  if ((rc = wav_level_list(p, TAB_INV, p->offHA, p->offGL, sum2, &p->syn_inv, "synthesis inverse at L"))) return rc;
  if ((rc = wav_level_list(p, TAB_INV_ADJ, p->offGL, p->offHL, GemmFuse(), &p->adj_invadj, "inverse-adjoint at L"))) return rc;
  if ((rc = wav_level_list(p, TAB_FWD, p->offGL, p->offHL, GemmFuse(), &p->ana_fwd, "analysis forward at L"))) return rc;
  if ((rc = wav_level_list(p, TAB_FWD_ADJ, p->offHA, p->offGL, sum2, &p->anadj_fwdadj, "analysis-adjoint forward-adjoint at L"))) return rc;
  p->lane_of.assign(p->nsc, -1);
  SidePool* sp = nullptr;
  if ((rc = side_pool(&sp))) return rc;
  for (int i = 0; i < p->nside; ++i) {
    p->side[i] = sp->side[i];
    p->ev_join[i] = sp->ev_join[i];
  }
  p->ev_fork = sp->ev_fork;
  int k = 0;
  for (int s = p->nsc - 1; s >= 0; --s)
    if (p->bl[s] < L) p->lane_of[s] = (k++) % p->nside;
  std::vector<const DftPlan*> dp;
  for (int s = 0; s < p->nsc; ++s) dp.push_back(&p->dft[s]);
  if ((rc = dft_group_create(dp, p->offG, p->coef_off, p->ncol, p->ws, &p->dft_group)) < 0) return rc;
  *plan = guard.release();
  return 0;
}

int pxm::wav_make_gram_lists(pxm_wav_plan_s* p) {
  if (p->gram.d) return 0;
  int rc;
  const char* split_env = getenv("PXM_GRAM_SPLIT");
  const int split = split_env ? atoi(split_env) : 2;
  const int kind = (!gram_can_split(*p->TL) || split == 0) ? TAB_GRAM : (split == 1 ? TAB_GRAM_SPLIT : TAB_GRAM_SPLIT0);
  if ((rc = get_tables(p->L, p->spin, 1u << kind, &p->TL))) return rc;
  wav_hold(p, p->TL);
  std::vector<GemmTask> v;
  GemmFuse fz;
  fz.x2_base = p->offHB;
  fz.hd_base = p->offHDc;
  fz.hd_stride = 2;
  append_gemm_tasks(*p->TL, kind, p->ncol, GemmSide{p->offHA, p->offHL, p->L, p->Rp, p->L, p->Rp, nullptr, 0, fz}, p->offS, p->ws, v);
  if ((rc = upload_tasks(v, p->TL->paired, &p->gram, {p->L}, p->ncol, p->ws, "Gram step"))) return rc;
  tasklist_set_gram(&p->gram, *p->TL, kind);
  return wav_level_list(p, TAB_INV_ADJ, p->offGD, p->offHD, GemmFuse(), &p->adj_invadj_D, "inverse-adjoint of the data rings");
}

namespace pxm {
__global__ void k_iter_add(uint64_t* c, uint64_t inc) { *c += inc; }

__global__ void k_count_nonfinite(const double* __restrict__ x, int64_t n, unsigned long long* cnt) {
  unsigned long long c = 0;
  for (int64_t i = blockIdx.x * (int64_t)blockDim.x + threadIdx.x; i < n; i += (int64_t)gridDim.x * blockDim.x)
    if (!isfinite(x[i])) ++c;
  if (c) atomicAdd(cnt, c);
}
}

extern "C" {

int pxm_wav_plan_create(int L, double B, int J_min, int max_chains, unsigned flags, pxm_wav_plan_t* plan) {
  (void)flags;
  return wav_plan_create_impl("pxm_wav_plan_create", L, B, J_min, 0, max_chains, plan);
}

int pxm_wav_plan_create_spin(int L, double B, int J_min, int spin, int max_chains, unsigned flags, pxm_wav_plan_t* plan) {
  (void)flags;
  return wav_plan_create_impl("pxm_wav_plan_create_spin", L, B, J_min, spin, max_chains, plan);
}

int pxm_wav_plan_destroy(pxm_wav_plan_t p) {
  if (!p) return 0;
  dft_group_destroy(&p->dft_group);
  for (auto& d : p->dft) free_dft_plan(&d);
  free_dft_plan(&p->dftL);
  deferred_free(p->ws);
  deferred_free(p->d_kc_syn);
  deferred_free(p->d_kc_ana);
  deferred_free(p->d_status);
  TaskList* tls[] = {&p->syn_fwd, &p->syn_inv, &p->adj_invadj, &p->adj_fwdadj, &p->gram, &p->adj_invadj_D,
                     &p->ana_fwd, &p->ana_inv, &p->anadj_invadj, &p->anadj_fwdadj};
  for (TaskList* t : tls) free_tasks(t);
  profiler_release(&p->prof);
  for (ShtTables* T : p->held) release_tables(T);
  wl_release(p->wl);
  delete p;
  drain_deferred();
  return 0;
}

int pxm_wav_set_iter_counter(pxm_wav_plan_t p, uint64_t* counter_dev) {
  PXM_REQUIRE(p, "pxm_wav_set_iter_counter: null plan");
  PXM_REQUIRE(!counter_dev || !p->iter_dev || p->iter_dev == counter_dev,
              "pxm_wav_set_iter_counter: this plan already has a live iteration counter (one stepping engine per plan "
              "at a time; release the first with pxm_wav_release_iter_counter)");
  p->iter_dev = counter_dev;
  return 0;
}

int pxm_wav_release_iter_counter(pxm_wav_plan_t p, const uint64_t* counter_dev) {
  PXM_REQUIRE(p, "pxm_wav_release_iter_counter: null plan");
  if (p->iter_dev == counter_dev) p->iter_dev = nullptr;
  return 0;
}

int pxm_wav_iter_counter_add(pxm_wav_plan_t p, uint64_t inc, pxm_stream_t stream) {
  PXM_REQUIRE(p && p->iter_dev, "pxm_wav_iter_counter_add: no counter registered on this plan");
  hipLaunchKernelGGL(k_iter_add, dim3(1), dim3(1), 0, (hipStream_t)stream, p->iter_dev, inc);
  PXM_HIP(hipGetLastError());
  return 0;
}

int pxm_wav_profile_enable(pxm_wav_plan_t p, int max_launches) {
  PXM_REQUIRE(p, "pxm_wav_profile_enable: null plan");
  return profiler_enable(&p->prof, max_launches);
}
int pxm_wav_profile_read(pxm_wav_plan_t p, double* gemm_ms, int64_t* gemm_launches, double* gemm_alg_bytes,
                         double* gemm_flops) {
  PXM_REQUIRE(p, "pxm_wav_profile_read: null plan");
  return profiler_read(&p->prof.gemm, gemm_ms, gemm_launches, gemm_alg_bytes, gemm_flops);
}
int pxm_wav_profile_read_launches(pxm_wav_plan_t p, double* launch_ms, double* launch_alg_bytes,
                                  int32_t* launch_workgroups, int64_t cap, int64_t* launches) {
  PXM_REQUIRE(p && launch_ms && launch_alg_bytes && cap >= 0, "pxm_wav_profile_read_launches: bad arguments");
  return profiler_read(&p->prof.gemm, nullptr, launches, nullptr, nullptr, launch_ms, launch_alg_bytes, cap, launch_workgroups);
}
int pxm_wav_profile_read_dft(pxm_wav_plan_t p, double* dft_ms, int64_t* dft_launches, double* dft_alg_bytes) {
  PXM_REQUIRE(p, "pxm_wav_profile_read_dft: null plan");
  return profiler_read(&p->prof.dft, dft_ms, dft_launches, dft_alg_bytes, nullptr);
}

int64_t pxm_wav_workspace_nonfinite(pxm_wav_plan_t p, pxm_stream_t stream) {
  PXM_REQUIRE(p, "pxm_wav_workspace_nonfinite: null plan");
  hipStream_t st = (hipStream_t)stream;
  unsigned long long* cnt = reinterpret_cast<unsigned long long*>(p->ws + p->offS);
  PXM_HIP(hipMemsetAsync(cnt, 0, sizeof(*cnt), st));
  hipLaunchKernelGGL(k_count_nonfinite, dim3(1024), dim3(256), 0, st, p->ws, p->offS, cnt);
  PXM_HIP(hipGetLastError());
  unsigned long long h = 0;
  PXM_HIP(hipMemcpyAsync(&h, cnt, sizeof(h), hipMemcpyDeviceToHost, st));
  PXM_HIP(hipStreamSynchronize(st));
  PXM_HIP(hipMemsetAsync(cnt, 0, sizeof(*cnt), st));
  return (int64_t)h;
}

int pxm_wav_status(pxm_wav_plan_t p, int clear, pxm_stream_t stream) {
  PXM_REQUIRE(p, "pxm_wav_status: null plan");
  return status_read(p->d_status, (hipStream_t)stream, clear);
}
int pxm_wav_exact_dft_scales(pxm_wav_plan_t p) {
  PXM_REQUIRE(p, "pxm_wav_exact_dft_scales: null plan");
  return p->dft_group.d ? p->dft_group.n_pfa : 0;
}

int64_t pxm_wav_table_bytes(pxm_wav_plan_t p, int op) {
  if (!p || op < 0 || op > 1) return -1;
  return p->table_bytes[op];
}

int pxm_tables_trim(void) {
  const int64_t freed = tables_trim();
  return (int)std::min<int64_t>(freed >> 20, 1 << 30);
}

int64_t pxm_host_check_address_ranges(int L, double B, int J_min, int spin, int max_chains, int what) {
  static std::mutex mu;
  std::lock_guard<std::mutex> lock(mu);
  PXM_REQUIRE(!capture_in_progress(), "pxm_host_check_address_ranges: not during a stream capture");
  set_dry_run(true);
  ranges_checked_reset();
  int rc = 0;
  if (what & 1) {
    pxm_sht_plan_t sp = nullptr;
    rc = pxm_sht_plan_create(L, spin, max_chains, 0, &sp);
    if (sp) pxm_sht_plan_destroy(sp);
  }
  if (!rc && (what & 2)) {
    pxm_wav_plan_t wp = nullptr;
    const int wspin = (what & 8) ? spin : 0;
    rc = pxm_wav_plan_create_spin(L, B, J_min, wspin, max_chains, 0, &wp);
    if (!rc) rc = wav_make_gram_lists(wp);
    if (!rc && (what & 4) && L >= 3 && wspin == 0) rc = pxm_wav_wl_attach(wp, nullptr, nullptr, (int64_t)L * (2 * L - 1));
    if (wp) pxm_wav_plan_destroy(wp);
  }
  if (!rc && (what & 16)) {
    pxm_dft_plan_t dp = nullptr;
    rc = pxm_dft_plan_create(L, max_chains, &dp);
    if (dp) pxm_dft_plan_destroy(dp);
  }
  tables_trim();
  set_dry_run(false);
  return rc ? -1 : ranges_checked();
}

int64_t pxm_host_gram_table_bytes(int L, double B, int J_min, int spin, int max_chains) {
  static std::mutex mu;
  std::lock_guard<std::mutex> lock(mu);
  PXM_REQUIRE(!capture_in_progress(), "pxm_host_gram_table_bytes: not during a stream capture");
  set_dry_run(true);
  pxm_wav_plan_t wp = nullptr;
  int rc = pxm_wav_plan_create_spin(L, B, J_min, spin, max_chains, 0, &wp);
  if (!rc) rc = wav_make_gram_lists(wp);
  const int64_t bytes = rc ? -1 : (int64_t)wp->gram.gram_table_bytes;
  if (wp) pxm_wav_plan_destroy(wp);
  tables_trim();
  set_dry_run(false);
  return bytes;
}

}
```

pxmcmc_amd/ops/__init__.py:

```python
from .._lib import (FISTA_SLICES_MAX, LCI_EMPTY, LCI_NONFINITE, LCI_POINTS, LCI_UNCONSTRAINED, SAPG_GROUPS_MAX, SAPG_SLICES_MAX,
                    PxmError, check, require_gpu)
from ._args import GEMM_KINDS, _batched, _p, _stream, as_device, device
from .host import (DFT_UNITS, GEMM_TASK_FIELDS, dft_geometry, gemm_plan_geometry, gemm_report, j_max, mw_ring_weights, noise_bits, rec_geometry, tiling_axisym,
                   wav_bandlimits)
from .lci import lci_data_terms, lci_eval, lci_scratch, lci_search
from .plans import (DftPlan, DirWavPlan, GemmPlan, HarmWavPlan, IterCounter, ShtPlan, WavPlan, _Plan, capture_scope, live_plans, raise_on_status,
                    tables_trim)
from .pxmala import logtransition, pxmala_accept, pxmala_finish, pxmala_propose, pxmala_propose_scratch
from .reduce import quantile_range, reduce_l1, reduce_l2, reduce_scratch_doubles, reduce_vdot
from .sparse import CsrMatrix
from .steps import (box_muller, chain_step, counter_add, fista_restart_scratch, fista_scratch, fista_step, fista_step_restart,
                    myula_step, randn, residual_grad, sapg_group_bounds, sapg_groups_scratch, sapg_scratch, sapg_step,
                    sapg_step_groups, select_copy_many, skrock_stage, soft)
from .summary import (acov_ess, acov_stage_depth, acov_update, moments_finalize, moments_update, tails_quantiles,
                      tails_stage_depth, tails_update)
```

pxmcmc_amd/ops/host.py:

```python
import ctypes as C

import numpy as np

from .._lib import check, lib


def j_max(L, B):
    return int(check(lib.pxm_j_max(int(L), float(B))))


def wav_bandlimits(L, B, J_min):
    buf = (C.c_int * 64)()
    n = check(lib.pxm_wav_bandlimits(int(L), float(B), int(J_min), buf, 64))
    return [int(buf[i]) for i in range(n)]


def tiling_axisym(L, B, J_min):
    J = j_max(L, B)
    k0 = np.zeros(L)
    k = np.zeros((J + 1, L))
    check(lib.pxm_tiling_axisym(int(L), float(B), int(J_min), k0.ctypes.data, k.ctypes.data))
    return k0, k


def mw_ring_weights(L):
    q = np.zeros(L)
    check(lib.pxm_mw_ring_weights(int(L), q.ctypes.data))
    return q


def rec_geometry(L, spin, chains):
    out = (C.c_int * 4)()
    if lib.pxm_host_rec_geometry(int(L), int(spin), int(chains), out) < 0:
        return None
    return tuple(int(v) for v in out)


DFT_UNITS = ("radix2", "pair", "quad")


def dft_geometry(L):
    out = (C.c_int * 6)()
    check(lib.pxm_host_dft_geometry(int(L), out))
    return (DFT_UNITS[out[0]], int(out[1]), int(out[2]), int(out[3]), int(out[4]), bool(out[5]))


def noise_bits():
    return int(lib.pxm_noise_bits())


GEMM_TASK_FIELDS = ("m_unit", "row0", "n_rt", "k_beg", "k_end", "pole_n", "nslab", "side", "par", "row_lo", "row_hi", "row_lo1",
                    "row_hi1", "sign1", "side_b", "m")
_GEMM_HEAD = ("ncol", "n_sides", "n_tasks", "flags", "nslab", "pk", "ws_doubles", "off_scratch", "scratch_doubles", "off_counter",
              "max_chains", "paired")
_GEMM_SIDE = ("off_x", "off_x2", "off_y", "off_ks", "off_rs", "off_hd", "xL", "xRp", "xn", "yL", "yRp", "yn", "n_x", "n_y", "n_tab",
              "n_pole")
_GEMM_TABLE = ("n_m", "Rp", "paired", "n_tab", "n_pole", "L", "spin", "kind")


def _gemm_words(call, what, side):
    n = check(call(what, side, None, 0))
    out = (C.c_int64 * max(int(n), 1))()
    check(call(what, side, out, n))
    return np.array(out[:n], dtype=np.int64)


def gemm_report(call, n_sides):
    w = _gemm_words(call, 0, 0)
    rep = {"layout": dict(zip(_GEMM_HEAD, (int(v) for v in w[:16]))),
           "sides": [dict(zip(_GEMM_SIDE, (int(v) for v in w[16 + 16 * i:32 + 16 * i]))) for i in range(n_sides)],
           "tasks": _gemm_words(call, 1, 0).reshape(-1, len(GEMM_TASK_FIELDS)), "tables": []}
    for i in range(n_sides):
        t = _gemm_words(call, 2, i)
        tab = dict(zip(_GEMM_TABLE, (int(v) for v in t[:8])))
        tab["orders"] = t[8:].reshape(-1, 5)
        rep["tables"].append(tab)
    return rep


def gemm_plan_geometry(sides, spin=0, max_chains=8, pk=0):
    from ._args import _gemm_sides

    desc = _gemm_sides(sides, max_chains, pk)
    return gemm_report(lambda what, side, out, cap: lib.pxm_host_gemm_plan_report(int(spin), int(max_chains), int(pk), desc, len(sides),
                                                                                  what, side, out, cap), len(sides))
```

pxmcmc_amd/ops/plans.py:

```python
import ctypes as C
import threading
import weakref

import numpy as np
import torch

from .._lib import STATUS_PAIR_SYNC, PxmError, check, lib, require_gpu
from .host import gemm_report
from ._args import (_CPLX, _REAL, _batched, _data_invcov, _dev_tensors, _gemm_sides, _nf, _noise_args, _p, _pair_noise_args, _result, _stream, _vecT, as_device,
                    device)


def raise_on_status(status, what):
    if status:
        bits = []
        if status & STATUS_PAIR_SYNC:
            bits.append("a wave-pair wait or ring-group wait of the fused phi-DFT kernels expired (csrc/dft_wave.h: d5_pair_sync)")
        if status & ~STATUS_PAIR_SYNC:
            bits.append(f"unknown status bits {status:#x}")
        raise PxmError(f"{what}: device status {status:#x}: " + "; ".join(bits) + " -- the results of this plan since its last "
                       "status check are invalid")


_LIVE_PLANS = weakref.WeakSet()
# ... 150 lines not shown
    def _table(self, side, which, n):
        if not 0 <= int(side) < self.n_sides:
            raise ValueError("GemmPlan: no such side")
        out = torch.empty(n, dtype=_REAL, device=device())
        if n:
            check(lib.pxm_gemm_plan_table_read(self._h, int(side), which, _p(out), n, _stream()))
        return out

    def table(self, side=0):
        return self._table(side, 0, self.tables[side]["n_tab"] if 0 <= int(side) < self.n_sides else 0)

    def pole(self, side=0):
        return self._table(side, 1, self.tables[side]["n_pole"] if 0 <= int(side) < self.n_sides else 0)

    def run(self, C_, affine=None, bump=False):
        if not 1 <= int(C_) <= self.max_chains:
            raise ValueError("more chains than the plan was created for")
        ns, w = (0.0, 0.0) if affine is None else affine
        w = complex(w)
        check(lib.pxm_gemm_plan_run(self._h, int(C_), int(affine is not None), float(ns), w.real, w.imag, int(bool(bump)), _stream()))

    def counter(self):
        return int(self.read(self.layout["off_counter"], 1).view(torch.int64).item())


def _update_out(out, x):
    return _result(out, x.shape, _CPLX, x.device, "out= buffer must be a distinct contiguous complex128 tensor of the state's shape",
                   distinct_from=x)


def _preds_out(preds_out, x, n):
    return _result(preds_out, (x.shape[0], n), _CPLX, x.device, "preds_out= buffer has the wrong shape / dtype / layout")


class _WaveletPlan(_Plan):

    def _fn(self, name):
        return getattr(lib, f"pxm_{self._abi}_{name}")

    @property
    def _nimg(self):
        return getattr(self, self._image)

    def synthesis(self, X, out=None):
        return self._run(self._fn("synthesis"), X, self.ncoefs, self._nimg, out=out)

    def synthesis_adjoint(self, f):
        return self._run(self._fn("synthesis_adjoint"), f, self._nimg, self.ncoefs)

    def analysis(self, f):
        return self._run(self._fn("analysis"), f, self._nimg, self.ncoefs)

    def analysis_adjoint(self, X):
        return self._run(self._fn("analysis_adjoint"), X, self.ncoefs, self._nimg)


class WavPlan(_WaveletPlan):

    _abi, _image = "wav", "npix"

    def __init__(self, L, B, J_min, max_chains=1, spin=0):
        require_gpu()
        self.L, self.B, self.J_min, self.max_chains = int(L), float(B), int(J_min), int(max_chains)
        self.spin = int(spin)
        self.npix = L * (2 * L - 1)
        nscal = C.c_int64()
        self.ncoefs = int(check(lib.pxm_wav_ncoefs(self.L, self.B, self.J_min, C.byref(nscal))))
        self.nscal = int(nscal.value)
        super().__init__(lib.pxm_wav_plan_create_spin, (self.L, self.B, self.J_min, self.spin, self.max_chains, 0),
                         lib.pxm_wav_plan_destroy, lib.pxm_wav_status, f"WavPlan(L={self.L}, spin={self.spin})")

    def _update_args(self, x, T, noise, noise_complex, pairs, out):
        Tv, Ts = _vecT(T, self.ncoefs, x.device)
        w, wc = _pair_noise_args(noise, x) if pairs else _noise_args(noise, x, noise_complex)
        return Tv, Ts, w, wc, _update_out(out, x)

    def gradg_step(self, X, preds, data, invcov, T, delta, lmda, noise=None, noise_complex=False, seed=0, chain0=0, it=0, out=None,
                   pairs=False, noise64=False):
        x, squeeze = _batched(as_device(X, _CPLX))
        p, _ = _batched(as_device(preds, _CPLX))
        if x.shape[1] != self.ncoefs or p.shape[1] != self.npix or p.shape[0] != x.shape[0]:
            raise AssertionError("gradg_step: shape mismatch")
        d, ic = _data_invcov(data, invcov, self.npix, _CPLX)
        Tv, Ts, w, wc, out = self._update_args(x, T, noise, noise_complex, pairs, out)
        check(
            lib.pxm_wav_gradg_step(
                self._h, _p(x), _p(p), _p(d), _p(ic), int(ic.is_complex()), _p(Tv), Ts, float(delta), float(lmda),
                _p(w), wc | _nf(noise64), seed, chain0, it, _p(out), x.shape[0], _stream(),
            )
        )
        return out[0] if squeeze else out

    def image_init(self, preds, data, invcov):
        p, _ = _batched(as_device(preds, _CPLX))
        if p.shape[1] != self.npix or p.shape[0] > self.max_chains:
            raise AssertionError("image_init: shape mismatch")
        d, ic = _data_invcov(data, invcov, self.npix, _CPLX)
        check(lib.pxm_wav_image_init(self._h, _p(p), _p(d), _p(ic), int(ic.is_complex()), p.shape[0], _stream()))

    def image_step(self, X, data, invcov, T, delta, lmda, noise=None, noise_complex=False, seed=0, chain0=0, it=0,
                   out=None, preds_out=None, pairs=False, noise64=False):
        x, squeeze = _batched(as_device(X, _CPLX))
        if x.shape[1] != self.ncoefs or x.shape[0] > self.max_chains:
            raise AssertionError("image_step: shape mismatch")
        d, ic = _data_invcov(data, invcov, self.npix, _CPLX)
        Tv, Ts, w, wc, out = self._update_args(x, T, noise, noise_complex, pairs, out)
        preds_out = _preds_out(preds_out, x, self.npix)
        check(
            lib.pxm_wav_image_step(
                self._h, _p(x), _p(d), _p(ic), int(ic.is_complex()), _p(Tv), Ts, float(delta), float(lmda),
                _p(w), wc | _nf(noise64), seed, chain0, it, _p(out), _p(preds_out), x.shape[0], _stream(),
            )
        )
        return (out[0], preds_out[0]) if squeeze else (out, preds_out)

    def ring_set_data(self, data):
        d = as_device(data, _CPLX).reshape(-1)
        if d.numel() != self.npix:
            raise ValueError("data length mismatch")
        check(lib.pxm_wav_ring_set_data(self._h, _p(d), _stream()))

    def ring_init(self, X):
        x, _ = _batched(as_device(X, _CPLX))
        if x.shape[1] != self.ncoefs or x.shape[0] > self.max_chains:
            raise AssertionError("ring_init: shape mismatch")
        check(lib.pxm_wav_ring_init(self._h, _p(x), x.shape[0], _stream()))

    def ring_step(self, X, w, T, delta, lmda, noise=None, noise_complex=False, seed=0, chain0=0, it=0, out=None, pairs=False,
                  noise64=False):
        x, squeeze = _batched(as_device(X, _CPLX))
        if x.shape[1] != self.ncoefs or x.shape[0] > self.max_chains:
            raise AssertionError("ring_step: shape mismatch")
        Tv, Ts, wn, wc, out = self._update_args(x, T, noise, noise_complex, pairs, out)
        w = complex(w)
        check(
            lib.pxm_wav_ring_step(
                self._h, _p(x), w.real, w.imag, _p(Tv), Ts, float(delta), float(lmda), _p(wn), wc | _nf(noise64), seed, chain0, it,
                _p(out), x.shape[0], _stream(),
            )
        )
        return out[0] if squeeze else out

    def ring_preds(self, C_, out=None):
        if out is None:
            out = torch.empty((C_, self.npix), dtype=_CPLX, device=device())
        check(lib.pxm_wav_ring_preds(self._h, _p(out), C_, _stream()))
        return out

    def table_bytes(self, op):
        return int(lib.pxm_wav_table_bytes(self._h, op))

    def exact_dft_scales(self):
        return int(check(lib.pxm_wav_exact_dft_scales(self._h)))

    def wl_attach(self, pix2data, weight, ndata):
        if pix2data is not None:
            pix2data = pix2data.to(device=device(), dtype=torch.int32).contiguous()
            if pix2data.numel() != self.npix:
                raise ValueError("pix2data must have one entry per pixel")
        if weight is not None:
            weight = as_device(weight, _REAL).reshape(-1)
            if weight.numel() != int(ndata):
                raise ValueError("weight must have one entry per datum")
        self._wl = (pix2data, weight, int(ndata))
        check(lib.pxm_wav_wl_attach(self._h, _p(pix2data), _p(weight), int(ndata)))

    def wl_uses_recursion(self):
        return int(check(lib.pxm_wav_wl_uses_recursion(self._h)))

    def wl_forward(self, X, out=None):
        x, squeeze = _batched(as_device(X, _CPLX))
        if x.shape[1] != self.ncoefs or x.shape[0] > self.max_chains:
            raise AssertionError("wl_forward: shape mismatch")
        nd = self._wl[2]
        if out is None:
            out = torch.empty((x.shape[0], nd), dtype=_CPLX, device=x.device)
        check(lib.pxm_wav_wl_forward(self._h, _p(x), _p(out), x.shape[0], _stream()))
        return out[0] if squeeze else out

    def wl_adjoint(self, gamma, data=None, invcov=None, out=None):
        g, squeeze = _batched(as_device(gamma, _CPLX))
        nd = self._wl[2]
        if g.shape[1] != nd or g.shape[0] > self.max_chains:
            raise AssertionError("wl_adjoint: shape mismatch")
        d = ic = None
        if data is not None:
            d, ic = _data_invcov(data, invcov, nd, _CPLX)
        if out is None:
            out = torch.empty((g.shape[0], self.ncoefs), dtype=_CPLX, device=g.device)
        check(lib.pxm_wav_wl_adjoint(self._h, _p(g), _p(d), _p(ic), int(ic.is_complex()) if ic is not None else 0, _p(out),
                                     g.shape[0], _stream()))
        return out[0] if squeeze else out

    def workspace_nonfinite(self):
        return int(check(lib.pxm_wav_workspace_nonfinite(self._h, _stream())))

    def profile_enable(self, max_launches):
        check(lib.pxm_wav_profile_enable(self._h, int(max_launches)))

    def profile_read_launches(self, cap):
        ms, nb, wg, n = np.zeros(cap), np.zeros(cap), np.zeros(cap, dtype=np.int32), C.c_int64()
        check(lib.pxm_wav_profile_read_launches(self._h, ms.ctypes.data, nb.ctypes.data, wg.ctypes.data, int(cap), C.byref(n)))
        k = min(int(n.value), cap)
        return ms[:k], nb[:k], wg[:k]

    def profile_read(self):
        ms, nl, nb, nf = C.c_double(), C.c_int64(), C.c_double(), C.c_double()
        check(lib.pxm_wav_profile_read(self._h, C.byref(ms), C.byref(nl), C.byref(nb), C.byref(nf)))
        dms, dnl, dnb = C.c_double(), C.c_int64(), C.c_double()
        check(lib.pxm_wav_profile_read_dft(self._h, C.byref(dms), C.byref(dnl), C.byref(dnb)))
        return (ms.value, nl.value, nb.value, nf.value), (dms.value, dnl.value, dnb.value)


class DirWavPlan(_WaveletPlan):

    _abi, _image = "dwav", "npix"

    def __init__(self, L, B, J_min, N, max_chains=1):
        require_gpu()
        self.L, self.B, self.J_min, self.N, self.max_chains = int(L), float(B), int(J_min), int(N), int(max_chains)
        self.npix = L * (2 * L - 1)
        nscal = C.c_int64()
        self.ncoefs = int(check(lib.pxm_dwav_ncoefs(self.L, self.B, self.J_min, self.N, C.byref(nscal))))
        self.nscal = int(nscal.value)
        super().__init__(lib.pxm_dwav_plan_create, (self.L, self.B, self.J_min, self.N, self.max_chains, 0),
                         lib.pxm_dwav_plan_destroy, lib.pxm_dwav_status, f"DirWavPlan(L={self.L}, N={self.N})")

    def table_bytes(self):
        return int(lib.pxm_dwav_table_bytes(self._h))

    def info(self):
        a, b, c = C.c_int(), C.c_int(), C.c_int()
        check(lib.pxm_dwav_plan_info(self._h, C.byref(a), C.byref(b), C.byref(c)))
        return a.value, b.value, c.value


class HarmWavPlan(_WaveletPlan):

    _abi, _image = "hwav", "nlm"

    def __init__(self, L, B, J_min, N=1, spin=0, max_chains=1):
        require_gpu()
        self.L, self.B, self.J_min, self.N, self.max_chains = int(L), float(B), int(J_min), int(N), int(max_chains)
        self.spin = int(spin)
        self.nlm = self.L * self.L
        nscal = C.c_int64()
        self.ncoefs = int(check(lib.pxm_hwav_ncoefs(self.L, self.B, self.J_min, self.N, C.byref(nscal))))
        self.nscal = int(nscal.value)
        super().__init__(lib.pxm_hwav_plan_create, (self.L, self.B, self.J_min, self.N, self.spin, self.max_chains, 0),
                         lib.pxm_hwav_plan_destroy, lib.pxm_hwav_status,
                         f"HarmWavPlan(L={self.L}, N={self.N}, spin={self.spin})")

    def info(self):
        a, b, c = C.c_int(), C.c_int(), C.c_int()
        check(lib.pxm_hwav_plan_info(self._h, C.byref(a), C.byref(b), C.byref(c)))
        return a.value, b.value, c.value

    def myula_step(self, X, data, invcov, kernel, T, delta, lmda, noise_complex=False, seed=0, chain0=0, it=0, iter_dev=None,
                   out=None, preds_out=None, noise64=False):
        x, squeeze = _batched(as_device(X, _CPLX))
        if x.shape[1] != self.ncoefs or x.shape[0] > self.max_chains:
            raise AssertionError("myula_step: shape mismatch")
        d, ic = _data_invcov(data, invcov, self.nlm, _CPLX)
        k = None
        if kernel is not None:
            k = as_device(kernel, _REAL).reshape(-1)
            if k.numel() != self.nlm:
                raise ValueError("kernel length mismatch")
        Tv, Ts = _vecT(T, self.ncoefs, x.device)
        out, preds_out = _update_out(out, x), _preds_out(preds_out, x, self.nlm)
        check(
            lib.pxm_hwav_myula_step(
                self._h, _p(x), _p(d), _p(ic), int(ic.is_complex()), _p(k), _p(Tv), Ts, float(delta), float(lmda),
                int(bool(noise_complex)) | _nf(noise64), seed, chain0, it, _p(iter_dev), _p(out), _p(preds_out), x.shape[0],
                _stream(),
            )
        )
        return (out[0], preds_out[0]) if squeeze else (out, preds_out)


class IterCounter:

    def __init__(self, plan, start=0):
        self.plan = plan
        self.t = torch.full((1,), int(start), dtype=torch.int64, device=device())
        check(lib.pxm_wav_set_iter_counter(plan._h, C.c_void_p(self.t.data_ptr())))
        self.active = True

    def set(self, value):
        self.t.fill_(int(value))

    def add(self, inc=1):
        check(lib.pxm_wav_iter_counter_add(self.plan._h, int(inc), _stream()))

    def close(self):
        if self.active:
            if getattr(self.plan, "_h", None):
                lib.pxm_wav_release_iter_counter(self.plan._h, C.c_void_p(self.t.data_ptr()))
            self.active = False

    def __del__(self):
        try:
            self.close()
        except Exception:
            pass

# ... 15 lines not shown
```

Measured before the change: 126,800.

## Add specialized stock fused ring2px MYULA step kernel with parked transform values

Adds a STOCK template instantiation of the fused ring-to-pixel DFT + MYULA chain update kernels. It is selected at runtime when the step matches the common configuration: real pairs, even chain0, device iteration counter, and no data or weights. The specialized path parks the DFT output in LDS, batches the X/T loads and Philox draws, and splits the Box-Muller computation into a table-lookup phase and a finish phase with scheduling barriers and uniform constants. This is meant to cut branching and register pressure and to overlap memory latency with RNG work. It is on by default and can be turned off with PXM_DFT_STOCK, at the cost of extra kernel instantiations and a duplicated code path.

```diff
diff --git a/include/pxmcmc_amd.h b/include/pxmcmc_amd.h
--- a/include/pxmcmc_amd.h
+++ b/include/pxmcmc_amd.h
@@ -42,6 +42,7 @@
 int pxm_host_rec_geometry(int L, int spin, int C, int* out);
 int pxm_host_pfa511_tables(uint16_t* idx, double* b2);
 int pxm_host_dft_geometry(int L, int* out);
+int pxm_host_dft_step_is_stock(unsigned fields, int mode, uint64_t chain0);
 
 int pxm_sht_plan_create(int L, int spin, int max_chains, unsigned flags, pxm_sht_plan_t* plan);
 int pxm_sht_plan_destroy(pxm_sht_plan_t plan);
@@ -111,6 +112,7 @@
 int pxm_wav_status(pxm_wav_plan_t plan, int clear, pxm_stream_t stream);
 int pxm_sht_status(pxm_sht_plan_t plan, int clear, pxm_stream_t stream);
 int pxm_wav_exact_dft_scales(pxm_wav_plan_t plan);
+int pxm_wav_dft_stock(pxm_wav_plan_t plan);
 
 int pxm_wav_profile_enable(pxm_wav_plan_t plan, int max_launches);
 int pxm_wav_profile_read(pxm_wav_plan_t plan, double* gemm_ms, int64_t* gemm_launches, double* gemm_alg_bytes,
diff --git a/pxmcmc_amd/_lib.py b/pxmcmc_amd/_lib.py
--- a/pxmcmc_amd/_lib.py
+++ b/pxmcmc_amd/_lib.py
@@ -23,6 +23,7 @@
     "pxm_wav_release_iter_counter": (c_int, [c_vp, c_vp]),
     "pxm_wav_iter_counter_add": (c_int, [c_vp, c_u64, c_vp]),
     "pxm_wav_exact_dft_scales": (c_int, [c_vp]),
+    "pxm_wav_dft_stock": (c_int, [c_vp]),
     "pxm_wav_status": (c_int, [c_vp, c_int, c_vp]),
     "pxm_sht_status": (c_int, [c_vp, c_int, c_vp]),
     "pxm_wav_profile_enable": (c_int, [c_vp, c_int]),
@@ -41,6 +42,7 @@
     "pxm_host_rec_geometry": (c_int, [c_int, c_int, c_int, c_vp]),
     "pxm_host_pfa511_tables": (c_int, [c_vp, c_vp]),
     "pxm_host_dft_geometry": (c_int, [c_int, c_vp]),
+    "pxm_host_dft_step_is_stock": (c_int, [C.c_uint, c_int, c_u64]),
     "pxm_quantile_range": (c_int, [c_vp, c_i64, c_i64, c_i64, c_dbl, c_vp, c_vp]),
     "pxm_moments_update": (c_int, [c_vp, c_int, c_vp, c_vp, c_vp, c_vp, c_vp, c_int, c_vp, c_vp, c_i64, c_int, c_vp]),
     "pxm_moments_scratch_doubles": (c_i64, [c_i64]),
diff --git a/pxmcmc_amd/csrc/dft.hip b/pxmcmc_amd/csrc/dft.hip
--- a/pxmcmc_amd/csrc/dft.hip
+++ b/pxmcmc_amd/csrc/dft.hip
@@ -160,6 +160,7 @@
   p->n = 2 * L - 1;
   p->Rp = round_up(L, 16);
   p->unit = g.unit;
+  if (const char* e = getenv("PXM_DFT_STOCK")) p->stock = atoi(e) != 0;
   if (g.unit == DFT_PAIR) {
     if (const char* e = getenv("PXM_DEBUG_PAIR_SYNC_LIMIT")) p->spin_limit = (unsigned)std::max(0, atoi(e));
     return pair_make_tables(p->n, g.pfa, &p->pair);
diff --git a/pxmcmc_amd/csrc/dft_pfa.h b/pxmcmc_amd/csrc/dft_pfa.h
--- a/pxmcmc_amd/csrc/dft_pfa.h
+++ b/pxmcmc_amd/csrc/dft_pfa.h
@@ -132,9 +132,10 @@
 constexpr int PFA_STAGE_S = 514;
 static_assert(4 * PFA_STAGE_S <= 4 * PFA_PLANE, "a ring group's stage fits in its four planes");
 
-template <bool RING_OUT, bool N64>
+template <bool RING_OUT, bool N64, bool STOCK = false>
 __device__ __forceinline__ void ring2px_body_pfa(const Dft5Args& a, const PfaTabs& pt, double* __restrict__ G, int ncol,
                                                  const PxOut& out, int C, int bxw, int by, int passes, double2* lds5) {
+  static_assert(!STOCK || (RING_OUT && N64), "the stock instantiation is the fused step with the fp64 noise stream");
   if ((by << 2) >= C) return;
 #ifdef PXM_D5_TRACE
   unsigned long long d5_stamp[7] = {0, 0, 0, 0, 0, 0, 0};
@@ -179,7 +180,7 @@
     (void)ch; (void)stage; (void)plane; (void)logt; (void)sct; (void)gcnt; (void)x0k; (void)lane;
     if (tid < 72) B2l[tid] = pt.B2[tid];
 #if !defined(PXM_NOISE_F64_POLY)
-    if (N64 && out.X && !out.noise && tid < NOISE_LOG_N + 256)
+    if (N64 && (STOCK || (out.X && !out.noise)) && tid < NOISE_LOG_N + 256)
       B2l[72 + tid] = tid < NOISE_LOG_N ? reinterpret_cast<const double2*>(&NOISE_LOG_TAB[0][0])[tid]
                                         : reinterpret_cast<const double2*>(&NOISE_SINCOS_TAB[0][0])[tid - NOISE_LOG_N];
 #endif
@@ -228,10 +229,24 @@
   const int64_t e0 = out.ring0 + (int64_t)t * n + lane;
   const int64_t ce0 = (int64_t)ch * out.chain_stride + e0;
   const bool last_ok = lane < 63;
-  const uint64_t it_eff = out.iter + (out.iter_dev ? *out.iter_dev : 0);
+  const uint64_t it_eff = out.iter + ((STOCK || out.iter_dev) ? *out.iter_dev : 0);
   const int ch_s = __builtin_amdgcn_readfirstlane(ch);
 #pragma unroll
   for (int g0 = 0; g0 < 8; g0 += 4) {
+    if constexpr (STOCK) {
+      double2* park = plane + lane + 64 * g0;
+      if (act) {
+        const bool ok[4] = {true, true, true, g0 + 3 < 7 || last_ok};
+        px_stock_update4<64>(out, ok, e0 + 64 * g0, ce0 + 64 * g0, -lane - 64 * g0, ch_s, it_eff, park, logt, sct);
+      } else {
+#pragma unroll
+        for (int u = 0; u < 4; ++u) park[64 * u] = double2{0.0, 0.0};
+      }
+#ifdef PXM_D5_TRACE
+      if (g0 == 0) PXM_D5_STAMP(3) else PXM_D5_STAMP(4)
+#endif
+      continue;
+    }
     double2 x[4];
     if (!N64 || !(act && out.X)) {
 #pragma unroll
diff --git a/pxmcmc_amd/csrc/dft_plan.hip b/pxmcmc_amd/csrc/dft_plan.hip
--- a/pxmcmc_amd/csrc/dft_plan.hip
+++ b/pxmcmc_amd/csrc/dft_plan.hip
@@ -11,6 +11,25 @@
 };
 
 extern "C" {
+
+int pxm_host_dft_step_is_stock(unsigned fields, int mode, uint64_t chain0) {
+  PXM_REQUIRE((fields & ~0xffu) == 0, "pxm_host_dft_step_is_stock: fields has eight bits");
+  static const double some = 0;
+  static const uint64_t some_u = 0;
+  static const int32_t some_i = 0;
+  PxOut o;
+  o.X = (fields & 1) ? &some : nullptr;
+  o.T = (fields & 2) ? &some : nullptr;
+  o.noise = (fields & 4) ? &some : nullptr;
+  o.iter_dev = (fields & 8) ? &some_u : nullptr;
+  o.rdata = (fields & 16) ? &some : nullptr;
+  o.rinvcov = (fields & 32) ? &some : nullptr;
+  o.gidx = (fields & 64) ? &some_i : nullptr;
+  o.gw = (fields & 128) ? &some : nullptr;
+  o.mode = mode;
+  o.chain0 = chain0;
+  return dft_step_is_stock(o) ? 1 : 0;
+}
 
 int pxm_host_dft_geometry(int L, int* out) {
   PXM_REQUIRE(out, "pxm_host_dft_geometry: null output");
diff --git a/pxmcmc_amd/csrc/dft_wave.hip b/pxmcmc_amd/csrc/dft_wave.hip
--- a/pxmcmc_amd/csrc/dft_wave.hip
+++ b/pxmcmc_amd/csrc/dft_wave.hip
@@ -72,6 +72,18 @@
 #pragma unroll
   for (int u = 0; u < 4; ++u) {
     const double2 o = pplane[256 * SLOT + 64 * u + lane], own = x[u];
+    x[u] = d5_sel(half, o, own);
+    x[4 + u] = d5_sel(half, own, o);
+  }
+}
+
+template <int SLOT>
+__device__ __forceinline__ void d5_exchange_fill_parked(double2 (&x)[8], const double2* plane, const double2* pplane, int lane, int half,
+                                                        unsigned* pcnt, unsigned& epoch, const D5Sync& sy) {
+  d5_pair_sync(pcnt, epoch += 2, lane, sy);
+#pragma unroll
+  for (int u = 0; u < 4; ++u) {
+    const double2 o = pplane[256 * SLOT + 64 * u + lane], own = plane[256 * SLOT + 64 * u + lane];
     x[u] = d5_sel(half, o, own);
     x[4 + u] = d5_sel(half, own, o);
   }
@@ -188,7 +200,7 @@
 #else
 #define PXM_D5_STAMP(K)
 #endif
-template <int R0, bool RING_OUT, bool N64>
+template <int R0, bool RING_OUT, bool N64, bool STOCK = false>
 __device__ __forceinline__ void ring2px_body5(const Dft5Args& a, double* __restrict__ G, int ncol, const PxOut& out, int C,
                                               int bx, int by, double2* lds5) {
   if ((by << 2) >= C) return;
@@ -243,7 +255,19 @@
   const bool act = ch < C && tv;
   const int64_t e0 = out.ring0 + (int64_t)t * n + jb + (int64_t)(8 * R0) * pb;
   const int64_t ce0 = (int64_t)ch * out.chain_stride + e0;
-  if (act && out.X) {
+  if constexpr (STOCK) {
+    static_assert(RING_OUT && N64, "the stock instantiation is the fused step with the fp64 noise stream");
+    double2* park = plane + 256 + lane;
+#pragma unroll
+    for (int u = 0; u < 4; ++u) park[64 * u] = act ? x[u] : double2{0.0, 0.0};
+    if (act) {
+      bool ok[4];
+#pragma unroll
+      for (int u = 0; u < 4; ++u) ok[u] = jb + 8 * R0 * (pb + u) < n;
+      px_stock_update4<8 * R0>(out, ok, e0, ce0, -(jb + 8 * R0 * pb), __builtin_amdgcn_readfirstlane(ch), out.iter + *out.iter_dev, park,
+                               reinterpret_cast<const double2*>(&NOISE_LOG_TAB[0][0]), reinterpret_cast<const double2*>(&NOISE_SINCOS_TAB[0][0]));
+    }
+  } else if (act && out.X) {
     const uint64_t it_eff = out.iter + (out.iter_dev ? *out.iter_dev : 0);
     const int ch_s = __builtin_amdgcn_readfirstlane(ch);
 #pragma unroll
@@ -331,7 +355,8 @@
   }
   if (!RING_OUT) return;
   PXM_D5_STAMP(2)
-  d5_exchange_fill<1>(x, plane, pplane, lane, half, pcnt, epoch, sy);
+  if constexpr (STOCK) d5_exchange_fill_parked<1>(x, plane, pplane, lane, half, pcnt, epoch, sy);
+  else d5_exchange_fill<1>(x, plane, pplane, lane, half, pcnt, epoch, sy);
   d5_pair_sync(pcnt, epoch += 2, lane, sy);
   PXM_D5_TRANSFORM(0)
   PXM_D5_STAMP(3)
@@ -368,7 +393,7 @@
   px2ring_body5<R0>(a, in, G, ncol, C, blockIdx.x, blockIdx.y, lds5);
 }
 
-template <int R0, bool RING_OUT, bool N64>
+template <int R0, bool RING_OUT, bool N64, bool STOCK = false>
 __global__ __launch_bounds__(128 * D5_RMAX, 4) void k_ring2px5(Dft5Args a, double* __restrict__ G, int ncol,
                                                                                  PxOut out, int C) {
   extern __shared__ double2 lds5[];
@@ -376,11 +401,11 @@
     if (a.pfa && ncol >= 8) {
       const PfaTabs pt{reinterpret_cast<const uint16_t*>(a.pfa + PFA_TAB_GAT), reinterpret_cast<const uint16_t*>(a.pfa + PFA_TAB_KIDX),
                        reinterpret_cast<const double2*>(a.pfa + PFA_TAB_B2)};
-      ring2px_body_pfa<RING_OUT, N64>(a, pt, G, ncol, out, C, blockIdx.x, blockIdx.y, 1, lds5);
+      ring2px_body_pfa<RING_OUT, N64, STOCK>(a, pt, G, ncol, out, C, blockIdx.x, blockIdx.y, 1, lds5);
       return;
     }
   }
-  ring2px_body5<R0, RING_OUT, N64>(a, G, ncol, out, C, blockIdx.x, blockIdx.y, lds5);
+  ring2px_body5<R0, RING_OUT, N64, STOCK>(a, G, ncol, out, C, blockIdx.x, blockIdx.y, lds5);
 }
 
 #define PXM_D5_GROUP_DECODE                                              \
@@ -415,7 +440,7 @@
   return hipMemcpyToSymbol(HIP_SYMBOL(g_dft_trace), &buf, sizeof(buf)) == hipSuccess ? 0 : -1;
 }
 #endif
-template <bool RING_OUT, bool N64>
+template <bool RING_OUT, bool N64, bool STOCK = false>
 __global__ __launch_bounds__(128 * D5_RMAX, 4) void k_ring2px_group5(const Dft5Group* __restrict__ ents, int nent,
                                                                                        double* __restrict__ ws, int ncol, PxOut out,
                                                                                        int C) {
@@ -429,14 +454,14 @@
     const double* pb = ws + g.tbase + g.pfa_off;
     const PfaTabs pt{reinterpret_cast<const uint16_t*>(pb + PFA_TAB_GAT), reinterpret_cast<const uint16_t*>(pb + PFA_TAB_KIDX),
                      reinterpret_cast<const double2*>(pb + PFA_TAB_B2)};
-    ring2px_body_pfa<RING_OUT, N64>(a, pt, G, ncol, out, C, bx, by, g.pfa_passes, lds5);
+    ring2px_body_pfa<RING_OUT, N64, STOCK>(a, pt, G, ncol, out, C, bx, by, g.pfa_passes, lds5);
   }
   switch (g.r0) {
     case 9: break;
-    case 8: ring2px_body5<8, RING_OUT, N64>(a, G, ncol, out, C, bx, by, lds5); break;
-    case 4: ring2px_body5<4, RING_OUT, N64>(a, G, ncol, out, C, bx, by, lds5); break;
-    case 2: ring2px_body5<2, RING_OUT, N64>(a, G, ncol, out, C, bx, by, lds5); break;
-    default: ring2px_body5<1, RING_OUT, N64>(a, G, ncol, out, C, bx, by, lds5); break;
+    case 8: ring2px_body5<8, RING_OUT, N64, STOCK>(a, G, ncol, out, C, bx, by, lds5); break;
+    case 4: ring2px_body5<4, RING_OUT, N64, STOCK>(a, G, ncol, out, C, bx, by, lds5); break;
+    case 2: ring2px_body5<2, RING_OUT, N64, STOCK>(a, G, ncol, out, C, bx, by, lds5); break;
+    default: ring2px_body5<1, RING_OUT, N64, STOCK>(a, G, ncol, out, C, bx, by, lds5); break;
   }
 #ifdef PXM_D5_TRACE
   if (threadIdx.x == 0 && g_dft_trace) {
@@ -802,7 +827,8 @@
   static std::atomic<uint64_t> done{0};
   return allow_dynamic_lds(done, {reinterpret_cast<const void*>(k_px2ring5<R0>), reinterpret_cast<const void*>(k_ring2px5<R0, false, false>),
                                   reinterpret_cast<const void*>(k_ring2px5<R0, true, false>), reinterpret_cast<const void*>(k_ring2px5<R0, false, true>),
-                                  reinterpret_cast<const void*>(k_ring2px5<R0, true, true>)});
+                                  reinterpret_cast<const void*>(k_ring2px5<R0, true, true>),
+                                  reinterpret_cast<const void*>(k_ring2px5<R0, true, true, true>)});
 }
 
 template <int R0>
@@ -829,7 +855,8 @@
   double* Gw = const_cast<double*>(G);
   const bool n64 = out.X && !out.noise && out.noise64;
   if (ring_out) {
-    if (n64) hipLaunchKernelGGL((k_ring2px5<R0, true, true>), grid, block, D5_LDS, st, da, Gw, ncol, out, C);
+    if (n64 && p.stock && dft_step_is_stock(out)) hipLaunchKernelGGL((k_ring2px5<R0, true, true, true>), grid, block, D5_LDS, st, da, Gw, ncol, out, C);
+    else if (n64) hipLaunchKernelGGL((k_ring2px5<R0, true, true>), grid, block, D5_LDS, st, da, Gw, ncol, out, C);
     else hipLaunchKernelGGL((k_ring2px5<R0, true, false>), grid, block, D5_LDS, st, da, Gw, ncol, out, C);
   } else {
     if (n64) hipLaunchKernelGGL((k_ring2px5<R0, false, true>), grid, block, D5_LDS, st, da, Gw, ncol, out, C);
@@ -931,9 +958,11 @@
   out->n = (int)v.size();
   out->all = v.size() == plans.size();
   out->blocks = b0;
+  out->stock = plans[order[0]]->stock;
   if (int rc = dev_table(&out->d, v, "DFT group entries")) return rc;
   static std::atomic<uint64_t> lds_done{0};
   return allow_dynamic_lds(lds_done, {reinterpret_cast<const void*>(k_ring2px_group5<true, false>), reinterpret_cast<const void*>(k_ring2px_group5<true, true>),
+                                      reinterpret_cast<const void*>(k_ring2px_group5<true, true, true>),
                                       reinterpret_cast<const void*>(k_ring2px_group5<false, false>), reinterpret_cast<const void*>(k_ring2px_group5<false, true>),
                                       reinterpret_cast<const void*>(k_px2ring_group5)});
 }
@@ -951,7 +980,10 @@
   hipEvent_t ev0 = nullptr, ev1 = nullptr;
   if (prof) prof->next(prof->dft, &ev0, &ev1, bytes, 0.0);
   const Dft5Group* ents = reinterpret_cast<const Dft5Group*>(g.d);
-  if (out.X && !out.noise && out.noise64)
+  if (g.stock && out.noise64 && dft_step_is_stock(out))
+    hipExtLaunchKernelGGL((k_ring2px_group5<true, true, true>), dim3(g.blocks), dim3(128 * D5_RMAX), D5_LDS, st, ev0, ev1, 0,
+                          ents, g.n, ws, ncol, out, C);
+  else if (out.X && !out.noise && out.noise64)
     hipExtLaunchKernelGGL((k_ring2px_group5<true, true>), dim3(g.blocks), dim3(128 * D5_RMAX), D5_LDS, st, ev0, ev1, 0,
                           ents, g.n, ws, ncol, out, C);
   else
diff --git a/pxmcmc_amd/csrc/elem.h b/pxmcmc_amd/csrc/elem.h
--- a/pxmcmc_amd/csrc/elem.h
+++ b/pxmcmc_amd/csrc/elem.h
@@ -27,6 +27,9 @@
 __device__ inline double chain_step_real(double X, double px, double g, double w, double delta, double lmda) {
   const double r = delta / lmda;
   return (1 - r) * X + r * px - delta * g + sqrt(2 * delta) * w;
+}
+__device__ __forceinline__ double chain_step_real_rs(double X, double px, double g, double w, double delta, double r, double s) {
+  return (1 - r) * X + r * px - delta * g + s * w;
 }
 __device__ inline double2 chain_step_cplx(double2 X, double2 px, double2 g, double2 w, double delta, double lmda) {
   return double2{chain_step_real(X.x, px.x, g.x, w.x, delta, lmda), chain_step_real(X.y, px.y, g.y, w.y, delta, lmda)};
diff --git a/pxmcmc_amd/csrc/philox.h b/pxmcmc_amd/csrc/philox.h
--- a/pxmcmc_amd/csrc/philox.h
+++ b/pxmcmc_amd/csrc/philox.h
@@ -129,6 +129,61 @@
   const double S = cs.y + fma(cs.x, sa, cs.y * cm1);
   return NormalPair{g * C, g * S};
 }
+struct BoxMullerLook {
+  double m;
+  int ex;
+  double a;
+  double2 lt, cs;
+};
+__device__ inline BoxMullerLook box_muller_f64_tab_look(double u1, double u2, const double2* logt, const double2* sct) {
+  BoxMullerLook L;
+  L.ex = __builtin_amdgcn_frexp_exp(u1);
+  L.m = __builtin_amdgcn_frexp_mant(u1);
+  const int j = min(max((int)__builtin_rint(L.m * 256.0), NOISE_LOG_J0), 256);
+  L.lt = logt[j - NOISE_LOG_J0];
+  const double t = 256.0 * u2;
+  const double k = __builtin_rint(t);
+  L.a = (t - k) * 0.024543692606170259675;
+  L.cs = sct[(int)k & 255];
+  return L;
+}
+template <bool PIN>
+__device__ __forceinline__ double box_muller_const(double c) {
+  if constexpr (PIN) asm volatile("" : "+s"(c));
+  return c;
+}
+template <bool PIN>
+__device__ inline NormalPair box_muller_f64_tab_finish(const BoxMullerLook& L) {
+  const double m = L.m;
+  const double2 lt = L.lt;
+  const double r = fma(m, lt.x, -1.0);
+  double p = 1.0 / 7.0;
+  p = fma(p, r, box_muller_const<PIN>(-1.0 / 6.0));
+  p = fma(p, r, box_muller_const<PIN>(1.0 / 5.0));
+  p = fma(p, r, box_muller_const<PIN>(-0.25));
+  p = fma(p, r, box_muller_const<PIN>(1.0 / 3.0));
+  p = fma(p, r, -0.5);
+  p = fma(p, r, 1.0);
+  p *= r;
+  const double e = (double)L.ex;
+  double x = fma(-2.0, p, fma(e, -2.0 * 0.693147180369123816490, fma(e, -2.0 * 1.90821492927058770002e-10, lt.y)));
+  x = fmax(x, 1e-300);
+  double h = __builtin_amdgcn_rsq(x);
+  double g = x * h;
+  h *= 0.5;
+  const double rr = fma(-h, g, 0.5);
+  g = fma(g, rr, g);
+  g = fma(fma(-g, g, x), h, g);
+  const double a = L.a;
+  const double2 cs = L.cs;
+  const double a2 = a * a;
+  const double q = fma(fma(a2, -1.0 / 5040.0, box_muller_const<PIN>(1.0 / 120.0)), a2, box_muller_const<PIN>(-1.0 / 6.0));
+  const double sa = fma(a * a2, q, a);
+  const double cm1 = fma(fma(a2, -1.0 / 720.0, box_muller_const<PIN>(1.0 / 24.0)), a2, -0.5) * a2;
+  const double C = cs.x + fma(-cs.y, sa, cs.x * cm1);
+  const double S = cs.y + fma(cs.x, sa, cs.y * cm1);
+  return NormalPair{g * C, g * S};
+}
 __device__ inline NormalPair box_muller_f64_tab(double u1, double u2) {
   return box_muller_f64_tab(u1, u2, reinterpret_cast<const double2*>(&NOISE_LOG_TAB[0][0]), reinterpret_cast<const double2*>(&NOISE_SINCOS_TAB[0][0]));
 }
@@ -163,6 +218,16 @@
   const uint64_t b = (((uint64_t)c.w << 32) | c.z) >> 11;
   return box_muller_f64_tab(((double)a + 0.5) * 0x1.0p-53, ((double)b + 0.5) * 0x1.0p-53, logt, sct);
 }
+__device__ inline BoxMullerLook normal_look_from_bits(const uint4 c, const double2* logt, const double2* sct) {
+  const uint64_t a = (((uint64_t)c.y << 32) | c.x) >> 11;
+  const uint64_t b = (((uint64_t)c.w << 32) | c.z) >> 11;
+  return box_muller_f64_tab_look(((double)a + 0.5) * 0x1.0p-53, ((double)b + 0.5) * 0x1.0p-53, logt, sct);
+}
+__device__ inline NormalPair normal_pair_from_bits_poly(const uint4 c) {
+  const uint64_t a = (((uint64_t)c.y << 32) | c.x) >> 11;
+  const uint64_t b = (((uint64_t)c.w << 32) | c.z) >> 11;
+  return box_muller_f64_poly(((double)a + 0.5) * 0x1.0p-53, ((double)b + 0.5) * 0x1.0p-53);
+}
 __device__ inline NormalPair philox_normal_pair_tabs(uint64_t seed, uint64_t chain, uint64_t index, uint64_t iter, const double2* logt,
                                                      const double2* sct) {
   const uint64_t key = seed + chain * 0x9E3779B97F4A7C15ull;
diff --git a/pxmcmc_amd/csrc/sht_core.h b/pxmcmc_amd/csrc/sht_core.h
--- a/pxmcmc_amd/csrc/sht_core.h
+++ b/pxmcmc_amd/csrc/sht_core.h
@@ -106,6 +106,7 @@
   QuadTables quad;
   unsigned* d_status = nullptr;
   unsigned spin_limit = 1u << 18;
+  bool stock = true;
 };
 enum { PXM_STATUS_PAIR_SYNC_BIT = 2 };
 
@@ -154,6 +155,10 @@
   const double* gw = nullptr;
 };
 
+inline bool dft_step_is_stock(const PxOut& o) {
+  return o.X && o.T && !o.noise && o.mode == 2 && !(o.chain0 & 1) && o.iter_dev && !o.rdata && !o.rinvcov && !o.gidx && !o.gw;
+}
+
 struct DftGroupList {
   void* d = nullptr;
   int n = 0, blocks = 0;
@@ -162,6 +167,7 @@
   int64_t ring_end = 0;
   std::vector<char> member;
   bool all = false;
+  bool stock = true;
 };
 int dft_group_create(const std::vector<const DftPlan*>& plans, const std::vector<int64_t>& g_off,
                      const std::vector<int64_t>& ring0, int ncol, const double* ws_base,
diff --git a/pxmcmc_amd/csrc/update.h b/pxmcmc_amd/csrc/update.h
--- a/pxmcmc_amd/csrc/update.h
+++ b/pxmcmc_amd/csrc/update.h
@@ -187,4 +187,56 @@
   return chain_step_cplx(x, px, g, w, o.delta, o.lmda);
 }
 
-}
+static_assert(PXM_MODE_REAL_PAIRS == 2, "dft_step_is_stock (sht_core.h) names the real-pair mode by its value");
+
+__device__ __forceinline__ double px_uniform(double v) {
+  const uint64_t b = __builtin_bit_cast(uint64_t, v);
+  const uint32_t lo = __builtin_amdgcn_readfirstlane((uint32_t)b), hi = __builtin_amdgcn_readfirstlane((uint32_t)(b >> 32));
+  return __builtin_bit_cast(double, ((uint64_t)hi << 32) | lo);
+}
+
+template <int ES>
+__device__ __forceinline__ void px_stock_update4(const PxOut& out, const bool (&ok)[4], int64_t e0, int64_t ce0, int zoff, int ch_s,
+                                                 uint64_t it, double2* park, const double2* logt, const double2* sct) {
+  const double delta = out.delta, r_dl = px_uniform(out.delta / out.lmda), s_2d = px_uniform(sqrt(2 * out.delta));
+  double2 xs[4];
+  double Ts[4];
+  int eo[4];
+#pragma unroll
+  for (int u = 0; u < 4; ++u) eo[u] = ok[u] ? ES * u : zoff;
+#pragma unroll
+  for (int u = 0; u < 4; ++u) xs[u] = reinterpret_cast<const double2*>(out.X)[ce0 + eo[u]];
+#pragma unroll
+  for (int u = 0; u < 4; ++u) Ts[u] = out.T[e0 + eo[u]];
+  __builtin_amdgcn_sched_barrier(0);
+  uint4 pbits[4];
+#pragma unroll
+  for (int u = 0; u < 4; ++u) pbits[u] = philox_bits(out.seed + PXM_PAIR_TWEAK, (out.chain0 >> 1) + ch_s, (uint64_t)(e0 + ES * u), it);
+  __builtin_amdgcn_sched_barrier(0);
+  auto finish_elem = [&](int u, const NormalPair& q) {
+    double2 xn{0.0, 0.0};
+    if (ok[u]) {
+      const double2 xv = park[64 * u];
+      xn = double2{chain_step_real_rs(xs[u].x, soft_real(xs[u].x, Ts[u]), xv.x, q.z0, delta, r_dl, s_2d),
+                   chain_step_real_rs(xs[u].y, soft_real(xs[u].y, Ts[u]), -xv.y, q.z1, delta, r_dl, s_2d)};
+      reinterpret_cast<double2*>(out.f)[ce0 + ES * u] = xn;
+    }
+    park[64 * u] = xn;
+  };
+#pragma unroll
+  for (int u = 0; u < 4; u += 2) {
+#if defined(PXM_NOISE_F64_POLY)
+    (void)logt, (void)sct;
+    const NormalPair qa = normal_pair_from_bits_poly(pbits[u]), qb = normal_pair_from_bits_poly(pbits[u + 1]);
+#else
+    const BoxMullerLook la = normal_look_from_bits(pbits[u], logt, sct), lb = normal_look_from_bits(pbits[u + 1], logt, sct);
+    const NormalPair qa = box_muller_f64_tab_finish<true>(la), qb = box_muller_f64_tab_finish<true>(lb);
+#endif
+    __builtin_amdgcn_sched_barrier(0);
+    finish_elem(u, qa);
+    finish_elem(u + 1, qb);
+    __builtin_amdgcn_sched_barrier(0);
+  }
+}
+
+}
diff --git a/pxmcmc_amd/csrc/wav_plan.hip b/pxmcmc_amd/csrc/wav_plan.hip
--- a/pxmcmc_amd/csrc/wav_plan.hip
+++ b/pxmcmc_amd/csrc/wav_plan.hip
@@ -338,6 +338,11 @@
   return p->dft_group.d ? p->dft_group.n_pfa : 0;
 }
 
+int pxm_wav_dft_stock(pxm_wav_plan_t p) {
+  PXM_REQUIRE(p, "pxm_wav_dft_stock: null plan");
+  return (p->dft_group.d && p->dft_group.stock) ? 1 : 0;
+}
+
 int64_t pxm_wav_table_bytes(pxm_wav_plan_t p, int op) {
   if (!p || op < 0 || op > 1) return -1;
   return p->table_bytes[op];
diff --git a/pxmcmc_amd/ops/__init__.py b/pxmcmc_amd/ops/__init__.py
--- a/pxmcmc_amd/ops/__init__.py
+++ b/pxmcmc_amd/ops/__init__.py
@@ -1,7 +1,7 @@
 from .._lib import (FISTA_SLICES_MAX, LCI_EMPTY, LCI_NONFINITE, LCI_POINTS, LCI_UNCONSTRAINED, SAPG_GROUPS_MAX, SAPG_SLICES_MAX,
                     PxmError, check, require_gpu)
 from ._args import GEMM_KINDS, _batched, _p, _stream, as_device, device
-from .host import (DFT_UNITS, GEMM_TASK_FIELDS, dft_geometry, gemm_plan_geometry, gemm_report, j_max, mw_ring_weights, noise_bits, rec_geometry, tiling_axisym,
+from .host import (DFT_STEP_FIELDS, DFT_UNITS, GEMM_TASK_FIELDS, dft_geometry, dft_step_is_stock, gemm_plan_geometry, gemm_report, j_max, mw_ring_weights, noise_bits, rec_geometry, tiling_axisym,
                    wav_bandlimits)
 from .lci import lci_data_terms, lci_eval, lci_scratch, lci_search
 from .plans import (DftPlan, DirWavPlan, GemmPlan, HarmWavPlan, IterCounter, ShtPlan, WavPlan, _Plan, capture_scope, live_plans, raise_on_status,
diff --git a/pxmcmc_amd/ops/host.py b/pxmcmc_amd/ops/host.py
--- a/pxmcmc_amd/ops/host.py
+++ b/pxmcmc_amd/ops/host.py
@@ -45,6 +45,16 @@
     return (DFT_UNITS[out[0]], int(out[1]), int(out[2]), int(out[3]), int(out[4]), bool(out[5]))
 
 
+DFT_STEP_FIELDS = ("X", "T", "noise", "iter_dev", "rdata", "rinvcov", "gidx", "gw")
+
+
+def dft_step_is_stock(fields, mode, chain0):
+    bits = 0
+    for f in fields:
+        bits |= 1 << DFT_STEP_FIELDS.index(f)
+    return bool(check(lib.pxm_host_dft_step_is_stock(bits, int(mode), int(chain0))))
+
+
 def noise_bits():
     return int(lib.pxm_noise_bits())
 
diff --git a/pxmcmc_amd/ops/plans.py b/pxmcmc_amd/ops/plans.py
--- a/pxmcmc_amd/ops/plans.py
+++ b/pxmcmc_amd/ops/plans.py
@@ -326,6 +326,9 @@
 
     def exact_dft_scales(self):
         return int(check(lib.pxm_wav_exact_dft_scales(self._h)))
+
+    def dft_stock(self):
+        return bool(check(lib.pxm_wav_dft_stock(self._h)))
 
     def wl_attach(self, pix2data, weight, ndata):
         if pix2data is not None:
```

New measurement: 129,400, median of 6. 2.0% higher.
